# google-research/semivl

Hardware: AMD Instinct MI355X
Metric: train images/sec (512^2, ViT-B/16) (higher is better)
Workload: dtype f32 (fp32 in / out / accumulate everywhere; the MFMA products as split 16-bit terms with fp32 accumulation: the ViT's linears, in_proj weight gradients and fused attention and the decoder's 3x3 convolutions (tiled: forward, input and weight gradient; dilated: forward, input gradient) on fp16 x 2 ope; 1 GPU; SemiVL step, pascal N=21, vlm-vlg-aspp-s2p4-sk04-ftap-mcvitb, 512x512, bs=16/GPU labeled + 16/GPU unlabeled (BASELINE configs[1]); global_batch=32, parallelism=dp1

## Files before the change

### include/semivl_hip.h

```cpp
#ifndef SEMIVL_HIP_H_
#define SEMIVL_HIP_H_

#include <stddef.h>
#include <stdint.h>

#ifdef __cplusplus
extern "C" {
#endif

typedef void* svl_stream_t;

typedef enum svl_status {
  SVL_OK = 0,
  SVL_ERR_INVALID_ARG = -1,
  SVL_ERR_LAUNCH = -2,
  SVL_ERR_UNSUPPORTED = -3
} svl_status;

int svl_version(void);
int svl_stream_release(svl_stream_t stream);
int svl_stream_prepare(svl_stream_t stream);
int svl_stream_helper(svl_stream_t stream, void** helper);
int svl_shutdown(void);
int svl_num_stream_contexts(void);
// ... 128 lines not shown
                        svl_stream_t stream);

int svl_cutmix_f32(float* out, const float* a, const float* b, const float* box, int B, int C, int64_t HW,
                   svl_stream_t stream);
int svl_cutmix_i64(int64_t* out, const int64_t* a, const int64_t* b, const float* box, int B, int64_t HW,
                   svl_stream_t stream);

typedef struct svl_ce_desc {
  const float* logits;
  int B, N;
  int64_t HW;
  const int64_t* target;
  int use_ignore_t;
  const float* conf;
  const int64_t* ign;
  float conf_thresh;
  int all_pixels;
  const int64_t* mc_target;
  float* partials;
  float* dlogits;
  const float* gscale;
  const float* img_weight;
} svl_ce_desc;
int64_t svl_ce_num_blocks(int B, int N, int64_t HW);
int svl_ce_fused_f32(const svl_ce_desc* d, svl_stream_t stream);
int svl_ce_finalize(const float* partials, int64_t nblocks, double* sums , svl_stream_t stream);

typedef struct svl_ce_up_desc {
  const float* logits;
  int B, N;
  int h, w, H, W;
  int align_corners;
  const int64_t* target;
  int use_ignore_t;
  const float* conf;
  const int64_t* ign;
  float conf_thresh;
  int all_pixels;
  const int64_t* mc_target;
  float* partials;
  float* dlogits;
  const float* gscale;
  const float* img_weight;
} svl_ce_up_desc;
int64_t svl_ce_up_num_blocks(int B, int N, int h, int w, int H, int W, int align_corners);
int svl_ce_up_fused_f32(const svl_ce_up_desc* d, svl_stream_t stream);
int svl_softmax_max_up_f32(const float* logits, int B, int N, int h, int w, int H, int W, int align_corners, float* conf,
                           int64_t* label, svl_stream_t stream);

int svl_semivl_gscale(const int64_t* counts, double numel_u, float lam, const double* factors, const int64_t* mc_counts,
                      float* gscale, svl_stream_t stream);
int64_t svl_conf_avg_ws_doubles(int B);
int svl_conf_avg_factor(const float* conf, const int64_t* ign, int B, int64_t HW, double* factor, double* workspace,
                        svl_stream_t stream);
int svl_conf_ratio_f32(const float* conf, const int64_t* ign, int B, int64_t HW, float thresh, float* ratio,
                       double* workspace, svl_stream_t stream);
int svl_semivl_loss(const double* sums, double numel_u, float lam, const double* factors, const int64_t* mc_counts,
                    float* out, svl_stream_t stream);
int svl_softmax_planes_f32(const float* logits, int B, int N, int64_t HW, float* out, svl_stream_t stream);

int svl_target_prob_f32(const float* logits, int B, int N, int64_t HW, const int64_t* target, float* prob,
                        svl_stream_t stream);
int svl_target_prob_up_f32(const float* logits, int B, int N, int h, int w, int H, int W, int align_corners,
                           const int64_t* target, float* prob, svl_stream_t stream);
int64_t svl_ohem_ws_bytes(int64_t n);
int svl_ohem_threshold_f32(const float* prob, int64_t n, int64_t k, const int64_t* num_valid, int64_t min_kept,
                           float thresh, void* ws, float* threshold, svl_stream_t stream);
int svl_ohem_relabel_i64(const int64_t* target, const float* prob, int64_t n, const float* threshold, int64_t* out,
                         int64_t* count, svl_stream_t stream);

int svl_count_valid_i64(const int64_t* map, int64_t n, int64_t* count, svl_stream_t stream);

int svl_maskclip_labels(const float* dense, int B, int N, int h, int w, int H, int W, float scale,
                        float thresh, const int64_t* ign, int64_t* out, svl_stream_t stream);

int svl_concept_max_f32(const float* pred, int B, int NC, int64_t HW, const int* concept_offsets, int N,
                        float* out, svl_stream_t stream);

int svl_iou_hist_i64(const int64_t* pred, const int64_t* target, int64_t n, int K, int ignore_index, int64_t* hist,
                     svl_stream_t stream);


int svl_layernorm_fwd(const float* x, const float* gamma, const float* beta, float eps, int64_t rows, int C,
                      float* y, float* stats, svl_stream_t stream);
int svl_layernorm_fwd_planes(const float* x, const float* gamma, const float* beta, float eps, int64_t rows, int C,
                             float* y, float* stats, void* planes, int64_t planes_rows, svl_stream_t stream);
int svl_layernorm_fwd_planes_f16x2(const float* x, const float* gamma, const float* beta, float eps, int64_t rows, int C,
                                   float* y, float* stats, void* planes, int64_t planes_rows, int32_t* sexp, float* rnorm,
                                   svl_stream_t stream);
int svl_layernorm_fwd_pack_f16x2(const float* x, const float* gamma, const float* beta, float eps, int64_t rows, int C,
                                 float* y, float* stats, void* planes, int64_t planes_rows, int64_t row_off, int32_t* sexp,
                                 float* rnorm, int row_rnorm, unsigned* tensor_amax, svl_stream_t stream);
int svl_layernorm_bwd_pack_f16x2(const float* dy, const float* x, const float* stats, const float* gamma, int64_t rows, int C,
                                 const float* dx_add, float* dx, void* planes, int64_t planes_rows, int64_t row_off,
                                 int32_t* sexp, float* rnorm, unsigned* tensor_amax, svl_stream_t stream);
int svl_layernorm_bwd_parts(int64_t rows);
int svl_layernorm_bwd(const float* dy, const float* x, const float* stats, const float* gamma, int64_t rows,
                      int C, const float* dx_add, float* dx, float* dgamma_part, float* dbeta_part,
                      svl_stream_t stream);
int svl_softmax_rows_fwd(float* s, int64_t rows, int cols, int64_t ld, float scale, svl_stream_t stream);
int svl_softmax_rows_bwd(float* dp, const float* p, int64_t rows, int cols, int64_t ld, float scale,
                         svl_stream_t stream);

int svl_l2norm_fwd(const float* x, int64_t rows, int C, float eps, float* y, float* inv_norm, svl_stream_t stream);
int svl_l2norm_bwd(const float* dy, const float* y, const float* inv_norm, int64_t rows, int C, float* dx,
                   svl_stream_t stream);

int64_t svl_colsum_ws_floats(int64_t rows, int C);
int svl_colsum_f32(const float* x, int64_t rows, int C, int64_t ld, float* out, int accumulate, float* ws,
                   svl_stream_t stream);

int svl_eltwise_f32(int mode, const float* a, const float* b, float* out, int64_t n, svl_stream_t stream);
int svl_chanmask_f32(const float* x, const float* mask, float scale, int64_t rows, int rows_per_img, int C,
                     float* out, svl_stream_t stream);
int svl_fill_f32(float* p, float v, int64_t n, svl_stream_t stream);
int svl_bernoulli_f32(float* p, int64_t n, float keep_prob, uint64_t seed, uint64_t offset, svl_stream_t stream);
int svl_affine_planes_f32(const float* x, int64_t planes, int C, int64_t HW, const float* k4, float* y, svl_stream_t stream);
int svl_copy2d_f32(const float* src, int64_t sgrp, int64_t src_go, int64_t src_ld, float* dst, int64_t dgrp,
                   int64_t dst_go, int64_t dst_ld, int64_t rows, int C, int accumulate, svl_stream_t stream);
int svl_permute4_f32(const float* src, float* dst, int64_t n0, int64_t n1, int64_t n2, int64_t n3, int64_t s0, int64_t s1,
                     int64_t s2, int64_t s3, svl_stream_t stream);
int svl_bound2_f32(const float* rnorm, int64_t rows, const float* bias, int64_t nbias, float* out2, svl_stream_t stream);
int svl_permute_rows_f32(const float* src, int64_t outer, int A, int B, int C, float* dst, svl_stream_t stream);

int svl_groupnorm_fwd(const float* x, int64_t ldx, const float* gamma, const float* beta, float eps, int imgs,
                      int64_t HW, int C, int G, int relu, float* y, int64_t ldy, float* stats, svl_stream_t stream);
int64_t svl_conv3x3_gn_ws_doubles(int imgs, int H, int W, int N);
int svl_conv3x3_gn_f32(const float* src1, int64_t ld1, int C1, const float* src2, int64_t ld2, int C2, int rep,
                       const float* w, int imgs, int H, int W, int N, float* out, int64_t ldo, float eps, double* ws,
                       float* stats, const float* gn_in, const void* w_planes, svl_stream_t stream);
int64_t svl_conv3x3_weight_planes_bytes(int N, int Ct);
int svl_conv3x3_weight_planes(const float* w, int N, int Ct, void* planes, svl_stream_t stream);
int svl_groupnorm_scale_shift(const float* stats, const float* gamma, const float* beta, int imgs, int C, int G, float* scsh,
                              svl_stream_t stream);
int svl_groupnorm_apply(const float* x, int64_t ldx, const float* gamma, const float* beta, int imgs, int64_t HW, int C, int G,
                        int relu, const float* stats, float* y, int64_t ldy, svl_stream_t stream);
int svl_groupnorm_bwd(const float* dy, int64_t lddy, const float* x, int64_t ldx, const float* y, int64_t ldy,
                      const float* stats, const float* gamma, const float* beta, int imgs, int64_t HW, int C, int G,
                      int relu, float* dx, int64_t lddx, float* chan_sums, svl_stream_t stream);
int64_t svl_conv3x3_gnb_ws_doubles(int imgs, int H, int W, int N);
int svl_conv3x3_dgrad_gnb_f32(const float* dy, int64_t lddy, int C1, const float* w, int imgs, int H, int W, int N, float* out,
                              int64_t ldo, int accumulate, const float* gnb_x, const float* gnb_table, const float* gnb_stats,
                              double* ws, float* chan_sums, const void* w_planes, svl_stream_t stream);
int svl_groupnorm_bwd_apply(const float* dy, int64_t lddy, const float* x, int64_t ldx, const float* stats, const float* gamma,
                            const float* beta, int imgs, int64_t HW, int C, int G, int relu, const float* chan_sums, float* dx,
                            int64_t lddx, svl_stream_t stream);


int svl_attention_fwd(const float* qkv, int B, int T, int H, float* out, float* lse, void* out_planes,
                      int64_t planes_rows, svl_stream_t stream);
int svl_attention_bwd(const float* qkv, const float* out, const float* dout, const float* lse, int B, int T, int H,
                      float* dsum_ws, float* dqkv, void* dqkv_planes, int64_t planes_rows, svl_stream_t stream);
int64_t svl_attention_h2_ws_bytes(int B, int T, int H, int backward);
int svl_attention_fwd_h2(const float* qkv, int B, int T, int H, float* out, float* lse, void* out_planes,
                         int64_t planes_rows, void* ws, int64_t ws_bytes, svl_stream_t stream);
int svl_attention_bwd_h2(const float* qkv, const float* out, const float* dout, const float* lse, int B, int T, int H,
                         float* dsum_ws, float* dqkv, void* dqkv_planes, int64_t planes_rows, void* ws, int64_t ws_bytes,
                         svl_stream_t stream);

typedef struct svl_seqattn_desc {
  int groups, inner, seq, heads;
  int64_t outer_stride, inner_stride, seq_stride;
  const float* qkv;
  float* out;
  float* probs;
  const float* dout;
  float* dqkv;
  float* dscores;
} svl_seqattn_desc;
int svl_seqattn_fwd(const svl_seqattn_desc* d, svl_stream_t stream);
int svl_seqattn_bwd(const svl_seqattn_desc* d, svl_stream_t stream);

int svl_conv_cout1_fwd(const float* x, int64_t ldx, int imgs, int H, int W, int C, int KH, int KW, int dil, int pad,
                       const float* w, const float* bias, const float* gn_in, float* y, svl_stream_t stream);
int svl_conv_cout1_wgrad_blocks(int imgs, int H, int W);
int svl_conv_cout1_wgrad(const float* dy, const float* x, int64_t ldx, int imgs, int H, int W, int C, int dil, int pad,
                         const float* gn_in, float* slabs, svl_stream_t stream);
int svl_tap_gather(const float* T, int imgs, int H, int W, int KH, int KW, int dil, int pad, int sign, float* out,
                   svl_stream_t stream);

int svl_bilinear_nhwc_fwd(const float* x, int64_t ldx, int imgs, int h, int w, int C, int align_corners, int rep,
                          int H, int W, float* y, int64_t ldy, int accumulate, svl_stream_t stream);
int svl_sum_rep_f32(const float* src, int64_t ld, int64_t groups, int rep, int64_t rows, int C, float* out,
                    svl_stream_t stream);
int svl_bilinear_nhwc_bwd(const float* dy, int64_t lddy, int imgs, int h, int w, int C, int align_corners, int rep,
                          int H, int W, float* dx, int64_t lddx, int accumulate, svl_stream_t stream);
int svl_bilinear_planes_fwd(const float* x, int64_t planes, int h, int w, int align_corners, int H, int W, float* y,
                            svl_stream_t stream);
int svl_bilinear_planes_bwd(const float* dy, int64_t planes, int h, int w, int align_corners, int H, int W,
                            float* dx, svl_stream_t stream);
int svl_avgpool_cat_fwd(const float* x, int imgs, int H, int W, int C, int PH, int PW, const float* text, int Ct,
                        int nclass, float* y, svl_stream_t stream);
int svl_avgpool_cat_bwd(const float* dy, int imgs, int H, int W, int C, int PH, int PW, int Ct, float* dx,
                        int accumulate, svl_stream_t stream);
int svl_avgpool_cat_bwd_text(const float* dy, int imgs, int64_t HWp, int C, int Ct, int nclass, float* part, float* dtext,
                             svl_stream_t stream);

int svl_adamw_step(float* p, const float* g, float* m, float* v, const int64_t* seg_off, const float* seg_lr,
                   const float* seg_wd, int nseg, int64_t total, float beta1, float beta2, float eps, int step,
                   float gscale, float* ema, float ema_decay, svl_stream_t stream);
int svl_sgd_step(float* p, const float* g, float* m, const int64_t* seg_off, const float* seg_lr, const float* seg_wd,
                 int nseg, int64_t total, float momentum, float dampening, int nesterov, int step, float gscale,
                 float* ema, float ema_decay, svl_stream_t stream);

int64_t svl_bn_ws_doubles(int64_t rows, int C);
int svl_bn_stats(const float* x, int64_t ldx, int64_t rows, int C, double* sums, double* ws, svl_stream_t stream);
int svl_bn_finalize(const double* sums, double count, float eps, float momentum, float* running_mean, float* running_var,
                    int C, float* mean, float* invstd, svl_stream_t stream);
int svl_bn_eval_invstd(const float* running_var, float eps, int C, float* invstd, svl_stream_t stream);
int svl_bn_apply(const float* x, int64_t ldx, int64_t rows, int C, const float* mean, const float* invstd,
                 const float* gamma, const float* beta, const float* resid, int64_t ldr, int relu, float* y, int64_t ldy,
                 svl_stream_t stream);
int svl_bn_bwd_reduce(const float* dy, int64_t lddy, const float* x, int64_t ldx, const float* y, int64_t ldy,
                      const float* mean, const float* invstd, const float* remask_gamma, const float* remask_beta,
                      int64_t rows, int C, double* sums, double* ws, svl_stream_t stream);
int svl_bn_bwd_apply(const float* dy, int64_t lddy, const float* x, int64_t ldx, const float* y, int64_t ldy,
                     const float* mean, const float* invstd, const float* gamma, const float* remask_beta,
                     const double* sums, double count, int64_t rows, int C, float* dx, int64_t lddx, float* dres,
                     int64_t lddr, svl_stream_t stream);
int svl_maxpool3x3s2_fwd(const float* x, int imgs, int H, int W, int C, float* y, unsigned char* idx,
                         svl_stream_t stream);
int svl_maxpool3x3s2_bwd(const float* dy, const unsigned char* idx, int imgs, int H, int W, int C, float* dx,
                         svl_stream_t stream);

int svl_gap_tokens_fwd(const float* x, int64_t ldx, int imgs, int64_t HW, int C, float* pool, int64_t ldp,
                       svl_stream_t stream);
int svl_gap_tokens_bwd(const float* dpool, int64_t ldp, int imgs, int64_t HW, int C, float* dx, int64_t lddx,
                       int accumulate, svl_stream_t stream);
int svl_bcast_rows_fwd(const float* v, int64_t ldv, int imgs, int64_t HW, int C, float* dst, int64_t ldd, int c_off,
                       svl_stream_t stream);
int svl_bcast_rows_bwd(const float* dy, int64_t lddy, int c_off, int imgs, int64_t HW, int C, float* dv, int64_t ldv,
                       svl_stream_t stream);

int svl_aug_resample_u8(const unsigned char* src, int H, int W, int C, int rh, int rw, int x0, int y0, int OH, int OW,
                        int flip, int mode, int fill, unsigned char* dst, svl_stream_t stream);
int svl_aug_to_float(const unsigned char* src, int npix, const float* mean3, const float* std3, float* dst,
                     svl_stream_t stream);
int svl_aug_mask_i64(const unsigned char* src, int npix, int from, int to, int64_t* dst, svl_stream_t stream);
int svl_aug_photometric_u8(unsigned char* img, int npix, int op, float factor, unsigned long long* scratch,
                           svl_stream_t stream);
int svl_aug_gaussian_blur_u8(const unsigned char* src, int H, int W, float sigma, unsigned char* tmp, unsigned char* dst,
                             svl_stream_t stream);

#ifdef __cplusplus
}
#endif
#endif
```

### semivl_amd/csrc/attention.hip

```cpp
#include "attn_shared.h"
#include "attn_h2.h"

namespace {

__device__ __forceinline__ void tile_gload(float4 (&rg)[4], const float* base, long ld, int row0, int T, int tid) {
#pragma unroll
  for (int p = 0; p < 4; ++p) {
    const int f = tid + 256 * p;
    const int row = row0 + (f >> 4), c4 = (f & 15) << 2;
    rg[p] = (row < T) ? *reinterpret_cast<const float4*>(base + (long)row * ld + c4) : make_float4(0.f, 0.f, 0.f, 0.f);
  }
}
template <int LD>
__device__ __forceinline__ void tile_sstore(float* S, const float4 (&rg)[4], int tid, float mul) {
#pragma unroll
  for (int p = 0; p < 4; ++p) {
    const int f = tid + 256 * p;
    const int row = f >> 4, c = (f & 15) << 2;
    *reinterpret_cast<float4*>(S + row * LD + c) = make_float4(rg[p].x * mul, rg[p].y * mul, rg[p].z * mul, rg[p].w * mul);
  }
}

__device__ __forceinline__ float4 ld4(const float* p) { return *reinterpret_cast<const float4*>(p); }
__device__ __forceinline__ void row_gload32(float (&r)[32], const float* p, float mul) {
// ... 408 lines not shown
  sum = block_sum_256(sum, red);
  const float o = weighted_rowsum(w, head + 2 * p.E, p.ld, p.T, red, tid);
  if (tid < D) {
    if (p.out) p.out[((long)b * p.T + qi) * p.E + h * D + tid] = o / sum;
  }
  if (tid == 0 && p.lse) p.lse[(long)z * p.T + qi] = mx + logf(sum);
}

__global__ __launch_bounds__(256) void attn_bwd_dq_rows_kernel(const AttnP p, int row0) {
  __shared__ __attribute__((aligned(16))) float qv[D];
  __shared__ __attribute__((aligned(16))) float ov[D];
  __shared__ float w[ROWS_MAX_T];
  __shared__ float red[256];
  const int tid = threadIdx.x, sub = tid & 15, grp = tid >> 4;
  const int z = blockIdx.y, b = z / p.H, h = z - b * p.H, qi = row0 + blockIdx.x;
  const float* head = p.qkv + (long)b * p.T * p.ld + h * D;
  if (tid < D) {
    qv[tid] = head[(long)qi * p.ld + tid] * p.scale;
    ov[tid] = p.dout[((long)b * p.T + qi) * p.E + h * D + tid];
  }
  __syncthreads();
  const float lse_i = p.lse[(long)z * p.T + qi], d_i = p.dsum[(long)z * p.T + qi];
  for (int j0 = 0; j0 < p.T; j0 += 16) {
    const int j = j0 + grp;
    const float* kr = head + p.E + (long)min(j, p.T - 1) * p.ld;
    const float sc = dot16(qv, kr, sub), dp = dot16(ov, kr + p.E, sub);
    if (j < p.T && sub == 0) w[j] = expf(sc - lse_i) * (dp - d_i);
  }
  __syncthreads();
  const float dq = weighted_rowsum(w, head + p.E, p.ld, p.T, red, tid);
  if (tid < D) {
    p.dqkv[((long)b * p.T + qi) * p.ld + h * D + tid] = dq * p.scale;
  }
}

__global__ __launch_bounds__(256) void attn_bwd_dkv_rows_kernel(const AttnP p, int row0) {
  __shared__ __attribute__((aligned(16))) float kv[D];
  __shared__ __attribute__((aligned(16))) float vv[D];
  __shared__ float wp[ROWS_MAX_T];
  __shared__ float wd[ROWS_MAX_T];
  __shared__ float red[256];
  const int tid = threadIdx.x, sub = tid & 15, grp = tid >> 4;
  const int z = blockIdx.y, b = z / p.H, h = z - b * p.H, kj = row0 + blockIdx.x;
  const float* head = p.qkv + (long)b * p.T * p.ld + h * D;
  const float* dhead = p.dout + (long)b * p.T * p.E + h * D;
  if (tid < D) {
    kv[tid] = head[p.E + (long)kj * p.ld + tid] * p.scale;
    vv[tid] = head[2 * p.E + (long)kj * p.ld + tid];
  }
  __syncthreads();
  for (int i0 = 0; i0 < p.T; i0 += 16) {
    const int i = i0 + grp, ic = min(i, p.T - 1);
    const float sc = dot16(kv, head + (long)ic * p.ld, sub), dp = dot16(vv, dhead + (long)ic * p.E, sub);
    if (i < p.T && sub == 0) {
      const float pv = expf(sc - p.lse[(long)z * p.T + i]);
      wp[i] = pv;
      wd[i] = pv * (dp - p.dsum[(long)z * p.T + i]);
    }
  }
  __syncthreads();
  const float dv = weighted_rowsum(wp, dhead, p.E, p.T, red, tid);
  const float dk = weighted_rowsum(wd, head, p.ld, p.T, red, tid);
  if (tid < D) {
    float* row = p.dqkv + ((long)b * p.T + kj) * p.ld + h * D;
    row[p.E + tid] = dk * p.scale;
    row[2 * p.E + tid] = dv;
  }
}

__host__ inline int rows_split(int T, int* nb, int BQ = 128) {
  const int full = T / BQ, r = T - full * BQ;
  const bool use = r > 0 && r <= 4 && full > 0 && T <= ROWS_MAX_T;
  *nb = use ? full : (T + BQ - 1) / BQ;
  return use ? r : 0;
}

int check(const float* qkv, int B, int T, int H, const char* who) {
  SVL_CHECK_ARG(qkv && B > 0 && T > 0 && H > 0 && (long)B * H <= 65535, "%s: bad args", who);
  SVL_CHECK_ARG(((uintptr_t)qkv & 15) == 0, "%s: qkv must be 16-byte aligned", who);
  return SVL_OK;
}

int no_planes(const void* planes, const char* who) {
  if (!planes) return SVL_OK;
  svl_set_error("%s: planes outputs were retired with the bf16 x 6 attention kernels (pass null; pack the fp32 result)", who);
  return SVL_ERR_UNSUPPORTED;
}

}

extern "C" int svl_attention_fwd(const float* qkv, int B, int T, int H, float* out, float* lse, void* out_planes,
                                 int64_t planes_rows, svl_stream_t stream) {
  int rc = check(qkv, B, T, H, "svl_attention_fwd");
  if (rc) return rc;
  SVL_CHECK_ARG(out, "svl_attention_fwd: out missing");
  (void)planes_rows;
  rc = no_planes(out_planes, "svl_attention_fwd");
  if (rc) return rc;
  AttnP p;
  memset(&p, 0, sizeof(p));
  p.qkv = qkv; p.out = out; p.lse = lse; p.B = B; p.T = T; p.H = H; p.E = (long)H * D; p.ld = 3 * p.E; p.scale = 0.125f;
  hipStream_t st = (hipStream_t)stream;
  int nb = 0;
  const int r = rows_split(T, &nb, 128);
  if (r > 0) {
    hipStream_t aux = nullptr;
    rc = svl_fork(st, &aux);
    if (rc) return rc;
    hipLaunchKernelGGL(attn_fwd_rows_kernel, dim3(r, B * H), dim3(256), 0, aux, p, nb * 128);
    SVL_LAUNCH_CHECK("svl_attention_fwd/rows");
  }
  hipLaunchKernelGGL(attn_fwd_kernel, dim3(nb, B * H), dim3(256), 0, st, p);
  SVL_LAUNCH_CHECK("svl_attention_fwd");
  return r > 0 ? svl_join(st) : SVL_OK;
}

extern "C" int svl_attention_bwd(const float* qkv, const float* out, const float* dout, const float* lse, int B, int T,
                                 int H, float* dsum_ws, float* dqkv, void* dq_planes, int64_t planes_rows,
                                 svl_stream_t stream) {
  int rc = check(qkv, B, T, H, "svl_attention_bwd");
  if (rc) return rc;
  SVL_CHECK_ARG(out && dout && lse && dsum_ws && dqkv, "svl_attention_bwd: null args");
  (void)planes_rows;
  rc = no_planes(dq_planes, "svl_attention_bwd");
  if (rc) return rc;
  hipStream_t st = (hipStream_t)stream;
  AttnP p;
  memset(&p, 0, sizeof(p));
  p.qkv = qkv; p.dout = dout; p.lse = const_cast<float*>(lse); p.dsum = dsum_ws; p.dqkv = dqkv;
  p.B = B; p.T = T; p.H = H; p.E = (long)H * D; p.ld = 3 * p.E; p.scale = 0.125f;
  const long groups = (long)B * T * H;
  hipLaunchKernelGGL(attn_dsum_kernel, dim3((unsigned)((groups * 16 + 255) / 256)), dim3(256), 0, st, dout, out, dsum_ws,
                     B, T, H, p.E);
  SVL_LAUNCH_CHECK("svl_attention_bwd/dsum");
  int nb = 0;
  const int r = rows_split(T, &nb, 128);
  if (r > 0) {
    hipStream_t aux = nullptr;
    rc = svl_fork(st, &aux);
    if (rc) return rc;
    hipLaunchKernelGGL(attn_bwd_dkv_rows_kernel, dim3(r, B * H), dim3(256), 0, aux, p, nb * 128);
    SVL_LAUNCH_CHECK("svl_attention_bwd/dkv_rows");
    hipLaunchKernelGGL(attn_bwd_dq_rows_kernel, dim3(r, B * H), dim3(256), 0, aux, p, nb * 128);
    SVL_LAUNCH_CHECK("svl_attention_bwd/dq_rows");
  }
  hipLaunchKernelGGL(attn_bwd_dkv_kernel, dim3(nb, B * H), dim3(256), 0, st, p);
  SVL_LAUNCH_CHECK("svl_attention_bwd/dkv");
  hipLaunchKernelGGL(attn_bwd_dq_kernel, dim3(nb, B * H), dim3(256), 0, st, p);
  SVL_LAUNCH_CHECK("svl_attention_bwd/dq");
  return r > 0 ? svl_join(st) : SVL_OK;
}

extern "C" int64_t svl_attention_h2_ws_bytes(int B, int T, int H, int backward) {
  if (B <= 0 || T <= 0 || H <= 0) return 0;
  return svl_attn_h2::ws_bytes(B, T, H, backward);
}

extern "C" int svl_attention_fwd_h2(const float* qkv, int B, int T, int H, float* out, float* lse, void* out_planes,
                                    int64_t planes_rows, void* ws, int64_t ws_bytes, svl_stream_t stream) {
  int rc = check(qkv, B, T, H, "svl_attention_fwd_h2");
  if (rc) return rc;
  SVL_CHECK_ARG(out, "svl_attention_fwd_h2: out missing");
  (void)planes_rows;
  rc = no_planes(out_planes, "svl_attention_fwd_h2");
  if (rc) return rc;
  AttnP p;
  memset(&p, 0, sizeof(p));
  p.qkv = qkv; p.out = out; p.lse = lse; p.B = B; p.T = T; p.H = H; p.E = (long)H * D; p.ld = 3 * p.E; p.scale = 0.125f;
  hipStream_t st = (hipStream_t)stream;
  int nb = 0;
  const int r = rows_split(T, &nb, FQ);
  rc = svl_attn_h2::fwd_pack(p, ws, ws_bytes, st);
  if (rc) return rc;
  if (r > 0) {
    hipStream_t aux = nullptr;
    rc = svl_fork(st, &aux);
    if (rc) return rc;
    rc = svl_attn_h2::fwd_tail(p, nb * FQ, ws, aux);
    if (rc) return rc;
  }
  rc = svl_attn_h2::fwd(p, nb, ws, ws_bytes, st);
  if (rc) return rc;
  return r > 0 ? svl_join(st) : SVL_OK;
}

extern "C" int svl_attention_bwd_h2(const float* qkv, const float* out, const float* dout, const float* lse, int B, int T,
                                    int H, float* dsum_ws, float* dqkv, void* dq_planes, int64_t planes_rows, void* ws,
                                    int64_t ws_bytes, svl_stream_t stream) {
  int rc = check(qkv, B, T, H, "svl_attention_bwd_h2");
  if (rc) return rc;
  SVL_CHECK_ARG(out && dout && lse && dsum_ws && dqkv, "svl_attention_bwd_h2: null args");
  (void)planes_rows;
  rc = no_planes(dq_planes, "svl_attention_bwd_h2");
  if (rc) return rc;
  hipStream_t st = (hipStream_t)stream;
  AttnP p;
  memset(&p, 0, sizeof(p));
  p.qkv = qkv; p.dout = dout; p.lse = const_cast<float*>(lse); p.dsum = dsum_ws; p.dqkv = dqkv;
  p.B = B; p.T = T; p.H = H; p.E = (long)H * D; p.ld = 3 * p.E; p.scale = 0.125f;
  rc = svl_attn_h2::bwd_prepare(p, out, dsum_ws, ws, ws_bytes, st);
  if (rc) return rc;
  int nb = 0;
  const int r = rows_split(T, &nb, FQ);
  if (r > 0) {
    hipStream_t aux = nullptr;
    rc = svl_fork(st, &aux);
    if (rc) return rc;
    rc = svl_attn_h2::bwd_tail(p, nb * FQ, ws, aux);
    if (rc) return rc;
  }
  rc = svl_attn_h2::bwd_main(p, nb, ws, st);
  if (rc) return rc;
  return r > 0 ? svl_join(st) : SVL_OK;
}
```

### semivl_amd/csrc/attn_h2.h

```cpp
#pragma once
#include "attn_shared.h"

namespace svl_attn_h2 {

long ws_bytes(int B, int T, int H, int backward);
int fwd(const AttnP& p, int nb, void* ws, long wsb, hipStream_t st);
int bwd_prepare(const AttnP& p, const float* out, float* dsum_ws, void* ws, long wsb, hipStream_t st);
int bwd_main(const AttnP& p, int nb, void* ws, hipStream_t st);
int fwd_pack(const AttnP& p, void* ws, long wsb, hipStream_t st);
int fwd_tail(const AttnP& p, int row0, void* ws, hipStream_t aux);
int bwd_tail(const AttnP& p, int row0, void* ws, hipStream_t aux);

}
```

### semivl_amd/csrc/attn_h2.hip

```cpp
#include "attn_h2.h"
#include <atomic>

namespace {

typedef _Float16 f16x8 __attribute__((ext_vector_type(8)));
typedef _Float16 f16x2 __attribute__((ext_vector_type(2)));

struct H2W {
  const char *q_rm, *k_rm, *v_rm, *do_rm, *q_tr, *k_tr, *v_tr, *do_tr;
  const int* exps;
  const float* nrm;
  const float* ld;
  int Tp;
};

__device__ __forceinline__ void glds16(const char* base_, unsigned lane_off, unsigned lds_dst_) {
  const unsigned long long bv = (unsigned long long)base_;
  const unsigned b_hi = (unsigned)__builtin_amdgcn_readfirstlane((int)(bv >> 32));
  const unsigned b_lo = (unsigned)__builtin_amdgcn_readfirstlane((int)(unsigned)bv);
  const char* base = (const char*)(((unsigned long long)b_hi << 32) | (unsigned long long)b_lo);
  const unsigned lds_dst = __builtin_amdgcn_readfirstlane(lds_dst_);
  unsigned keep;
  asm volatile("s_mov_b32 %0, m0\n\ts_mov_b32 m0, %3\n\ts_nop 3\n\tglobal_load_lds_dwordx4 %2, %1\n\ts_mov_b32 m0, %0"
               : "=&s"(keep)
               : "s"(base), "v"(lane_off), "s"(lds_dst)
               : "memory");
}
template <int N_>
__device__ __forceinline__ void wait_vm() {
  asm volatile("s_waitcnt vmcnt(%0)" ::"n"(N_) : "memory");
}
__device__ __forceinline__ void interval_barrier() {
  asm volatile("s_waitcnt lgkmcnt(0)" ::: "memory");
  __builtin_amdgcn_sched_barrier(0);
  __builtin_amdgcn_s_barrier();
  __builtin_amdgcn_sched_barrier(0);
}

__device__ __forceinline__ f32x16 mfma_h(const f16x8& a, const f16x8& b, const f32x16& c) {
  return __builtin_amdgcn_mfma_f32_32x32x16_f16(a, b, c, 0, 0, 0);
}
#define H2_PAIR(c0, a0, c1, a1, b)    \
  c0 = mfma_h(a0[1], b[0], c0);       \
  c1 = mfma_h(a1[1], b[0], c1);       \
  c0 = mfma_h(a0[0], b[1], c0);       \
  c1 = mfma_h(a1[0], b[1], c1);       \
  c0 = mfma_h(a0[0], b[0], c0);       \
  c1 = mfma_h(a1[0], b[0], c1);
#define H2_2(c0, a0, b0, c1, a1, b1)  \
  c0 = mfma_h(a0[1], b0[0], c0);      \
  c1 = mfma_h(a1[1], b1[0], c1);      \
  c0 = mfma_h(a0[0], b0[1], c0);      \
  c1 = mfma_h(a1[0], b1[1], c1);      \
  c0 = mfma_h(a0[0], b0[0], c0);      \
  c1 = mfma_h(a1[0], b1[0], c1);
#define H2_2T(c0, a0, b0, c1, a1, b1) \
  c0 = mfma_h(a0[0], b0[1], c0);      \
  c1 = mfma_h(a1[0], b1[1], c1);      \
  c0 = mfma_h(a0[1], b0[0], c0);      \
  c1 = mfma_h(a1[1], b1[0], c1);      \
  c0 = mfma_h(a0[0], b0[0], c0);      \
  c1 = mfma_h(a1[0], b1[0], c1);

template <bool MIX>
__device__ __forceinline__ void split2x8(const float (&x)[8], f16x8 (&h)[2]) {
  u32x4 w0, w1;
#pragma unroll
  for (int jp = 0; jp < 4; ++jp) {
    const f32x2 pr = {x[2 * jp], x[2 * jp + 1]};
    const f16x2 ah = __builtin_convertvector(pr, f16x2);
    const unsigned a = __builtin_bit_cast(unsigned, ah);
    f32x2 r;
    if constexpr (MIX) {
      asm("v_fma_mix_f32 %0, %1, -1.0, %2 op_sel_hi:[1,0,0]" : "=v"(r[0]) : "v"(a), "v"(pr[0]));
      asm("v_fma_mix_f32 %0, %1, -1.0, %2 op_sel:[1,0,0] op_sel_hi:[1,0,0]" : "=v"(r[1]) : "v"(a), "v"(pr[1]));
    } else {
      r = pr - __builtin_convertvector(ah, f32x2);
    }
    w0[jp] = a;
    w1[jp] = __builtin_bit_cast(unsigned, __builtin_convertvector(r, f16x2));
  }
  h[0] = __builtin_bit_cast(f16x8, w0);
  h[1] = __builtin_bit_cast(f16x8, w1);
}
__device__ __forceinline__ void frag2(f16x8 (&a)[2], const char* chunk0) {
  a[0] = *reinterpret_cast<const f16x8*>(chunk0);
  a[1] = *reinterpret_cast<const f16x8*>(chunk0 + 1024);
}
__device__ __forceinline__ int ds_exp(float nrm_do, float nrm_v) {
  const float bt = 2.f * nrm_do * nrm_v;
  int g = bt > 0.f ? __builtin_amdgcn_frexp_expf(bt) : 0;
  return g < -100 ? -100 : (g > 100 ? 100 : g);
}

struct PackP {
  const float* src[4];
  long ld[4];
  char* rm[4];
  char* tr[4];
  int which[4];
  int* exps;
  float* nrm;
  int B, T, H, Tp;
};

__global__ __launch_bounds__(256) void attn_pack_kernel(const PackP p) {
  __shared__ __attribute__((aligned(16))) float tile[64 * LDP];
  __shared__ float red[4];
  const int tid = threadIdx.x, z = blockIdx.x, w = p.which[blockIdx.y];
  const int b = z / p.H, h = z - b * p.H;
  const long ld = p.ld[w];
  const float* src = p.src[w] + (long)b * p.T * ld + h * D;
  const int r16 = tid >> 4, c4 = (tid & 15) << 2;
  const int nrb = p.Tp >> 5;
  char* rm = p.rm[w] ? p.rm[w] + (long)z * nrb * 8192 : nullptr;
  char* tr = p.tr[w] ? p.tr[w] + (long)z * p.Tp * 256 : nullptr;
  const int lane = tid & 63, cq = tid >> 6, hh = lane >> 5, r = lane & 31;
  auto rows = [&](int r0, float4 (&v)[4]) __attribute__((always_inline)) {
#pragma unroll
    for (int i = 0; i < 4; ++i) {
      const int row = r0 + 16 * i + r16;
      v[i] = row < p.T ? *reinterpret_cast<const float4*>(src + (long)row * ld + c4) : make_float4(0.f, 0.f, 0.f, 0.f);
    }
  };
  auto amax4 = [](const float4& a) { return fmaxf(fmaxf(fabsf(a.x), fabsf(a.y)), fmaxf(fabsf(a.z), fabsf(a.w))); };
  auto exp_of = [](float mx) {
    const int e = mx > 0.f ? __builtin_amdgcn_frexp_expf(mx) - 15 : 0;
    return e < -100 ? -100 : (e > 100 ? 100 : e);
  };
  float4 v[4];
  rows(0, v);
  float m0 = fmaxf(fmaxf(amax4(v[0]), amax4(v[1])), fmaxf(amax4(v[2]), amax4(v[3])));
  m0 = block_max_256(m0, red);
  int e = exp_of(m0) + 3;
  float mx = 0.f, nr = 0.f;
  for (int attempt = 0; attempt < 2; ++attempt) {
    if (attempt) rows(0, v);
    mx = 0.f;
    nr = 0.f;
    for (int r0 = 0; r0 < p.Tp; r0 += 64) {
#pragma unroll
      for (int i = 0; i < 4; ++i) {
        mx = fmaxf(mx, amax4(v[i]));
        float ss = v[i].x * v[i].x + v[i].y * v[i].y + v[i].z * v[i].z + v[i].w * v[i].w;
#pragma unroll
        for (int o = 8; o > 0; o >>= 1) ss += __shfl_xor(ss, o, 64);
        nr = fmaxf(nr, ss);
        *reinterpret_cast<float4*>(&tile[(16 * i + r16) * LDP + c4]) =
            make_float4(__builtin_amdgcn_ldexpf(v[i].x, -e), __builtin_amdgcn_ldexpf(v[i].y, -e),
                        __builtin_amdgcn_ldexpf(v[i].z, -e), __builtin_amdgcn_ldexpf(v[i].w, -e));
      }
      if (r0 + 64 < p.Tp) rows(r0 + 64, v);
      __syncthreads();
#pragma unroll
      for (int half = 0; half < 2; ++half) {
        const int rb = (r0 >> 5) + half;
        const float* th = tile + half * 32 * LDP;
        if (rm) {
          const float* t = th + r * LDP + 16 * cq + 4 * hh;
          const float4 u = *reinterpret_cast<const float4*>(t), q = *reinterpret_cast<const float4*>(t + 8);
          const float x[8] = {u.x, u.y, u.z, u.w, q.x, q.y, q.z, q.w};
          f16x8 hp[2];
          split2x8<true>(x, hp);
          char* c = rm + (long)((rb * 4 + cq) * 2) * 1024 + lane * 16;
          *reinterpret_cast<f16x8*>(c) = hp[0];
          *reinterpret_cast<f16x8*>(c + 1024) = hp[1];
        }
        if (tr) {
          const int kgl = cq >> 1, rbd = cq & 1;
          const float* t = th + (16 * kgl + 4 * hh) * LDP + 32 * rbd + r;
          float x[8];
#pragma unroll
          for (int j = 0; j < 8; ++j) x[j] = t[((j & 3) + 8 * (j >> 2)) * LDP];
          f16x8 hp[2];
          split2x8<true>(x, hp);
          char* c = tr + (long)(((2 * rb + kgl) * 2 + rbd) * 2) * 1024 + lane * 16;
          *reinterpret_cast<f16x8*>(c) = hp[0];
          *reinterpret_cast<f16x8*>(c + 1024) = hp[1];
        }
      }
      __syncthreads();
    }
    mx = block_max_256(mx, red);
    const int ex = exp_of(mx);
    if (ex <= e && ex >= e - 3) break;
    e = ex;
  }
  nr = block_max_256(nr, red);
  if (tid == 0) {
    p.exps[z * 4 + w] = e;
    p.nrm[z * 4 + w] = sqrtf(nr);
  }
}

__global__ __launch_bounds__(256) void attn_ld_kernel(const float* __restrict__ dout, const float* __restrict__ out,
                                                      const float* __restrict__ lse, const float* __restrict__ nrm,
                                                      float* __restrict__ dsum, float* __restrict__ ld, int B, int T, int H,
                                                      int Tp, long E) {
  const long total = (long)B * H * Tp;
  const long g = ((long)blockIdx.x * 256 + threadIdx.x) >> 4;
  const int sub = threadIdx.x & 15;
  if (g >= total) return;
  const int z = (int)(g / Tp), t = (int)(g - (long)z * Tp);
  const int b = z / H, h = z - b * H;
  float s = 0.f;
  if (t < T) {
    const long off = ((long)b * T + t) * E + h * D + sub * 4;
    const float4 a = *reinterpret_cast<const float4*>(dout + off), c = *reinterpret_cast<const float4*>(out + off);
    s = a.x * c.x + a.y * c.y + a.z * c.z + a.w * c.w;
  }
#pragma unroll
  for (int o = 8; o > 0; o >>= 1) s += __shfl_xor(s, o, 64);
  if (sub == 0) {
    float2 v = make_float2(-INFINITY, 0.f);
    if (t < T) {
      dsum[(long)z * T + t] = s;
      v.x = -lse[(long)z * T + t] * LOG2E;
      v.y = __builtin_amdgcn_ldexpf(s, 14 - ds_exp(nrm[z * 4 + 3], nrm[z * 4 + 2]));
    }
    *reinterpret_cast<float2*>(ld + ((long)z * Tp + t) * 2) = v;
  }
}

constexpr int STG_F = 32 * 1024;

template <int V>
__global__ __launch_bounds__(512) void attn_fwd_h2_kernel(const AttnP p, const H2W w) {
  constexpr bool MIX = (V & 1) != 0;
  extern __shared__ __attribute__((aligned(1024))) char sm[];
  const int tid = threadIdx.x, lane = tid & 63, l31 = lane & 31, hi = lane >> 5;
  const int wave = __builtin_amdgcn_readfirstlane(tid >> 6);
  int rb_, z;
  attn_block(p, FQ, rb_, z);
  const int b = z / p.H, h = z - b * p.H;
  const int q0 = rb_ * FQ + wave * 32;
  const int qi = q0 + l31;
  const bool wave_active = q0 < p.T;
  const int off = wave >= 4 ? 1 : 0;
  const int nkt = w.Tp >> 6;
  const long rmz = (long)(w.Tp >> 5) * 8192, trz = (long)w.Tp * 256;
  const char* ksrc = w.k_rm + z * rmz;
  const char* vsrc = w.v_tr + z * trz;
  const unsigned lane16 = lane * 16;
  const unsigned sm_base = (unsigned)(uintptr_t)(__attribute__((address_space(3))) char*)sm;
  f16x8 qf[2][4];
  {
    const char* qs = w.q_rm + z * rmz + (long)(min(q0, w.Tp - 32) >> 5) * 8192 + lane16;
#pragma unroll
    for (int kg = 0; kg < 4; ++kg)
#pragma unroll
      for (int pl = 0; pl < 2; ++pl) qf[pl][kg] = *reinterpret_cast<const f16x8*>(qs + (kg * 2 + pl) * 1024);
  }
  const int eq = w.exps[z * 4], ek = w.exps[z * 4 + 1], ev = w.exps[z * 4 + 2];
  const float c = __builtin_amdgcn_ldexpf(LOG2E, eq + ek - 3);
  auto issue_part = [&](int tile, int part, int stage) __attribute__((always_inline)) {
    const int tc = min(tile, nkt - 1);
    const char* s = (part ? vsrc : ksrc) + (long)tc * 16384 + wave * 2048;
    const unsigned dst = sm_base + stage * STG_F + part * 16384 + wave * 2048;
    glds16(s, lane16, dst);
    glds16(s + 1024, lane16, dst + 1024);
  };
  f32x16 o0, o1, s0, s1;
#pragma unroll
  for (int r = 0; r < 16; ++r) { o0[r] = 0.f; o1[r] = 0.f; s0[r] = 0.f; s1[r] = 0.f; }
  float m2s = -INFINITY, l = 0.f;
  issue_part(0, 0, 0);
  issue_part(0, 1, 0);
  issue_part(1, 0, 1);
  issue_part(1, 1, 1);
  wait_vm<6>();
  interval_barrier();

  const bool short_last = p.T - (nkt - 1) * 64 <= 32;
  auto phase1 = [&](int kt, auto last_c) __attribute__((always_inline)) {
    constexpr bool LAST = decltype(last_c)::value;
    const char* Ks = sm + (kt % 3) * STG_F + lane16;
#pragma unroll
    for (int r = 0; r < 16; ++r) { s0[r] = 0.f; s1[r] = 0.f; }
    if (LAST && short_last) {
#pragma unroll
      for (int kg = 0; kg < 4; ++kg) {
        f16x8 a0[2], bq[2] = {qf[0][kg], qf[1][kg]};
        frag2(a0, Ks + (kg * 2) * 1024);
        s0 = mfma_h(a0[1], bq[0], s0);
        s0 = mfma_h(a0[0], bq[1], s0);
        s0 = mfma_h(a0[0], bq[0], s0);
      }
      return;
    }
#pragma unroll
    for (int kg = 0; kg < 4; ++kg) {
      f16x8 a0[2], a1[2], bq[2] = {qf[0][kg], qf[1][kg]};
      frag2(a0, Ks + (kg * 2) * 1024);
      frag2(a1, Ks + ((4 + kg) * 2) * 1024);
      H2_PAIR(s0, a0, s1, a1, bq)
    }
  };
  auto phase2 = [&](int kt, auto last_c) __attribute__((always_inline)) {
    constexpr bool LAST = decltype(last_c)::value;
    const char* Vt = sm + (kt % 3) * STG_F + 16384 + lane16;
    if (LAST) {
      const int j0 = kt * 64;
#pragma unroll
      for (int r = 0; r < 16; ++r) {
        const int key = j0 + crow(r, hi);
        if (key >= p.T) s0[r] = -INFINITY;
        if (key + 32 >= p.T) s1[r] = -INFINITY;
      }
    }
    auto max3c = [](float a, float b, float c) { return __builtin_fmaxf(__builtin_fmaxf(a, b), c); };
    float ma = max3c(s0[0], s0[1], s0[2]), mb = max3c(s1[0], s1[1], s1[2]);
#pragma unroll
    for (int r = 3; r < 15; r += 2) {
      ma = max3c(ma, s0[r], s0[r + 1]);
      mb = max3c(mb, s1[r], s1[r + 1]);
    }
    float mloc = max3c(ma, mb, fmaxf(s0[15], s1[15]));
    mloc = fmaxf(mloc, __shfl_xor(mloc, 32, 64));
    const float mloc2 = mloc * c;
    const bool raise = mloc2 > m2s + (7.f + RESCALE_LOG2);
    if (__any(raise)) {
      const float mnew = raise ? mloc2 - 7.f : m2s;
      const float alpha = __builtin_amdgcn_exp2f(m2s - mnew);
      l *= alpha;
#pragma unroll
      for (int r = 0; r < 16; ++r) { o0[r] *= alpha; o1[r] *= alpha; }
      m2s = mnew;
    }
    float sum0 = 0.f, sum1 = 0.f;
    const int ntp = (LAST && short_last) ? 2 : 4;
#pragma unroll
    for (int tp = 0; tp < 4; ++tp) {
      if (tp >= ntp) break;
      float x[8];
#pragma unroll
      for (int j = 0; j < 8; ++j) {
        x[j] = __builtin_amdgcn_exp2f(fmaf((tp < 2) ? s0[8 * (tp & 1) + j] : s1[8 * (tp & 1) + j], c, -m2s));
        if (j & 1) sum1 += x[j]; else sum0 += x[j];
      }
      f16x8 pb[2], a0[2], a1[2];
      split2x8<MIX>(x, pb);
      frag2(a0, Vt + ((tp * 2) * 2) * 1024);
      frag2(a1, Vt + ((tp * 2 + 1) * 2) * 1024);
      H2_PAIR(o0, a0, o1, a1, pb)
    }
    l += sum0 + sum1;
  };

  if constexpr ((V & 2) != 0) {
    wait_vm<4>();
    interval_barrier();
    for (int kt = 0; kt < nkt - 1; ++kt) {
      issue_part(kt + 2, 0, (kt + 2) % 3);
      issue_part(kt + 2, 1, (kt + 2) % 3);
      if (wave_active) {
        phase1(kt, std::false_type{});
        phase2(kt, std::false_type{});
      }
      wait_vm<4>();
      interval_barrier();
    }
    if (wave_active) {
      phase1(nkt - 1, std::true_type{});
      phase2(nkt - 1, std::true_type{});
    }
    interval_barrier();
  } else {
    const int nint = 2 * nkt + 1;
    for (int n = 0; n < nint; ++n) {
      issue_part((n >> 1) + 2, n & 1, ((n >> 1) + 2) % 3);
      const int k = n - off;
      if (wave_active && k >= 0 && k < 2 * nkt) {
        if ((k >> 1) == nkt - 1) {
          if (k & 1) phase2(k >> 1, std::true_type{});
          else phase1(k >> 1, std::true_type{});
        } else {
          if (k & 1) phase2(k >> 1, std::false_type{});
          else phase1(k >> 1, std::false_type{});
        }
      }
      wait_vm<6>();
      interval_barrier();
    }
  }
  wait_vm<0>();
  if (wave_active && qi < p.T) {
    const float lt = l + __shfl_xor(l, 32, 64);
    const float inv = __builtin_amdgcn_ldexpf(1.f / lt, ev);
    if (p.out) {
      float* orow = p.out + ((long)b * p.T + qi) * p.E + h * D;
#pragma unroll
      for (int g = 0; g < 4; ++g) {
        const int d0 = 8 * g + 4 * hi;
        *reinterpret_cast<float4*>(orow + d0) =
            make_float4(o0[4 * g] * inv, o0[4 * g + 1] * inv, o0[4 * g + 2] * inv, o0[4 * g + 3] * inv);
        *reinterpret_cast<float4*>(orow + 32 + d0) =
            make_float4(o1[4 * g] * inv, o1[4 * g + 1] * inv, o1[4 * g + 2] * inv, o1[4 * g + 3] * inv);
      }
    }
    if (p.lse && hi == 0) p.lse[(long)z * p.T + qi] = (m2s + __log2f(lt)) * LN2;
  } else if (wave_active) {
    (void)__shfl_xor(l, 32, 64);
  }
}

constexpr int STG_Q = 48 * 1024;

template <int V>
__global__ __launch_bounds__(512) void attn_dq_h2_kernel(const AttnP p, const H2W w) {
  constexpr bool MIX = (V & 1) != 0;
  extern __shared__ __attribute__((aligned(1024))) char sm[];
  const int tid = threadIdx.x, lane = tid & 63, l31 = lane & 31, hi = lane >> 5;
  const int wave = __builtin_amdgcn_readfirstlane(tid >> 6);
  int rb_, z;
  attn_block(p, FQ, rb_, z);
  const int b = z / p.H, h = z - b * p.H;
  const int q0 = rb_ * FQ + wave * 32;
  const int qi = q0 + l31;
  const bool wave_active = q0 < p.T;
  const int nkt = w.Tp >> 6;
  const long rmz = (long)(w.Tp >> 5) * 8192, trz = (long)w.Tp * 256;
  const char* src3[3] = {w.k_rm + z * rmz, w.v_rm + z * rmz, w.k_tr + z * trz};
  const unsigned lane16 = lane * 16;
  const unsigned sm_base = (unsigned)(uintptr_t)(__attribute__((address_space(3))) char*)sm;
  f16x8 qf[2][4], of[2][4];
  {
    const long ro = z * rmz + (long)(min(q0, w.Tp - 32) >> 5) * 8192 + lane16;
#pragma unroll
    for (int kg = 0; kg < 4; ++kg)
#pragma unroll
      for (int pl = 0; pl < 2; ++pl) {
        qf[pl][kg] = *reinterpret_cast<const f16x8*>(w.q_rm + ro + (kg * 2 + pl) * 1024);
        of[pl][kg] = *reinterpret_cast<const f16x8*>(w.do_rm + ro + (kg * 2 + pl) * 1024);
      }
  }
  const float2 ad = *reinterpret_cast<const float2*>(w.ld + ((long)z * w.Tp + min(qi, w.Tp - 1)) * 2);
  const float a_i = ad.x, d_i = ad.y;
  const int eq = w.exps[z * 4], ek = w.exps[z * 4 + 1], ev = w.exps[z * 4 + 2], edo = w.exps[z * 4 + 3];
  const int gs = ds_exp(w.nrm[z * 4 + 3], w.nrm[z * 4 + 2]);
  const float c = __builtin_amdgcn_ldexpf(LOG2E, eq + ek - 3);
  const float cdp = __builtin_amdgcn_ldexpf(1.f, edo + ev + 14 - gs);
  f32x16 dq0, dq1;
#pragma unroll
  for (int r = 0; r < 16; ++r) { dq0[r] = 0.f; dq1[r] = 0.f; }
  auto issue_tile = [&](int tile, int stage) __attribute__((always_inline)) {
    const int tc = min(tile, nkt - 1);
#pragma unroll
    for (int i = 0; i < 6; ++i) {
      const int cidx = wave * 6 + i, part = cidx >> 4, cc = cidx & 15;
      const char* s = (part == 0 ? src3[0] : part == 1 ? src3[1] : src3[2]) + (long)tc * 16384 + cc * 1024;
      glds16(s, lane16, sm_base + stage * STG_Q + cidx * 1024);
    }
  };
  issue_tile(0, 0);
  issue_tile(1, 1);
  wait_vm<6>();
  interval_barrier();
  auto tile = [&](int kt, auto last_c) __attribute__((always_inline)) {
    constexpr bool last = decltype(last_c)::value;
    {
      const char* Ks = sm + (kt % 3) * STG_Q + lane16;
      const char* Vs = Ks + 16384;
      const char* Kt = Ks + 32768;
#pragma unroll
      for (int jt = 0; jt < 2; ++jt) {
        if (!last || jt == 0 || p.T - kt * 64 > 32) {
          f32x16 sa, dp;
#pragma unroll
          for (int r = 0; r < 16; ++r) { sa[r] = 0.f; dp[r] = 0.f; }
#pragma unroll
          for (int kg = 0; kg < 4; ++kg) {
            f16x8 ka[2], va[2], bq[2] = {qf[0][kg], qf[1][kg]}, bo[2] = {of[0][kg], of[1][kg]};
            frag2(ka, Ks + ((jt * 4 + kg) * 2) * 1024);
            frag2(va, Vs + ((jt * 4 + kg) * 2) * 1024);
            H2_2(sa, ka, bq, dp, va, bo)
          }
          if (last) {
#pragma unroll
            for (int r = 0; r < 16; ++r)
              if (kt * 64 + jt * 32 + crow(r, hi) >= p.T) sa[r] = -INFINITY;
          }
#pragma unroll
          for (int t = 0; t < 2; ++t) {
            float x[8];
#pragma unroll
            for (int j = 0; j < 8; ++j)
              x[j] = __builtin_amdgcn_exp2f(fmaf(sa[8 * t + j], c, a_i)) * fmaf(dp[8 * t + j], cdp, -d_i);
            f16x8 pb[2], a0[2], a1[2];
            split2x8<MIX>(x, pb);
            frag2(a0, Kt + (((2 * jt + t) * 2) * 2) * 1024);
            frag2(a1, Kt + (((2 * jt + t) * 2 + 1) * 2) * 1024);
            H2_PAIR(dq0, a0, dq1, a1, pb)
          }
        }
      }
    }
  };
  for (int kt = 0; kt < nkt - 1; ++kt) {
    issue_tile(kt + 2, (kt + 2) % 3);
    if (wave_active) tile(kt, std::false_type{});
    wait_vm<6>();
    interval_barrier();
  }
  if (wave_active) tile(nkt - 1, std::true_type{});
  wait_vm<0>();
  if (wave_active && qi < p.T) {
    const float f = __builtin_amdgcn_ldexpf(1.f, gs - 14 + ek - 3);
    float* row = p.dqkv + ((long)b * p.T + qi) * p.ld + h * D;
#pragma unroll
    for (int g = 0; g < 4; ++g) {
      const int d0 = 8 * g + 4 * hi;
      *reinterpret_cast<float4*>(row + d0) = make_float4(dq0[4 * g] * f, dq0[4 * g + 1] * f, dq0[4 * g + 2] * f, dq0[4 * g + 3] * f);
      *reinterpret_cast<float4*>(row + 32 + d0) = make_float4(dq1[4 * g] * f, dq1[4 * g + 1] * f, dq1[4 * g + 2] * f, dq1[4 * g + 3] * f);
    }
  }
}

constexpr int STG_K = 33 * 1024;

template <int V>
__global__ __launch_bounds__(512) void attn_dkv_h2_kernel(const AttnP p, const H2W w) {
  constexpr bool MIX = (V & 1) != 0;
  extern __shared__ __attribute__((aligned(1024))) char sm[];
  const int tid = threadIdx.x, lane = tid & 63, l31 = lane & 31, hi = lane >> 5;
  const int wave = __builtin_amdgcn_readfirstlane(tid >> 6);
  int rb_, z;
  attn_block(p, FQ, rb_, z);
  const int b = z / p.H, h = z - b * p.H;
  const int k0 = rb_ * FQ + wave * 32;
  const bool wave_active = k0 < p.T;
  const int nqt = (p.T + 31) >> 5;
  const long rmz = (long)(w.Tp >> 5) * 8192, trz = (long)w.Tp * 256;
  const char* src4[4] = {w.q_rm + z * rmz, w.do_rm + z * rmz, w.q_tr + z * trz, w.do_tr + z * trz};
  const char* ldsrc = reinterpret_cast<const char*>(w.ld + (long)z * w.Tp * 2);
  const unsigned lane16 = lane * 16;
  const unsigned sm_base = (unsigned)(uintptr_t)(__attribute__((address_space(3))) char*)sm;
  f16x8 kf[2][4], vf[2][4];
  {
    const long ro = z * rmz + (long)(min(k0, w.Tp - 32) >> 5) * 8192 + lane16;
#pragma unroll
    for (int kg = 0; kg < 4; ++kg)
#pragma unroll
      for (int pl = 0; pl < 2; ++pl) {
        kf[pl][kg] = *reinterpret_cast<const f16x8*>(w.k_rm + ro + (kg * 2 + pl) * 1024);
        vf[pl][kg] = *reinterpret_cast<const f16x8*>(w.v_rm + ro + (kg * 2 + pl) * 1024);
      }
  }
  const int eq = w.exps[z * 4], ek = w.exps[z * 4 + 1], ev = w.exps[z * 4 + 2], edo = w.exps[z * 4 + 3];
  const int gs = ds_exp(w.nrm[z * 4 + 3], w.nrm[z * 4 + 2]);
  const float c = __builtin_amdgcn_ldexpf(LOG2E, eq + ek - 3);
  const float cdp = __builtin_amdgcn_ldexpf(1.f, edo + ev + 14 - gs);
  f32x16 dv0, dv1, dk0, dk1;
#pragma unroll
  for (int r = 0; r < 16; ++r) { dv0[r] = 0.f; dv1[r] = 0.f; dk0[r] = 0.f; dk1[r] = 0.f; }
  auto issue_tile = [&](int tile, int stage) __attribute__((always_inline)) {
    const int tc = min(tile, nqt - 1);
#pragma unroll
    for (int i = 0; i < 4; ++i) {
      const int cidx = wave * 4 + i, part = cidx >> 3, cc = cidx & 7;
      const char* s = (part == 0 ? src4[0] : part == 1 ? src4[1] : part == 2 ? src4[2] : src4[3]) + (long)tc * 8192 + cc * 1024;
      glds16(s, lane16, sm_base + stage * STG_K + cidx * 1024);
    }
    if (wave == 0) glds16(ldsrc + (long)tc * 256, lane16, sm_base + stage * STG_K + 32768);
  };
  auto wait_older = [&]() __attribute__((always_inline)) {
    if (wave == 0) wait_vm<5>();
    else wait_vm<4>();
  };
  issue_tile(0, 0);
  issue_tile(1, 1);
  wait_older();
  interval_barrier();
  for (int qt = 0; qt < nqt; ++qt) {
    issue_tile(qt + 2, (qt + 2) % 3);
    if (wave_active) {
      const char* Qs = sm + (qt % 3) * STG_K + lane16;
      const char* Os = Qs + 8192;
      const char* Qt = Qs + 16384;
      const char* Ot = Qs + 24576;
      const float* LD = reinterpret_cast<const float*>(sm + (qt % 3) * STG_K + 32768);
      f32x16 sa, dp;
#pragma unroll
      for (int r = 0; r < 16; ++r) { sa[r] = 0.f; dp[r] = 0.f; }
#pragma unroll
      for (int kg = 0; kg < 4; ++kg) {
        f16x8 qa[2], oa[2], bk[2] = {kf[0][kg], kf[1][kg]}, bv[2] = {vf[0][kg], vf[1][kg]};
        frag2(qa, Qs + (kg * 2) * 1024);
        frag2(oa, Os + (kg * 2) * 1024);
        H2_2T(sa, qa, bk, dp, oa, bv)
      }
#pragma unroll
      for (int t = 0; t < 2; ++t) {
        float xp[8], xs[8];
#pragma unroll
        for (int g = 0; g < 2; ++g) {
          const int r0 = 8 * t + 4 * g;
          const float4 u = *reinterpret_cast<const float4*>(LD + crow(r0, hi) * 2);
          const float4 v = *reinterpret_cast<const float4*>(LD + crow(r0, hi) * 2 + 4);
          const float aq[4] = {u.x, u.z, v.x, v.z}, dq[4] = {u.y, u.w, v.y, v.w};
#pragma unroll
          for (int i = 0; i < 4; ++i) {
            const float pv = __builtin_amdgcn_exp2f(fmaf(sa[r0 + i], c, aq[i]));
            xp[4 * g + i] = pv * 16384.f;
            xs[4 * g + i] = pv * fmaf(dp[r0 + i], cdp, -dq[i]);
          }
        }
        f16x8 pa[2], sa2[2], o0[2], o1[2], q0f[2], q1f[2];
        split2x8<MIX>(xp, pa);
        split2x8<MIX>(xs, sa2);
        frag2(o0, Ot + ((t * 2) * 2) * 1024);
        frag2(o1, Ot + ((t * 2 + 1) * 2) * 1024);
        H2_2(dv0, pa, o0, dv1, pa, o1)
        frag2(q0f, Qt + ((t * 2) * 2) * 1024);
        frag2(q1f, Qt + ((t * 2 + 1) * 2) * 1024);
        H2_2(dk0, sa2, q0f, dk1, sa2, q1f)
      }
    }
    wait_older();
    interval_barrier();
  }
  wait_vm<0>();
  interval_barrier();
  if (wave_active) {
    const float fk = __builtin_amdgcn_ldexpf(1.f, gs - 14 + eq - 3);
    const float fv = __builtin_amdgcn_ldexpf(1.f, edo - 14);
#pragma unroll
    for (int r = 0; r < 16; ++r) { dk0[r] *= fk; dk1[r] *= fk; dv0[r] *= fv; dv1[r] *= fv; }
#pragma unroll
    for (int r = 0; r < 16; ++r) {
      const int key = k0 + crow(r, hi);
      if (key < p.T) {
        float* row = p.dqkv + ((long)b * p.T + key) * p.ld + h * D;
        row[p.E + l31] = dk0[r];
        row[p.E + 32 + l31] = dk1[r];
        row[2 * p.E + l31] = dv0[r];
        row[2 * p.E + 32 + l31] = dv1[r];
      }
    }
  }
}

constexpr int TAILW = 4;
template <bool MIX>
__global__ __launch_bounds__(64 * TAILW) __attribute__((amdgpu_waves_per_eu(4, 4))) void attn_fwd_tail_h2_kernel(const AttnP p, const H2W w, int row0) {
  const int lane = threadIdx.x & 63, l31 = lane & 31, hi = lane >> 5;
  const int wave = __builtin_amdgcn_readfirstlane(threadIdx.x >> 6);
  const int z = blockIdx.x, b = z / p.H, h = z - b * p.H;
  const int q0 = row0 + 32 * (int)blockIdx.y, qi = q0 + l31;
  const int nkt = w.Tp >> 6;
  const long rmz = (long)(w.Tp >> 5) * 8192, trz = (long)w.Tp * 256;
  const unsigned lane16 = lane * 16;
  const char* ksrc = w.k_rm + z * rmz + lane16;
  const char* vsrc = w.v_tr + z * trz + lane16;
  const char* qs = w.q_rm + z * rmz + (long)(q0 >> 5) * 8192 + lane16;
  const int eq = w.exps[z * 4], ek = w.exps[z * 4 + 1], ev = w.exps[z * 4 + 2];
  const float c = __builtin_amdgcn_ldexpf(LOG2E, eq + ek - 3);
  f32x16 o0, o1;
#pragma unroll
  for (int r = 0; r < 16; ++r) { o0[r] = 0.f; o1[r] = 0.f; }
  float m2s = -INFINITY, l = 0.f;
  const bool short_last = p.T - (nkt - 1) * 64 <= 32;
  for (int kt = wave; kt < nkt; kt += TAILW) {
    const char* Ks = ksrc + (long)kt * 16384;
    const char* Vt = vsrc + (long)kt * 16384;
    const bool last = kt == nkt - 1, half = last && short_last;
    f32x16 s0, s1;
#pragma unroll
    for (int r = 0; r < 16; ++r) { s0[r] = 0.f; s1[r] = 0.f; }
#pragma unroll
    for (int kg = 0; kg < 4; ++kg) {
      f16x8 a0[2], bq[2];
      frag2(bq, qs + (kg * 2) * 1024);
      frag2(a0, Ks + (kg * 2) * 1024);
      s0 = mfma_h(a0[1], bq[0], s0);
      s0 = mfma_h(a0[0], bq[1], s0);
      s0 = mfma_h(a0[0], bq[0], s0);
      if (!half) {
        f16x8 a1[2];
        frag2(a1, Ks + ((4 + kg) * 2) * 1024);
        s1 = mfma_h(a1[1], bq[0], s1);
        s1 = mfma_h(a1[0], bq[1], s1);
        s1 = mfma_h(a1[0], bq[0], s1);
      }
    }
    if (last) {
#pragma unroll
      for (int r = 0; r < 16; ++r) {
        const int key = kt * 64 + crow(r, hi);
        if (key >= p.T) s0[r] = -INFINITY;
        if (key + 32 >= p.T) s1[r] = -INFINITY;
      }
    }
    float mloc = fmaxf(s0[0], s1[0]);
#pragma unroll
    for (int r = 1; r < 16; ++r) mloc = fmaxf(mloc, fmaxf(s0[r], s1[r]));
    mloc = fmaxf(mloc, __shfl_xor(mloc, 32, 64));
    const float mloc2 = mloc * c;
    const bool raise = mloc2 > m2s + (7.f + RESCALE_LOG2);
    if (__any(raise)) {
      const float mnew = raise ? mloc2 - 7.f : m2s;
      const float alpha = __builtin_amdgcn_exp2f(m2s - mnew);
      l *= alpha;
#pragma unroll
      for (int r = 0; r < 16; ++r) { o0[r] *= alpha; o1[r] *= alpha; }
      m2s = mnew;
    }
    float sum = 0.f;
#pragma unroll
    for (int tp = 0; tp < 4; ++tp) {
      if (half && tp >= 2) break;
      float x[8];
#pragma unroll
      for (int j = 0; j < 8; ++j) {
        x[j] = __builtin_amdgcn_exp2f(fmaf((tp < 2) ? s0[8 * (tp & 1) + j] : s1[8 * (tp & 1) + j], c, -m2s));
        sum += x[j];
      }
      f16x8 pb[2], a0[2], a1[2];
      split2x8<MIX>(x, pb);
      frag2(a0, Vt + ((tp * 2) * 2) * 1024);
      frag2(a1, Vt + ((tp * 2 + 1) * 2) * 1024);
      H2_PAIR(o0, a0, o1, a1, pb)
    }
    l += sum;
  }
  __shared__ float cmb[TAILW][8][34];
  if (l31 < 4) {
    float* c_ = cmb[wave][hi * 4 + l31];
    c_[0] = m2s;
    c_[1] = l;
#pragma unroll
    for (int r = 0; r < 16; ++r) { c_[2 + r] = o0[r]; c_[18 + r] = o1[r]; }
  }
  __syncthreads();
  if (wave != 0) return;
  if (l31 < 4) {
    float mm = m2s;
#pragma unroll
    for (int w_ = 1; w_ < TAILW; ++w_) mm = fmaxf(mm, cmb[w_][hi * 4 + l31][0]);
    const float a0_ = m2s == -INFINITY ? 0.f : __builtin_amdgcn_exp2f(m2s - mm);
    l *= a0_;
#pragma unroll
    for (int r = 0; r < 16; ++r) { o0[r] *= a0_; o1[r] *= a0_; }
#pragma unroll
    for (int w_ = 1; w_ < TAILW; ++w_) {
      const float* c_ = cmb[w_][hi * 4 + l31];
      const float aw = c_[0] == -INFINITY ? 0.f : __builtin_amdgcn_exp2f(c_[0] - mm);
      l += c_[1] * aw;
#pragma unroll
      for (int r = 0; r < 16; ++r) { o0[r] += c_[2 + r] * aw; o1[r] += c_[18 + r] * aw; }
    }
    m2s = mm;
  }
  const float lt = l + __shfl_xor(l, 32, 64);
  if (qi < p.T && l31 < 4) {
    const float inv = __builtin_amdgcn_ldexpf(1.f / lt, ev);
    if (p.out) {
      float* orow = p.out + ((long)b * p.T + qi) * p.E + h * D;
#pragma unroll
      for (int g = 0; g < 4; ++g) {
        const int d0 = 8 * g + 4 * hi;
        *reinterpret_cast<float4*>(orow + d0) =
            make_float4(o0[4 * g] * inv, o0[4 * g + 1] * inv, o0[4 * g + 2] * inv, o0[4 * g + 3] * inv);
        *reinterpret_cast<float4*>(orow + 32 + d0) =
            make_float4(o1[4 * g] * inv, o1[4 * g + 1] * inv, o1[4 * g + 2] * inv, o1[4 * g + 3] * inv);
      }
    }
    if (p.lse && hi == 0) p.lse[(long)z * p.T + qi] = (m2s + __log2f(lt)) * LN2;
  }
}

template <bool MIX>
__global__ __launch_bounds__(64 * TAILW) __attribute__((amdgpu_waves_per_eu(4, 4))) void attn_dq_tail_h2_kernel(const AttnP p, const H2W w, int row0) {
  const int lane = threadIdx.x & 63, l31 = lane & 31, hi = lane >> 5;
  const int wave = __builtin_amdgcn_readfirstlane(threadIdx.x >> 6);
  const int z = blockIdx.x, b = z / p.H, h = z - b * p.H;
  const int q0 = row0 + 32 * (int)blockIdx.y, qi = q0 + l31;
  const int nkt = w.Tp >> 6;
  const long rmz = (long)(w.Tp >> 5) * 8192, trz = (long)w.Tp * 256;
  const unsigned lane16 = lane * 16;
  const char* k_rm = w.k_rm + z * rmz + lane16;
  const char* v_rm = w.v_rm + z * rmz + lane16;
  const char* k_tr = w.k_tr + z * trz + lane16;
  const char* qs = w.q_rm + z * rmz + (long)(q0 >> 5) * 8192 + lane16;
  const char* os = w.do_rm + z * rmz + (long)(q0 >> 5) * 8192 + lane16;
  const float2 ad = *reinterpret_cast<const float2*>(w.ld + ((long)z * w.Tp + min(qi, w.Tp - 1)) * 2);
  const float a_i = ad.x, d_i = ad.y;
  const int eq = w.exps[z * 4], ek = w.exps[z * 4 + 1], ev = w.exps[z * 4 + 2], edo = w.exps[z * 4 + 3];
  const int gs = ds_exp(w.nrm[z * 4 + 3], w.nrm[z * 4 + 2]);
  const float c = __builtin_amdgcn_ldexpf(LOG2E, eq + ek - 3);
  const float cdp = __builtin_amdgcn_ldexpf(1.f, edo + ev + 14 - gs);
  f32x16 dq0, dq1;
#pragma unroll
  for (int r = 0; r < 16; ++r) { dq0[r] = 0.f; dq1[r] = 0.f; }
  for (int kt = wave; kt < nkt; kt += TAILW) {
    const char* Ks = k_rm + (long)kt * 16384;
    const char* Vs = v_rm + (long)kt * 16384;
    const char* Kt = k_tr + (long)kt * 16384;
    const bool last = kt == nkt - 1;
#pragma unroll
    for (int jt = 0; jt < 2; ++jt) {
      if (!last || jt == 0 || p.T - kt * 64 > 32) {
        f32x16 sa, dp;
#pragma unroll
        for (int r = 0; r < 16; ++r) { sa[r] = 0.f; dp[r] = 0.f; }
#pragma unroll
        for (int kg = 0; kg < 4; ++kg) {
          f16x8 ka[2], bq[2];
          frag2(bq, qs + (kg * 2) * 1024);
          frag2(ka, Ks + ((jt * 4 + kg) * 2) * 1024);
          sa = mfma_h(ka[1], bq[0], sa);
          sa = mfma_h(ka[0], bq[1], sa);
          sa = mfma_h(ka[0], bq[0], sa);
          __builtin_amdgcn_sched_barrier(0);
        }
#pragma unroll
        for (int kg = 0; kg < 4; ++kg) {
          f16x8 va[2], bo[2];
          frag2(bo, os + (kg * 2) * 1024);
          frag2(va, Vs + ((jt * 4 + kg) * 2) * 1024);
          dp = mfma_h(va[1], bo[0], dp);
          dp = mfma_h(va[0], bo[1], dp);
          dp = mfma_h(va[0], bo[0], dp);
          __builtin_amdgcn_sched_barrier(0);
        }
        if (last) {
#pragma unroll
          for (int r = 0; r < 16; ++r)
            if (kt * 64 + jt * 32 + crow(r, hi) >= p.T) sa[r] = -INFINITY;
        }
#pragma unroll
        for (int t = 0; t < 2; ++t) {
          float x[8];
#pragma unroll
          for (int j = 0; j < 8; ++j)
            x[j] = __builtin_amdgcn_exp2f(fmaf(sa[8 * t + j], c, a_i)) * fmaf(dp[8 * t + j], cdp, -d_i);
          f16x8 pb[2], a0[2], a1[2];
          split2x8<MIX>(x, pb);
          frag2(a0, Kt + (((2 * jt + t) * 2) * 2) * 1024);
          frag2(a1, Kt + (((2 * jt + t) * 2 + 1) * 2) * 1024);
          H2_PAIR(dq0, a0, dq1, a1, pb)
          __builtin_amdgcn_sched_barrier(0);
        }
      }
    }
  }
  __shared__ float cmb[TAILW][8][32];
  if (l31 < 4 && wave != 0) {
    float* c_ = cmb[wave][hi * 4 + l31];
#pragma unroll
    for (int r = 0; r < 16; ++r) { c_[r] = dq0[r]; c_[16 + r] = dq1[r]; }
  }
  __syncthreads();
  if (wave != 0) return;
  if (l31 < 4) {
#pragma unroll
    for (int w_ = 1; w_ < TAILW; ++w_) {
      const float* c_ = cmb[w_][hi * 4 + l31];
#pragma unroll
      for (int r = 0; r < 16; ++r) { dq0[r] += c_[r]; dq1[r] += c_[16 + r]; }
    }
  }
  if (qi < p.T && l31 < 4) {
    const float f = __builtin_amdgcn_ldexpf(1.f, gs - 14 + ek - 3);
    float* row = p.dqkv + ((long)b * p.T + qi) * p.ld + h * D;
#pragma unroll
    for (int g = 0; g < 4; ++g) {
      const int d0 = 8 * g + 4 * hi;
      *reinterpret_cast<float4*>(row + d0) = make_float4(dq0[4 * g] * f, dq0[4 * g + 1] * f, dq0[4 * g + 2] * f, dq0[4 * g + 3] * f);
      *reinterpret_cast<float4*>(row + 32 + d0) = make_float4(dq1[4 * g] * f, dq1[4 * g + 1] * f, dq1[4 * g + 2] * f, dq1[4 * g + 3] * f);
    }
  }
}

template <bool MIX>
__global__ __launch_bounds__(64 * TAILW) __attribute__((amdgpu_waves_per_eu(4, 4))) void attn_dkv_tail_h2_kernel(const AttnP p, const H2W w, int row0) {
  const int lane = threadIdx.x & 63, l31 = lane & 31, hi = lane >> 5;
  const int wave = __builtin_amdgcn_readfirstlane(threadIdx.x >> 6);
  const int z = blockIdx.x, b = z / p.H, h = z - b * p.H;
  const int k0 = row0 + 32 * (int)blockIdx.y;
  const int nqt = (p.T + 31) >> 5;
  const long rmz = (long)(w.Tp >> 5) * 8192, trz = (long)w.Tp * 256;
  const unsigned lane16 = lane * 16;
  const char* q_rm = w.q_rm + z * rmz;
  const char* o_rm = w.do_rm + z * rmz;
  const char* q_tr = w.q_tr + z * trz;
  const char* o_tr = w.do_tr + z * trz;
  const float* ldz = w.ld + (long)z * w.Tp * 2;
  const char* ks = w.k_rm + z * rmz + (long)(k0 >> 5) * 8192;
  const char* vs = w.v_rm + z * rmz + (long)(k0 >> 5) * 8192;
  const int eq = w.exps[z * 4], ek = w.exps[z * 4 + 1], ev = w.exps[z * 4 + 2], edo = w.exps[z * 4 + 3];
  const int gs = ds_exp(w.nrm[z * 4 + 3], w.nrm[z * 4 + 2]);
  const float c = __builtin_amdgcn_ldexpf(LOG2E, eq + ek - 3);
  const float cdp = __builtin_amdgcn_ldexpf(1.f, edo + ev + 14 - gs);
  f32x16 dv0, dv1, dk0, dk1;
#pragma unroll
  for (int r = 0; r < 16; ++r) { dv0[r] = 0.f; dv1[r] = 0.f; dk0[r] = 0.f; dk1[r] = 0.f; }
  for (int qt = wave; qt < nqt; qt += TAILW) {
    const char* Qs = q_rm + (long)qt * 8192;
    const char* Os = o_rm + (long)qt * 8192;
    const char* Qt = q_tr + (long)qt * 8192;
    const char* Ot = o_tr + (long)qt * 8192;
    const float* LD = ldz + qt * 64;
    f32x16 sa, dp;
#pragma unroll
    for (int r = 0; r < 16; ++r) { sa[r] = 0.f; dp[r] = 0.f; }
#pragma unroll
    for (int kg = 0; kg < 4; ++kg) {
      f16x8 qa[2], bk[2];
      frag2(bk, ks + lane16 + (kg * 2) * 1024);
      frag2(qa, Qs + lane16 + (kg * 2) * 1024);
      sa = mfma_h(qa[0], bk[1], sa);
      sa = mfma_h(qa[1], bk[0], sa);
      sa = mfma_h(qa[0], bk[0], sa);
      __builtin_amdgcn_sched_barrier(0);
    }
#pragma unroll
    for (int kg = 0; kg < 4; ++kg) {
      f16x8 oa[2], bv[2];
      frag2(bv, vs + lane16 + (kg * 2) * 1024);
      frag2(oa, Os + lane16 + (kg * 2) * 1024);
      dp = mfma_h(oa[0], bv[1], dp);
      dp = mfma_h(oa[1], bv[0], dp);
      dp = mfma_h(oa[0], bv[0], dp);
      __builtin_amdgcn_sched_barrier(0);
    }
    f16x8 pa[2][2], sa2[2][2];
#pragma unroll
    for (int t = 0; t < 2; ++t) {
      float xp[8], xs[8];
#pragma unroll
      for (int g = 0; g < 2; ++g) {
        const int r0 = 8 * t + 4 * g;
        const float4 u = *reinterpret_cast<const float4*>(LD + crow(r0, hi) * 2);
        const float4 v = *reinterpret_cast<const float4*>(LD + crow(r0, hi) * 2 + 4);
        const float aq[4] = {u.x, u.z, v.x, v.z}, dq[4] = {u.y, u.w, v.y, v.w};
#pragma unroll
        for (int i = 0; i < 4; ++i) {
          const float pv = __builtin_amdgcn_exp2f(fmaf(sa[r0 + i], c, aq[i]));
          xp[4 * g + i] = pv * 16384.f;
          xs[4 * g + i] = pv * fmaf(dp[r0 + i], cdp, -dq[i]);
        }
      }
      split2x8<MIX>(xp, pa[t]);
      split2x8<MIX>(xs, sa2[t]);
    }
    __builtin_amdgcn_sched_barrier(0);
#pragma unroll
    for (int t = 0; t < 2; ++t) {
      f16x8 o0[2], o1[2], q0f[2], q1f[2];
      frag2(o0, Ot + lane16 + ((t * 2) * 2) * 1024);
      frag2(o1, Ot + lane16 + ((t * 2 + 1) * 2) * 1024);
      H2_2(dv0, pa[t], o0, dv1, pa[t], o1)
      __builtin_amdgcn_sched_barrier(0);
      frag2(q0f, Qt + lane16 + ((t * 2) * 2) * 1024);
      frag2(q1f, Qt + lane16 + ((t * 2 + 1) * 2) * 1024);
      H2_2(dk0, sa2[t], q0f, dk1, sa2[t], q1f)
      __builtin_amdgcn_sched_barrier(0);
    }
  }
  __shared__ float cmb[TAILW][32][16];
  if (hi == 0 && wave != 0) {
    float* c_ = cmb[wave][l31];
#pragma unroll
    for (int r = 0; r < 4; ++r) { c_[r] = dk0[r]; c_[4 + r] = dk1[r]; c_[8 + r] = dv0[r]; c_[12 + r] = dv1[r]; }
  }
  __syncthreads();
  if (wave != 0) return;
  if (hi == 0) {
#pragma unroll
    for (int w_ = 1; w_ < TAILW; ++w_) {
      const float* c_ = cmb[w_][l31];
#pragma unroll
      for (int r = 0; r < 4; ++r) { dk0[r] += c_[r]; dk1[r] += c_[4 + r]; dv0[r] += c_[8 + r]; dv1[r] += c_[12 + r]; }
    }
  }
  const float fk = __builtin_amdgcn_ldexpf(1.f, gs - 14 + eq - 3);
  const float fv = __builtin_amdgcn_ldexpf(1.f, edo - 14);
#pragma unroll
  for (int r = 0; r < 16; ++r) { dk0[r] *= fk; dk1[r] *= fk; dv0[r] *= fv; dv1[r] *= fv; }
#pragma unroll
  for (int r = 0; r < 16; ++r) {
    const int key = k0 + crow(r, hi);
    if (key < p.T) {
      float* row = p.dqkv + ((long)b * p.T + key) * p.ld + h * D;
      row[p.E + l31] = dk0[r];
      row[p.E + 32 + l31] = dk1[r];
      row[2 * p.E + l31] = dv0[r];
      row[2 * p.E + 32 + l31] = dv1[r];
    }
  }
}

struct Layout {
  long set;
  long exps, nrm, ld, total;
  int Tp;
};
Layout layout(int B, int T, int H, int backward) {
  Layout l;
  l.Tp = (T + 63) / 64 * 64;
  l.set = (long)B * H * l.Tp * 256;
  const long nset = backward ? 7 : 3;
  l.exps = nset * l.set;
  l.nrm = l.exps + (((long)B * H * 16 + 1023) & ~1023L);
  l.ld = l.nrm + (((long)B * H * 16 + 1023) & ~1023L);
  l.total = l.ld + (backward ? (((long)B * H * l.Tp * 8 + 1023) & ~1023L) + 1024 : 0);
  return l;
}

template <typename K>
int set_lds(K kernel, std::atomic<uint64_t>& mask, int bytes) {
  int dev = 0;
  (void)hipGetDevice(&dev);
  const uint64_t bit = 1ull << (dev & 63);
  if (mask.load(std::memory_order_acquire) & bit) return SVL_OK;
  SVL_HIP_CHECK(hipFuncSetAttribute(reinterpret_cast<const void*>(kernel), hipFuncAttributeMaxDynamicSharedMemorySize, bytes));
  mask.fetch_or(bit, std::memory_order_acq_rel);
  return SVL_OK;
}

H2W views(const Layout& l, char* ws, int backward) {
  H2W w;
  memset(&w, 0, sizeof(w));
  w.Tp = l.Tp;
  w.q_rm = ws;
  w.k_rm = ws + l.set;
  if (backward) {
    w.v_rm = ws + 2 * l.set;
    w.do_rm = ws + 3 * l.set;
    w.q_tr = ws + 4 * l.set;
    w.k_tr = ws + 5 * l.set;
    w.do_tr = ws + 6 * l.set;
  } else {
    w.v_tr = ws + 2 * l.set;
  }
  w.exps = reinterpret_cast<const int*>(ws + l.exps);
  w.nrm = reinterpret_cast<const float*>(ws + l.nrm);
  w.ld = reinterpret_cast<const float*>(ws + l.ld);
  return w;
}

int check_ws(const AttnP& p, const void* ws, long wsb, int backward, const char* who) {
  const Layout l = layout(p.B, p.T, p.H, backward);
  SVL_CHECK_ARG(ws && ((uintptr_t)ws & 1023) == 0 && wsb >= l.total, "%s: workspace of %ld bytes (1 KiB aligned) needed, got %ld",
                who, l.total, wsb);
  return SVL_OK;
}

}

namespace svl_attn_h2 {

long ws_bytes(int B, int T, int H, int backward) { return layout(B, T, H, backward).total; }

int fwd_pack(const AttnP& p, void* ws_, long wsb, hipStream_t st) {
  int rc = check_ws(p, ws_, wsb, 0, "svl_attention_fwd_h2");
  if (rc) return rc;
  const Layout l = layout(p.B, p.T, p.H, 0);
  char* ws = static_cast<char*>(ws_);
  const H2W w = views(l, ws, 0);
  PackP q;
  memset(&q, 0, sizeof(q));
  for (int i = 0; i < 3; ++i) {
    q.src[i] = p.qkv + i * p.E;
    q.ld[i] = p.ld;
    q.which[i] = i;
  }
  q.rm[0] = const_cast<char*>(w.q_rm);
  q.rm[1] = const_cast<char*>(w.k_rm);
  q.tr[2] = const_cast<char*>(w.v_tr);
  q.exps = const_cast<int*>(w.exps);
  q.nrm = const_cast<float*>(w.nrm);
  q.B = p.B; q.T = p.T; q.H = p.H; q.Tp = l.Tp;
  hipLaunchKernelGGL(attn_pack_kernel, dim3(p.B * p.H, 3), dim3(256), 0, st, q);
  SVL_LAUNCH_CHECK("svl_attention_fwd_h2/pack");
  return SVL_OK;
}

#define SVL_LAUNCH_V(KERN, LDS)                                       \
    rc = set_lds(KERN<3>, mask, LDS);                                   \
    if (rc) return rc;                                                  \
    hipLaunchKernelGGL(KERN<3>, grid, dim3(512), LDS, st, p, w);

int fwd(const AttnP& p, int nb, void* ws_, long wsb, hipStream_t st) {
  (void)wsb;
  if (nb <= 0) return SVL_OK;
  const Layout l = layout(p.B, p.T, p.H, 0);
  const H2W w = views(l, static_cast<char*>(ws_), 0);
  int rc = SVL_OK;
  static std::atomic<uint64_t> mask;
  const dim3 grid(nb * p.B * p.H);
  SVL_LAUNCH_V(attn_fwd_h2_kernel, 3 * STG_F)
  SVL_LAUNCH_CHECK("svl_attention_fwd_h2");
  return SVL_OK;
}

int bwd_prepare(const AttnP& p, const float* out, float* dsum_ws, void* ws_, long wsb, hipStream_t st) {
  int rc = check_ws(p, ws_, wsb, 1, "svl_attention_bwd_h2");
  if (rc) return rc;
  const Layout l = layout(p.B, p.T, p.H, 1);
  char* ws = static_cast<char*>(ws_);
  const H2W w = views(l, ws, 1);
  PackP q;
  memset(&q, 0, sizeof(q));
  for (int i = 0; i < 3; ++i) {
    q.src[i] = p.qkv + i * p.E;
    q.ld[i] = p.ld;
  }
  q.src[3] = p.dout;
  q.ld[3] = p.E;
  for (int i = 0; i < 4; ++i) q.which[i] = i;
  q.rm[0] = const_cast<char*>(w.q_rm);
  q.rm[1] = const_cast<char*>(w.k_rm);
  q.rm[2] = const_cast<char*>(w.v_rm);
  q.rm[3] = const_cast<char*>(w.do_rm);
  q.tr[0] = const_cast<char*>(w.q_tr);
  q.tr[1] = const_cast<char*>(w.k_tr);
  q.tr[3] = const_cast<char*>(w.do_tr);
  q.exps = const_cast<int*>(w.exps);
  q.nrm = const_cast<float*>(w.nrm);
  q.B = p.B; q.T = p.T; q.H = p.H; q.Tp = l.Tp;
  hipLaunchKernelGGL(attn_pack_kernel, dim3(p.B * p.H, 4), dim3(256), 0, st, q);
  SVL_LAUNCH_CHECK("svl_attention_bwd_h2/pack");
  const long groups = (long)p.B * p.H * l.Tp;
  hipLaunchKernelGGL(attn_ld_kernel, dim3((unsigned)((groups * 16 + 255) / 256)), dim3(256), 0, st, p.dout, out, p.lse, w.nrm,
                     dsum_ws, const_cast<float*>(w.ld), p.B, p.T, p.H, l.Tp, p.E);
  SVL_LAUNCH_CHECK("svl_attention_bwd_h2/dsum");
  return SVL_OK;
}

int fwd_tail(const AttnP& p, int row0, void* ws_, hipStream_t aux) {
  const Layout l = layout(p.B, p.T, p.H, 0);
  const H2W w = views(l, static_cast<char*>(ws_), 0);
  const dim3 grid(p.B * p.H, (p.T - row0 + 31) / 32);
  hipLaunchKernelGGL(attn_fwd_tail_h2_kernel<true>, grid, dim3(64 * TAILW), 0, aux, p, w, row0);
  SVL_LAUNCH_CHECK("svl_attention_fwd_h2/tail");
  return SVL_OK;
}

int bwd_tail(const AttnP& p, int row0, void* ws_, hipStream_t aux) {
  const Layout l = layout(p.B, p.T, p.H, 1);
  const H2W w = views(l, static_cast<char*>(ws_), 1);
  const dim3 grid(p.B * p.H, (p.T - row0 + 31) / 32);
  hipLaunchKernelGGL(attn_dkv_tail_h2_kernel<true>, grid, dim3(64 * TAILW), 0, aux, p, w, row0);
  hipLaunchKernelGGL(attn_dq_tail_h2_kernel<true>, grid, dim3(64 * TAILW), 0, aux, p, w, row0);
  SVL_LAUNCH_CHECK("svl_attention_bwd_h2/tail");
  return SVL_OK;
}

int bwd_main(const AttnP& p, int nb, void* ws_, hipStream_t st) {
  if (nb <= 0) return SVL_OK;
  const Layout l = layout(p.B, p.T, p.H, 1);
  const H2W w = views(l, static_cast<char*>(ws_), 1);
  int rc = SVL_OK;
  const dim3 grid(nb * p.B * p.H);
  {
    static std::atomic<uint64_t> mask;
    SVL_LAUNCH_V(attn_dkv_h2_kernel, 3 * STG_K)
    SVL_LAUNCH_CHECK("svl_attention_bwd_h2/dkv");
  }
  {
    static std::atomic<uint64_t> mask;
    SVL_LAUNCH_V(attn_dq_h2_kernel, 3 * STG_Q)
    SVL_LAUNCH_CHECK("svl_attention_bwd_h2/dq");
  }
  return SVL_OK;
}

}
```

### semivl_amd/lib.py

```python
import ctypes as C
import os
import subprocess

import torch

_HERE = os.path.dirname(os.path.abspath(__file__))
LIB_PATH = os.path.join(_HERE, "libsemivl_hip.so")
CSRC = os.path.join(_HERE, "csrc")

c_f32p = C.c_void_p
c_i64p = C.c_void_p


class Operand(C.Structure):
    _fields_ = [("ptr", C.c_void_p), ("ld", C.c_int64), ("bs_outer", C.c_int64), ("bs_inner", C.c_int64)]


class ConvGeom(C.Structure):
    _fields_ = [("H", C.c_int), ("W", C.c_int), ("Ho", C.c_int), ("Wo", C.c_int), ("stride", C.c_int),
                ("C1", C.c_int), ("C2", C.c_int), ("rep", C.c_int),
                ("KH", C.c_int), ("KW", C.c_int), ("dil", C.c_int), ("pad", C.c_int), ("sign", C.c_int),
                ("src2", C.c_void_p), ("ld2", C.c_int64), ("patch", C.c_int)]


class GemmDesc(C.Structure):
    _fields_ = [("a_mode", C.c_int), ("b_mode", C.c_int), ("M", C.c_int), ("N", C.c_int), ("K", C.c_int),
                ("batch", C.c_int), ("batch_inner", C.c_int), ("ksplit", C.c_int),
                ("A", Operand), ("B", Operand), ("conv", ConvGeom),
                ("C", C.c_void_p), ("out_mode", C.c_int),
                ("ldc_m", C.c_int64), ("ldc_n", C.c_int64), ("c_bs_outer", C.c_int64), ("c_bs_inner", C.c_int64),
                ("ct_H", C.c_int), ("ct_W", C.c_int), ("ct_Cout", C.c_int),
                ("alpha", C.c_float), ("bias", C.c_void_p), ("bias_mod", C.c_int), ("act", C.c_int),
                ("preact", C.c_void_p), ("resid", C.c_void_p),
                ("ldr_m", C.c_int64), ("ldr_n", C.c_int64), ("r_bs_outer", C.c_int64), ("r_bs_inner", C.c_int64),
                ("accumulate", C.c_int), ("conv_w_planes", C.c_void_p), ("emu_ws", C.c_void_p),
                ("b_stats", C.c_void_p), ("b_gamma", C.c_void_p), ("b_beta", C.c_void_p),
                ("a_amax", C.c_void_p), ("b_amax", C.c_void_p)]


class PGemmDesc(C.Structure):
    _fields_ = [("A", C.c_void_p), ("B", C.c_void_p), ("a_rows", C.c_int64), ("b_rows", C.c_int64),
                ("m_off", C.c_int), ("M", C.c_int), ("N", C.c_int), ("K", C.c_int),
                ("C", C.c_void_p), ("ldc", C.c_int64), ("planes_out", C.c_void_p), ("p_rows", C.c_int64),
                ("bias", C.c_void_p), ("act", C.c_int), ("preact", C.c_void_p), ("resid", C.c_void_p),
                ("ldr", C.c_int64), ("accumulate", C.c_int),
                ("fmt", C.c_int), ("p_fmt", C.c_int), ("a_sexp", C.c_void_p), ("b_sexp", C.c_void_p),
                ("a_rnorm", C.c_void_p), ("b_bound", C.c_void_p), ("p_sexp", C.c_void_p)]


class CeDesc(C.Structure):
    _fields_ = [("logits", C.c_void_p), ("B", C.c_int), ("N", C.c_int), ("HW", C.c_int64),
                ("target", C.c_void_p), ("use_ignore_t", C.c_int), ("conf", C.c_void_p), ("ign", C.c_void_p),
                ("conf_thresh", C.c_float), ("all_pixels", C.c_int), ("mc_target", C.c_void_p), ("partials", C.c_void_p),
                ("dlogits", C.c_void_p), ("gscale", C.c_void_p), ("img_weight", C.c_void_p)]


class CeUpDesc(C.Structure):
    _fields_ = [("logits", C.c_void_p), ("B", C.c_int), ("N", C.c_int), ("h", C.c_int), ("w", C.c_int), ("H", C.c_int),
                ("W", C.c_int), ("align_corners", C.c_int), ("target", C.c_void_p), ("use_ignore_t", C.c_int),
                ("conf", C.c_void_p), ("ign", C.c_void_p), ("conf_thresh", C.c_float), ("all_pixels", C.c_int),
                ("mc_target", C.c_void_p), ("partials", C.c_void_p), ("dlogits", C.c_void_p), ("gscale", C.c_void_p),
                ("img_weight", C.c_void_p)]


class SeqAttnDesc(C.Structure):
    _fields_ = [("groups", C.c_int), ("inner", C.c_int), ("seq", C.c_int), ("heads", C.c_int),
                ("outer_stride", C.c_int64), ("inner_stride", C.c_int64), ("seq_stride", C.c_int64),
                ("qkv", C.c_void_p), ("out", C.c_void_p), ("probs", C.c_void_p),
                ("dout", C.c_void_p), ("dqkv", C.c_void_p), ("dscores", C.c_void_p)]


_I, _L, _F, _D, _P = C.c_int, C.c_int64, C.c_float, C.c_double, C.c_void_p
SIGNATURES = {
    "svl_version": (_I, []),
    "svl_last_error": (_I, [C.c_char_p, C.c_size_t]),
    "svl_gemm_f32": (_I, [C.POINTER(GemmDesc), _P]),
    "svl_set_gemm_emulation": (_I, [_I]),
    "svl_get_gemm_emulation": (_I, []),
    "svl_set_conv_tiled": (_I, [_I]),
    "svl_planes_rows": (_L, [_L]),
    "svl_planes_bytes": (_L, [_L, _I]),
    "svl_split_planes_bf16x3": (_I, [_P, _L, _L, _L, _I, _P, _L, _L, _P]),
    "svl_planes_bytes_fmt": (_L, [_L, _I, _I]),
    "svl_split_planes_f16x2": (_I, [_P, _L, _L, _L, _I, _P, _L, _L, _P, _P, _P, _P]),
    "svl_gemm_planes_f32": (_I, [C.POINTER(PGemmDesc), _P]),
    "svl_conv3x3_wgrad_tiled_groups": (_I, [_I, _I, _I, _I, _I]),
    "svl_conv3x3_wgrad_tiled": (_I, [_P, _L, _I, _P, _L, _I, _P, _L, _I, _I, _I, _I, _I, _P, _I, _P, _P]),
    "svl_reduce_slabs_f32": (_I, [_P, _P, _I, _L, _I, _P]),
    "svl_softmax_max_f32": (_I, [_P, _I, _I, _L, _P, _P, _P]),
    "svl_cutmix_f32": (_I, [_P, _P, _P, _P, _I, _I, _L, _P]),
    "svl_cutmix_i64": (_I, [_P, _P, _P, _P, _I, _L, _P]),
    "svl_ce_num_blocks": (_L, [_I, _I, _L]),
    "svl_ce_fused_f32": (_I, [C.POINTER(CeDesc), _P]),
    "svl_ce_finalize": (_I, [_P, _L, _P, _P]),
    "svl_ce_up_num_blocks": (_L, [_I, _I, _I, _I, _I, _I, _I]),
    "svl_ce_up_fused_f32": (_I, [C.POINTER(CeUpDesc), _P]),
    "svl_softmax_max_up_f32": (_I, [_P, _I, _I, _I, _I, _I, _I, _I, _P, _P, _P]),
    "svl_semivl_gscale": (_I, [_P, _D, _F, _P, _P, _P, _P]),
    "svl_semivl_loss": (_I, [_P, _D, _F, _P, _P, _P, _P]),
    "svl_conf_ratio_f32": (_I, [_P, _P, _I, _L, _F, _P, _P, _P]),
    "svl_conf_avg_ws_doubles": (_L, [_I]),
    "svl_conf_avg_factor": (_I, [_P, _P, _I, _L, _P, _P, _P]),
    "svl_stream_release": (_I, [_P]),
    "svl_stream_prepare": (_I, [_P]),
    "svl_stream_helper": (_I, [_P, C.POINTER(C.c_void_p)]),
    "svl_last_gemm_path": (_I, []),
    "svl_absmax_launches": (_L, []),
    "svl_shutdown": (_I, []),
    "svl_num_stream_contexts": (_I, []),
    "svl_clock_probe": (_I, [_P, _I, C.c_uint64, _P]),
    "svl_bernoulli_f32": (_I, [_P, _L, _F, C.c_uint64, C.c_uint64, _P]),
    "svl_softmax_planes_f32": (_I, [_P, _I, _I, _L, _P, _P]),
    "svl_count_valid_i64": (_I, [_P, _L, _P, _P]),
    "svl_target_prob_f32": (_I, [_P, _I, _I, _L, _P, _P, _P]),
    "svl_target_prob_up_f32": (_I, [_P, _I, _I, _I, _I, _I, _I, _I, _P, _P, _P]),
    "svl_ohem_ws_bytes": (_L, [_L]),
    "svl_ohem_threshold_f32": (_I, [_P, _L, _L, _P, _L, _F, _P, _P, _P]),
    "svl_ohem_relabel_i64": (_I, [_P, _P, _L, _P, _P, _P, _P]),
    "svl_maskclip_labels": (_I, [_P, _I, _I, _I, _I, _I, _I, _F, _F, _P, _P, _P]),
    "svl_concept_max_f32": (_I, [_P, _I, _I, _L, _P, _I, _P, _P]),
    "svl_iou_hist_i64": (_I, [_P, _P, _L, _I, _I, _P, _P]),
    "svl_layernorm_fwd": (_I, [_P, _P, _P, _F, _L, _I, _P, _P, _P]),
    "svl_layernorm_fwd_planes": (_I, [_P, _P, _P, _F, _L, _I, _P, _P, _P, _L, _P]),
    "svl_layernorm_fwd_planes_f16x2": (_I, [_P, _P, _P, _F, _L, _I, _P, _P, _P, _L, _P, _P, _P]),
    "svl_layernorm_fwd_pack_f16x2": (_I, [_P, _P, _P, _F, _L, _I, _P, _P, _P, _L, _L, _P, _P, _I, _P, _P]),
    "svl_layernorm_bwd_pack_f16x2": (_I, [_P, _P, _P, _P, _L, _I, _P, _P, _P, _L, _L, _P, _P, _P, _P]),
    "svl_layernorm_bwd_parts": (_I, [_L]),
    "svl_layernorm_bwd": (_I, [_P, _P, _P, _P, _L, _I, _P, _P, _P, _P, _P]),
    "svl_softmax_rows_fwd": (_I, [_P, _L, _I, _L, _F, _P]),
    "svl_softmax_rows_bwd": (_I, [_P, _P, _L, _I, _L, _F, _P]),
    "svl_l2norm_fwd": (_I, [_P, _L, _I, _F, _P, _P, _P]),
    "svl_l2norm_bwd": (_I, [_P, _P, _P, _L, _I, _P, _P]),
    "svl_colsum_ws_floats": (_L, [_L, _I]),
    "svl_colsum_f32": (_I, [_P, _L, _I, _L, _P, _I, _P, _P]),
    "svl_eltwise_f32": (_I, [_I, _P, _P, _P, _L, _P]),
    "svl_chanmask_f32": (_I, [_P, _P, _F, _L, _I, _I, _P, _P]),
    "svl_fill_f32": (_I, [_P, _F, _L, _P]),
    "svl_affine_planes_f32": (_I, [_P, _L, _I, _L, _P, _P, _P]),
    "svl_permute_rows_f32": (_I, [_P, _L, _I, _I, _I, _P, _P]),
    "svl_permute4_f32": (_I, [_P, _P, _L, _L, _L, _L, _L, _L, _L, _L, _P]),
    "svl_bound2_f32": (_I, [_P, _L, _P, _L, _P, _P]),
    "svl_copy2d_f32": (_I, [_P, _L, _L, _L, _P, _L, _L, _L, _L, _I, _I, _P]),
    "svl_groupnorm_fwd": (_I, [_P, _L, _P, _P, _F, _I, _L, _I, _I, _I, _P, _L, _P, _P]),
    "svl_conv3x3_gn_ws_doubles": (_L, [_I, _I, _I, _I]),
    "svl_conv3x3_gn_f32": (_I, [_P, _L, _I, _P, _L, _I, _I, _P, _I, _I, _I, _I, _P, _L, _F, _P, _P, _P, _P, _P]),
    "svl_conv3x3_weight_planes_bytes": (_L, [_I, _I]),
    "svl_conv3x3_weight_planes": (_I, [_P, _I, _I, _P, _P]),
    "svl_groupnorm_scale_shift": (_I, [_P, _P, _P, _I, _I, _I, _P, _P]),
    "svl_groupnorm_apply": (_I, [_P, _L, _P, _P, _I, _L, _I, _I, _I, _P, _P, _L, _P]),
    "svl_groupnorm_bwd": (_I, [_P, _L, _P, _L, _P, _L, _P, _P, _P, _I, _L, _I, _I, _I, _P, _L, _P, _P]),
    "svl_conv3x3_gnb_ws_doubles": (_L, [_I, _I, _I, _I]),
    "svl_conv3x3_dgrad_gnb_f32": (_I, [_P, _L, _I, _P, _I, _I, _I, _I, _P, _L, _I, _P, _P, _P, _P, _P, _P, _P]),
    "svl_groupnorm_bwd_apply": (_I, [_P, _L, _P, _L, _P, _P, _P, _I, _L, _I, _I, _I, _P, _P, _L, _P]),
    "svl_bn_ws_doubles": (_L, [_L, _I]),
    "svl_bn_stats": (_I, [_P, _L, _L, _I, _P, _P, _P]),
    "svl_bn_finalize": (_I, [_P, _D, _F, _F, _P, _P, _I, _P, _P, _P]),
    "svl_bn_eval_invstd": (_I, [_P, _F, _I, _P, _P]),
    "svl_bn_apply": (_I, [_P, _L, _L, _I, _P, _P, _P, _P, _P, _L, _I, _P, _L, _P]),
    "svl_bn_bwd_reduce": (_I, [_P, _L, _P, _L, _P, _L, _P, _P, _P, _P, _L, _I, _P, _P, _P]),
    "svl_bn_bwd_apply": (_I, [_P, _L, _P, _L, _P, _L, _P, _P, _P, _P, _P, _D, _L, _I, _P, _L, _P, _L, _P]),
    "svl_maxpool3x3s2_fwd": (_I, [_P, _I, _I, _I, _I, _P, _P, _P]),
    "svl_maxpool3x3s2_bwd": (_I, [_P, _P, _I, _I, _I, _I, _P, _P]),
    "svl_aug_resample_u8": (_I, [_P, _I, _I, _I, _I, _I, _I, _I, _I, _I, _I, _I, _I, _P, _P]),
    "svl_aug_to_float": (_I, [_P, _I, C.POINTER(C.c_float), C.POINTER(C.c_float), _P, _P]),
    "svl_aug_mask_i64": (_I, [_P, _I, _I, _I, _P, _P]),
    "svl_aug_photometric_u8": (_I, [_P, _I, _I, _F, _P, _P]),
    "svl_aug_gaussian_blur_u8": (_I, [_P, _I, _I, _F, _P, _P, _P]),
    "svl_attention_fwd": (_I, [_P, _I, _I, _I, _P, _P, _P, _L, _P]),
    "svl_attention_bwd": (_I, [_P, _P, _P, _P, _I, _I, _I, _P, _P, _P, _L, _P]),
    "svl_attention_h2_ws_bytes": (_L, [_I, _I, _I, _I]),
    "svl_attention_fwd_h2": (_I, [_P, _I, _I, _I, _P, _P, _P, _L, _P, _L, _P]),
    "svl_attention_bwd_h2": (_I, [_P, _P, _P, _P, _I, _I, _I, _P, _P, _P, _L, _P, _L, _P]),
    "svl_conv_cout1_fwd": (_I, [_P, _L, _I, _I, _I, _I, _I, _I, _I, _I, _P, _P, _P, _P, _P]),
    "svl_conv_cout1_wgrad_blocks": (_I, [_I, _I, _I]),
    "svl_conv_cout1_wgrad": (_I, [_P, _P, _L, _I, _I, _I, _I, _I, _I, _P, _P, _P]),
    "svl_tap_gather": (_I, [_P, _I, _I, _I, _I, _I, _I, _I, _I, _P, _P]),
    "svl_seqattn_fwd": (_I, [C.POINTER(SeqAttnDesc), _P]),
    "svl_seqattn_bwd": (_I, [C.POINTER(SeqAttnDesc), _P]),
    "svl_bilinear_nhwc_fwd": (_I, [_P, _L, _I, _I, _I, _I, _I, _I, _I, _I, _P, _L, _I, _P]),
    "svl_sum_rep_f32": (_I, [_P, _L, _L, _I, _L, _I, _P, _P]),
    "svl_bilinear_nhwc_bwd": (_I, [_P, _L, _I, _I, _I, _I, _I, _I, _I, _I, _P, _L, _I, _P]),
    "svl_bilinear_planes_fwd": (_I, [_P, _L, _I, _I, _I, _I, _I, _P, _P]),
    "svl_bilinear_planes_bwd": (_I, [_P, _L, _I, _I, _I, _I, _I, _P, _P]),
    "svl_avgpool_cat_fwd": (_I, [_P, _I, _I, _I, _I, _I, _I, _P, _I, _I, _P, _P]),
    "svl_avgpool_cat_bwd": (_I, [_P, _I, _I, _I, _I, _I, _I, _I, _P, _I, _P]),
    "svl_avgpool_cat_bwd_text": (_I, [_P, _I, _L, _I, _I, _I, _P, _P, _P]),
    "svl_gap_tokens_fwd": (_I, [_P, _L, _I, _L, _I, _P, _L, _P]),
    "svl_gap_tokens_bwd": (_I, [_P, _L, _I, _L, _I, _P, _L, _I, _P]),
    "svl_bcast_rows_fwd": (_I, [_P, _L, _I, _L, _I, _P, _L, _I, _P]),
    "svl_bcast_rows_bwd": (_I, [_P, _L, _I, _I, _L, _I, _P, _L, _P]),
    "svl_adamw_step": (_I, [_P, _P, _P, _P, _P, _P, _P, _I, _L, _F, _F, _F, _I, _F, _P, _F, _P]),
    "svl_sgd_step": (_I, [_P, _P, _P, _P, _P, _P, _I, _L, _F, _F, _I, _I, _F, _P, _F, _P]),
}

_lib = None


def build_library(force=False):
    if os.path.exists(LIB_PATH) and not force:
        srcs = [os.path.join(CSRC, f) for f in os.listdir(CSRC) if f.endswith((".hip", ".h"))]
        srcs.append(os.path.join(_HERE, "..", "include", "semivl_hip.h"))
        if all(os.path.getmtime(s) <= os.path.getmtime(LIB_PATH) for s in srcs):
            return LIB_PATH
    subprocess.run(["make", "-C", CSRC, "-j8"], check=True, stdout=subprocess.DEVNULL)
    return LIB_PATH


def load():
    global _lib
    if _lib is not None:
        return _lib
    if not os.path.exists(LIB_PATH):
        raise RuntimeError(
            f"semivl_amd: {LIB_PATH} is missing. Build it with `python -c 'import __graft_entry__ as g; g.build()'` "
            "or `make -C semivl_amd/csrc`. There is no fallback path.")
    lib = C.CDLL(LIB_PATH)
    for name, (res, args) in SIGNATURES.items():
        fn = getattr(lib, name)
        fn.restype = res
        fn.argtypes = args
    _lib = lib
    return lib


def last_error():
    buf = C.create_string_buffer(512)
    load().svl_last_error(buf, 512)
    return buf.value.decode()


def check(rc, what=""):
    if rc != 0:
        raise RuntimeError(f"semivl_hip {what} failed (status {rc}): {last_error()}")
```

### semivl_amd/model/vit.py

```python
import math

import torch
import torch.nn as nn
import torch.nn.functional as F

from .. import gradsync, ops


class _MHAParams(nn.Module):
    def __init__(self, dims):
        super().__init__()
        self.in_proj_weight = nn.Parameter(torch.empty(3 * dims, dims))
        self.in_proj_bias = nn.Parameter(torch.zeros(3 * dims))
        self.out_proj = nn.Linear(dims, dims)
        nn.init.xavier_uniform_(self.in_proj_weight)
        nn.init.constant_(self.out_proj.bias, 0.)


class _AttnParams(nn.Module):
    def __init__(self, dims):
        super().__init__()
        self.attn = _MHAParams(dims)


class _FFNParams(nn.Module):
    def __init__(self, dims, hidden):
        super().__init__()
        self.layers = nn.Sequential(nn.Sequential(nn.Linear(dims, hidden), nn.Identity(), nn.Identity()),
                                    nn.Linear(hidden, dims), nn.Identity())


class TransformerEncoderLayer(nn.Module):

    def __init__(self, embed_dims, num_heads, feedforward_channels, eps=1e-5):
        super().__init__()
        self.embed_dims, self.num_heads, self.eps = embed_dims, num_heads, eps
        self.ln1 = nn.LayerNorm(embed_dims, eps=eps)
        self.attn = _AttnParams(embed_dims)
        self.ln2 = nn.LayerNorm(embed_dims, eps=eps)
        self.ffn = _FFNParams(embed_dims, feedforward_channels)

    def plist(self):
        a, f = self.attn.attn, self.ffn.layers
        return dict(ln1w=self.ln1.weight, ln1b=self.ln1.bias, win=a.in_proj_weight, bin=a.in_proj_bias,
                    wout=a.out_proj.weight, bout=a.out_proj.bias, ln2w=self.ln2.weight, ln2b=self.ln2.bias,
                    w1=f[0][0].weight, b1=f[0][0].bias, w2=f[1].weight, b2=f[1].bias)


class _PatchEmbedParams(nn.Module):
    def __init__(self, cin, dims, patch, bias):
        super().__init__()
        self.projection = nn.Conv2d(cin, dims, patch, stride=patch, bias=bias)


def sink_grad(param, grad_fn, shape=None):
    mg = getattr(param, "main_grad", None)
    if mg is not None:
        grad_fn(mg, True)
        return None
    out = ops.empty(*param.shape, device=param.device)
    grad_fn(out, False)
    return out


def block_forward(x, p, heads, eps, Bn, T, want_v, skip_x, save):
    E = x.shape[1]
    D = E // heads
    pp = ops.planes_eligible(x.shape[0], E, E)
    if pp:
        y1, st1, y1a = ops.layernorm_fwd(x, p["ln1w"], p["ln1b"], eps, planes=True, want_y=save is not None)
    else:
        y1, st1 = ops.layernorm_fwd(x, p["ln1w"], p["ln1b"], eps)
        y1a = y1
    if skip_x:
        vproj = ops.linear(y1a, p["win"][2 * E:], p["bin"][2 * E:])
        qkv = None
    else:
        qkv = ops.linear(y1a, p["win"], p["bin"])
        vproj = qkv[:, 2 * E:]
    v = None
    if save is not None:
        save.update(x=x, y1=y1, st1=st1, qkv=qkv, vproj=vproj, want_v=want_v, skip_x=skip_x, eps=eps,
                    y1_amax=y1a.amax if pp else None)

    def ffn(pre, want_pre):
        if pp:
            _, st2_, y2a = ops.layernorm_fwd(pre, p["ln2w"], p["ln2b"], eps, planes=True, want_y=False)
        else:
            y2a, st2_ = ops.layernorm_fwd(pre, p["ln2w"], p["ln2b"], eps)
        h_pre_ = ops.empty(pre.shape[0], p["w1"].shape[0], device=x.device) if want_pre else None
        h_ = ops.linear(y2a, p["w1"], p["b1"], act=ops.ACT_GELU, preact=h_pre_, planes_only=True)
        return ops.linear(h_, p["w2"], p["b2"], resid=pre), st2_, h_pre_

    if want_v:
        vo = ops.linear(ops.split_planes(vproj) if pp else vproj, p["wout"], p["bout"], resid=x)
        v, st2v, hv_pre = ffn(vo, save is not None)
        if save is not None:
            save.update(vo=vo, st2v=st2v, hv_pre=hv_pre)
    xo = None
    if not skip_x:
        o_p = None
        if D == 64 and pp and ops.attention_planes_ok():
            o, P, o_p = ops.attention_fwd(qkv, Bn, T, heads, want_lse=save is not None, planes=True, want_out=save is not None)
        elif D == 64:
            o, P = ops.attention_fwd(qkv, Bn, T, heads, want_lse=save is not None)
        else:
            o, P = ops.vit_attention_fwd(qkv, Bn, T, heads, D)
        x2 = ops.linear(o_p if o_p is not None else (ops.split_planes(o) if pp else o), p["wout"], p["bout"], resid=x)
        xo, st2, h_pre = ffn(x2, save is not None)
        if save is not None:
            save.update(o=o, P=P, x2=x2, st2=st2, h_pre=h_pre)
    return xo, v


FFN_LN_KEYS = ("ln1w", "ln1b", "ln2w", "ln2b", "w1", "b1", "w2", "b2")


def block_backward(dxo, dv, p, s, heads, Bn, T, want=frozenset(), dxo_p=None):
    x, y1 = s["x"], s["y1"]
    E = x.shape[1]
    D = E // heads
    pp = ops.planes_eligible(x.shape[0], E, E)
    g = {}
    dx_res = None
    dqkv = dqkv_p = dqkv_amax = None
    wout_parts = []
    need_h = "w1" in want or "b1" in want

    def ffn_ln_bwd(dout, dout_p, pre_ln_in, st2, h_pre):
        a_ = dout_p if dout_p is not None else dout
        dhp = ops.matmul_nn(a_, p["w2"], dact=ops.ACT_MUL_DGELU, z=h_pre, planes_only=not need_h)
        dy2 = ops.matmul_nn(dhp, p["w1"])
        if "w2" in want:
            g.setdefault("w2", []).append(("gelu", dout, h_pre))
        if "b2" in want:
            g.setdefault("b2", []).append(("sum", dout))
        if "w1" in want:
            g.setdefault("w1", []).append(("ln", dhp, pre_ln_in, st2))
        if "b1" in want:
            g.setdefault("b1", []).append(("sum", dhp))
        if "ln2w" in want or "ln2b" in want:
            r_ = ops.layernorm_bwd(dy2, pre_ln_in, st2, p["ln2w"], dx_add=dout, want_wgrad=True, planes=pp)
            g.setdefault("ln2w", []).append(("add", r_[1]))
            g.setdefault("ln2b", []).append(("add", r_[2]))
            return r_[0], (r_[3] if pp else None)
        if pp:
            return ops.layernorm_bwd(dy2, pre_ln_in, st2, p["ln2w"], dx_add=dout, planes=True)
        return ops.layernorm_bwd(dy2, pre_ln_in, st2, p["ln2w"], dx_add=dout), None

    if not s["skip_x"] and dxo is not None:
        dx2, dx2p = ffn_ln_bwd(dxo, dxo_p, s["x2"], s["st2"], s["h_pre"])
        do = ops.matmul_nn(dx2p if dx2p is not None else dx2, p["wout"])
        wout_parts.append((dx2, s["o"]))
        if D == 64 and pp and ops.attention_planes_ok() and not (s["want_v"] and dv is not None):
            dqkv, dqkv_p = ops.attention_bwd(do, s["qkv"], s["o"], s["P"], Bn, T, heads, planes=True)
            dqkv_amax = dqkv_p.amax
        elif D == 64:
            dqkv = ops.attention_bwd(do, s["qkv"], s["o"], s["P"], Bn, T, heads)
        else:
            dqkv = ops.vit_attention_bwd(do, s["qkv"], s["P"], Bn, T, heads, D)
        dx_res = dx2
    dvproj = None
    if s["want_v"] and dv is not None:
        dvo, dvop = ffn_ln_bwd(dv, None, s["vo"], s["st2v"], s["hv_pre"])
        dvproj = ops.matmul_nn(dvop if dvop is not None else dvo, p["wout"])
        wout_parts.append((dvo, s["vproj"]))
        dx_res = dvo if dx_res is None else ops.add(dx_res, dvo)
    if dqkv is not None and dvproj is not None:
        rows = dqkv.shape[0]
        ops.copy2d(dvproj, 0, rows, 0, E, dqkv, 2 * E, rows, 0, 3 * E, rows, E, accumulate=True)
        dvproj = dqkv_amax = None
    g["wout_parts"] = wout_parts
    if dqkv is not None:
        g["in_full"] = (dqkv, y1, dqkv_amax, s.get("y1_amax"))
        dy1 = ops.matmul_nn(dqkv_p if dqkv_p is not None else dqkv, p["win"])
    elif dvproj is not None:
        g["in_v"] = (dvproj, y1)
        dy1 = ops.matmul_nn(dvproj, p["win"][2 * E:])
    else:
        return dx_res, None, g
    if "ln1w" in want or "ln1b" in want:
        r_ = ops.layernorm_bwd(dy1, x, s["st1"], p["ln1w"], dx_add=dx_res, want_wgrad=True, planes=pp)
        g["ln1w"], g["ln1b"] = [("add", r_[1])], [("add", r_[2])]
        return r_[0], (r_[3] if pp else None), g
    if pp:
        dx_in, dx_in_p = ops.layernorm_bwd(dy1, x, s["st1"], p["ln1w"], dx_add=dx_res, planes=True)
        return dx_in, dx_in_p, g
    return ops.layernorm_bwd(dy1, x, s["st1"], p["ln1w"], dx_add=dx_res), None, g


def ffn_ln_wgrads(p, g):
    out = {}
    for key, parts in g.items():
        if key not in FFN_LN_KEYS:
            continue

        def fn(dst, acc, parts=parts):
            for j, part in enumerate(parts):
                a_ = acc or j > 0
                if part[0] == "gelu":
                    ops.matmul_tn_gelu(part[1], part[2], out=dst, accumulate=a_)
                elif part[0] == "ln":
                    ops.matmul_tn_ln(part[1], part[2], part[3], p["ln2w"], p["ln2b"], out=dst, accumulate=a_)
                elif part[0] == "sum":
                    ops.colsum(part[1], out=dst, accumulate=a_)
                elif a_:
                    ops.add(dst, part[1], out=dst)
                else:
                    ops.eltwise(4, part[1], None, out=dst)
        out[key] = sink_grad(p[key], fn)
    return out


def attn_wgrads(p_mod, g, E):
    a = p_mod.attn.attn
    out = {}

    def wout_fn(dst, acc):
        first = not acc
        for dy, xin in g["wout_parts"]:
            ops.matmul_tn(dy, xin, out=dst, accumulate=not first)
            first = False

    def bout_fn(dst, acc):
        first = not acc
        for dy, _ in g["wout_parts"]:
            ops.colsum(dy, out=dst, accumulate=not first)
            first = False

    if g["wout_parts"]:
        out["wout"] = sink_grad(a.out_proj.weight, wout_fn)
        out["bout"] = sink_grad(a.out_proj.bias, bout_fn)
    else:
        out["wout"] = out["bout"] = None
    if "in_full" in g:
        dqkv, y1, dq_amax, y1_amax = g["in_full"]
        out["win"] = sink_grad(a.in_proj_weight, lambda dst, acc: ops.matmul_tn(dqkv, y1, out=dst, accumulate=acc,
                                                                                a_amax=dq_amax, b_amax=y1_amax))
        out["bin"] = sink_grad(a.in_proj_bias, lambda dst, acc: ops.colsum(dqkv, out=dst, accumulate=acc))
    elif "in_v" in g:
        dvp, y1 = g["in_v"]

        def win_fn(dst, acc):
            if not acc:
                ops.fill(dst, 0.0)
            ops.matmul_tn(dvp, y1, out=dst[2 * E:], accumulate=acc)

        def bin_fn(dst, acc):
            if not acc:
                ops.fill(dst, 0.0)
            ops.colsum(dvp, out=dst[2 * E:], accumulate=acc)

        out["win"] = sink_grad(a.in_proj_weight, win_fn)
        out["bin"] = sink_grad(a.in_proj_bias, bin_fn)
    else:
        out["win"] = out["bin"] = None
    return out


class MaskClipVisionTransformer(nn.Module):
    def __init__(self, img_size=224, patch_size=16, patch_bias=True, in_channels=3, embed_dims=768, num_layers=12,
                 num_heads=12, mlp_ratio=4, out_indices=-1, qkv_bias=True, drop_rate=0., attn_drop_rate=0.,
                 drop_path_rate=0., with_cls_token=True, output_cls_token=False, norm_cfg=dict(type='LN'),
                 act_cfg=dict(type='GELU'), patch_norm=False, pre_norm=False, final_norm=False, return_qkv=False,
                 return_clip_embed=False, skip_last_attn=False, interpolate_mode='bicubic', num_fcs=2,
                 norm_eval=False, with_cp=False, pretrained=None, num_prompt_tokens=None, lora_layers=[], lora_r=4,
                 lora_scaling=1, lora_dropout=0, lora_targets='qkvo', init_cfg=None, type=None,
                 allow_random_init=False):
        super().__init__()
        if isinstance(img_size, int):
            img_size = (img_size, img_size)
        unsupported = dict(patch_bias=patch_bias, drop_rate=drop_rate, attn_drop_rate=attn_drop_rate,
                           drop_path_rate=drop_path_rate, patch_norm=patch_norm, skip_last_attn=skip_last_attn,
                           output_cls_token=output_cls_token, num_prompt_tokens=num_prompt_tokens,
                           lora_layers=list(lora_layers))
        bad = {k: v for k, v in unsupported.items() if v not in (False, 0, 0.0, None, [])}
        if bad or not (pre_norm and final_norm and return_clip_embed and with_cls_token and qkv_bias):
            raise NotImplementedError(f"MaskClipVisionTransformer (HIP): only the SemiVL hot-path configuration is "
                                      f"implemented (off-path options: {bad})")
        assert act_cfg.get("type") == "GELU" and norm_cfg.get("type") == "LN" and interpolate_mode == "bicubic"
        self.img_size, self.patch_size = tuple(img_size), patch_size
        self.embed_dims, self.num_layers, self.num_heads = embed_dims, num_layers, num_heads
        self.eps = norm_cfg.get("eps", 1e-5)
        self.pretrained = pretrained
        self.allow_random_init = allow_random_init
        self.patch_embed = _PatchEmbedParams(in_channels, embed_dims, patch_size, False)
        npatch = (img_size[0] // patch_size) * (img_size[1] // patch_size)
        self.cls_token = nn.Parameter(torch.zeros(1, 1, embed_dims))
        self.pos_embed = nn.Parameter(torch.zeros(1, npatch + 1, embed_dims))
        if out_indices is None:
            self.out_indices = [num_layers]
        elif isinstance(out_indices, int):
            self.out_indices = [num_layers - 1 if out_indices == -1 else out_indices]
        else:
            self.out_indices = list(out_indices)
        self.layers = nn.ModuleList([TransformerEncoderLayer(embed_dims, num_heads, mlp_ratio * embed_dims, self.eps)
                                     for _ in range(num_layers)])
        self.ln0 = nn.LayerNorm(embed_dims, eps=self.eps)
        self.ln1 = nn.LayerNorm(embed_dims, eps=self.eps)
        self.proj = nn.Conv2d(embed_dims, 512, 1, bias=False)
        self.return_qkv = [False] * num_layers
        rq = return_qkv if isinstance(return_qkv, (list, tuple)) else [return_qkv] * len(self.out_indices)
        for j, o in enumerate(self.out_indices):
            if o < num_layers:
                self.return_qkv[o] = bool(rq[j])
        self.return_qkv[num_layers - 1] = True
        for o in self.out_indices:
            if o < num_layers and not self.return_qkv[o]:
                raise NotImplementedError("out_indices without return_qkv is off the SemiVL path")
        self.init_weights()

# ... 314 lines not shown
```

### semivl_amd/ops.py

```python
import collections
import ctypes as C
import os
import math
import weakref

import torch

from . import lib as L

A_KC, A_MC, A_CONV, A_PATCH = 0, 1, 2, 3
B_KC, B_NC, B_CONVW = 0, 1, 2
B_NC_GELU, B_NC_LN, B_PATCHT = 3, 4, 5
ACT_NONE, ACT_GELU, ACT_RELU, ACT_MUL_DGELU, ACT_MUL_DRELU = 0, 1, 2, 3, 4
OUT_STRIDED, OUT_CONVT2X, OUT_PATCH = 0, 1, 2


def _st():
    return C.c_void_p(torch.cuda.current_stream().cuda_stream)


PROFILE = None
PROFILE_SCOPE = None


# ... 661 lines not shown
                "svl_layernorm_fwd")
        return (y if want_y else None), stats, split_planes(y, want_amax=True)
    pl = Planes(rows, Cc, device=x.device, fmt="b3")
    L.check(L.load().svl_layernorm_fwd_planes(_p(x), _p(gamma), _p(beta), float(eps), rows, Cc, None, _p(stats),
                                              _p(pl.buf), pl.prow, _st()), "svl_layernorm_fwd_planes")
    return None, stats, pl


def layernorm_bwd(dy, x, stats, gamma, dx_add=None, want_wgrad=False, planes=False):
    rows, Cc = x.shape
    dx = torch.empty_like(x)
    lib = L.load()
    if planes and not want_wgrad and PLANES_FMT == "h2" and ONEPASS and Cc == 768:
        pl = Planes(rows, Cc, device=x.device, fmt="h2")
        pl.rnorm = torch.empty(pl.prow, dtype=torch.float32, device=x.device)
        L.check(lib.svl_layernorm_bwd_pack_f16x2(_p(dy), _p(x), _p(stats), _p(gamma), rows, Cc, _p(dx_add), _p(dx), _p(pl.buf),
                                                 pl.prow, 0, _p(pl.sexp), _p(pl.rnorm), None, _st()),
                "svl_layernorm_bwd_pack_f16x2")
        return dx, pl
    dgp = dbp = None
    if want_wgrad:
        nparts = lib.svl_layernorm_bwd_parts(rows)
        dgp = empty(nparts, Cc, device=x.device)
        dbp = empty(nparts, Cc, device=x.device)
    L.check(lib.svl_layernorm_bwd(_p(dy), _p(x), _p(stats), _p(gamma), rows, Cc, _p(dx_add), _p(dx), _p(dgp), _p(dbp),
                                  _st()), "svl_layernorm_bwd")
    res = (dx, colsum(dgp), colsum(dbp)) if want_wgrad else (dx,)
    if planes:
        res = res + (split_planes(dx),)
    return res if len(res) > 1 else res[0]


def softmax_rows_fwd(s, rows, cols, ld, scale):
    L.check(L.load().svl_softmax_rows_fwd(_p(s), rows, cols, ld, float(scale), _st()), "svl_softmax_rows_fwd")


def softmax_rows_bwd(dp, p, rows, cols, ld, scale):
    L.check(L.load().svl_softmax_rows_bwd(_p(dp), _p(p), rows, cols, ld, float(scale), _st()), "svl_softmax_rows_bwd")


def l2norm_fwd(x, eps=0.0):
    rows, Cc = x.shape
    y = torch.empty_like(x)
    inv = empty(rows, device=x.device)
    L.check(L.load().svl_l2norm_fwd(_p(x), rows, Cc, float(eps), _p(y), _p(inv), _st()), "svl_l2norm_fwd")
    return y, inv


def l2norm_bwd(dy, y, inv):
    rows, Cc = y.shape
    dx = torch.empty_like(y)
    L.check(L.load().svl_l2norm_bwd(_p(dy), _p(y), _p(inv), rows, Cc, _p(dx), _st()), "svl_l2norm_bwd")
    return dx


def groupnorm_fwd(x, ldx, gamma, beta, eps, imgs, HW, Cc, G, relu, y, ldy):
    stats = empty(imgs, G, 2, device=x.device)
    L.check(L.load().svl_groupnorm_fwd(_p(x), ldx, _p(gamma), _p(beta), float(eps), imgs, HW, Cc, G, 1 if relu else 0,
                                       _p(y), ldy, _p(stats), _st()), "svl_groupnorm_fwd")
    return stats


UP_LOSS = not os.environ.get("SVL_NO_UP_LOSS")
GN_DEFER = True


def groupnorm_scale_shift(stats, gamma, beta, imgs, Cc, G):
    t = empty(imgs, 2, Cc, device=stats.device)
    L.check(L.load().svl_groupnorm_scale_shift(_p(stats), _p(gamma), _p(beta), imgs, Cc, G, _p(t), _st()),
            "svl_groupnorm_scale_shift")
    return t


def conv3x3_gn(x, ldx, imgs, H, W, C1, wf, Co, eps, src2=None, ld2=0, C2=0, rep=1, gn_in=None):
    if not (CONV_TILED and Co % 16 == 0):
        return None
    lib = L.load()
    ws = torch.empty(max(1, lib.svl_conv3x3_gn_ws_doubles(imgs, H, W, Co)), dtype=torch.float64, device=x.device)
    pre = empty(imgs * H * W, Co, device=x.device)
    stats = empty(imgs, Co // 16, 2, device=x.device)
    e0 = _prof_begin()
    rc = lib.svl_conv3x3_gn_f32(_p(x), ldx, C1, _p(src2), ld2, C2, rep, _p(wf), imgs, H, W, Co, _p(pre), Co, float(eps),
                                _p(ws), _p(stats), _p(gn_in), _p(w_planes_of(wf)), _st())
    if rc == -3:
        return None
    L.check(rc, "svl_conv3x3_gn_f32")
    if e0 is not None:
        x6 = get_gemm_emulation() == 6 and not os.environ.get("SVL_CONV_TILED_NO_EMU")
        K = 9 * (C1 + C2)
        _prof_end("gemm_bf16x" if x6 else "gemm", e0, 2.0 * imgs * H * W * Co * K, (A_CONV, B_KC, imgs * H * W, Co, K, 1))
    return pre, stats


def groupnorm_apply(x, ldx, gamma, beta, imgs, HW, Cc, G, relu, stats, y, ldy):
    L.check(L.load().svl_groupnorm_apply(_p(x), ldx, _p(gamma), _p(beta), imgs, HW, Cc, G, 1 if relu else 0, _p(stats),
                                         _p(y), ldy, _st()), "svl_groupnorm_apply")
    return y


def groupnorm_bwd(dy, lddy, x, ldx, y, ldy, stats, gamma, imgs, HW, Cc, G, relu, dx, lddx, beta=None):
    cs = empty(imgs, 2, Cc, device=x.device)
    L.check(L.load().svl_groupnorm_bwd(_p(dy), lddy, _p(x), ldx, _p(None if beta is not None else y), ldy, _p(stats),
                                       _p(gamma), _p(beta), imgs, HW, Cc, G, 1 if relu else 0, _p(dx), lddx, _p(cs),
                                       _st()), "svl_groupnorm_bwd")
    flat = cs.view(imgs, 2 * Cc)
    dbeta = colsum(flat, C_=Cc, ld=2 * Cc)
    dgamma = colsum(flat[:, Cc:], C_=Cc, ld=2 * Cc)
    return dgamma, dbeta


GN_BWD_FUSED = True


def conv3x3_dgrad_gnb(dy, lddy, imgs, H, W, Co, wd, Ci, gn_x, gn_stats, gn_gamma, gn_beta, G):
    if not (GN_BWD_FUSED and CONV_TILED and Ci % 16 == 0 and G * 16 == Ci and dy.is_cuda and get_gemm_emulation() == 6):
        return None
    lib = L.load()
    table = groupnorm_scale_shift(gn_stats, gn_gamma, gn_beta, imgs, Ci, G)
    ws = torch.empty(max(1, lib.svl_conv3x3_gnb_ws_doubles(imgs, H, W, Ci)), dtype=torch.float64, device=dy.device)
    dx = empty(imgs * H * W, Ci, device=dy.device)
    cs = empty(imgs, 2, Ci, device=dy.device)
    e0 = _prof_begin()
    rc = lib.svl_conv3x3_dgrad_gnb_f32(_p(dy), lddy, Co, _p(wd), imgs, H, W, Ci, _p(dx), Ci, 0, _p(gn_x), _p(table), _p(gn_stats),
                                       _p(ws), _p(cs), _p(w_planes_of(wd)), _st())
    if rc == -3:
        return None
    L.check(rc, "svl_conv3x3_dgrad_gnb_f32")
    _prof_end("gemm_bf16x", e0, 2.0 * imgs * H * W * Ci * 9 * Co, (A_CONV, B_KC, imgs * H * W, Ci, 9 * Co, 1))
    return dx, cs


def groupnorm_bwd_from_sums(dy, lddy, x, ldx, stats, gamma, beta, imgs, HW, Cc, G, relu, cs, dx, lddx):
    L.check(L.load().svl_groupnorm_bwd_apply(_p(dy), lddy, _p(x), ldx, _p(stats), _p(gamma), _p(beta), imgs, HW, Cc, G,
                                             1 if relu else 0, _p(cs), _p(dx), lddx, _st()), "svl_groupnorm_bwd_apply")
    flat = cs.view(imgs, 2 * Cc)
    dbeta = colsum(flat, C_=Cc, ld=2 * Cc)
    dgamma = colsum(flat[:, Cc:], C_=Cc, ld=2 * Cc)
    return dgamma, dbeta


def attention_h2():
    return get_gemm_emulation() == 6 and not os.environ.get("SVL_ATTN_NO_EMU")


def _attn_family():
    return "attention_bf16x" if (PROFILE is not None and attention_h2()) else "attention"


def attention_planes_ok():
    return attention_h2() and PLANES_PATH


def _attn_ws(Bn, T, H, backward, dev):
    n = L.load().svl_attention_h2_ws_bytes(Bn, T, H, 1 if backward else 0)
    return torch.empty(n + 1024, dtype=torch.uint8, device=dev), n


def _ws_ptr(ws):
    return (ws.data_ptr() + 1023) // 1024 * 1024


def attention_fwd(qkv, Bn, T, H, want_lse=True, planes=False, want_out=True):
    E = H * 64
    if planes and not attention_planes_ok():
        raise RuntimeError("attention_fwd: planes outputs need emulation mode 6 (attention_planes_ok())")
    out = empty(Bn * T, E, device=qkv.device)
    lse = empty(Bn * H * T, device=qkv.device) if want_lse else None
    e0 = _prof_begin()
    if attention_h2():
        ws, n = _attn_ws(Bn, T, H, False, qkv.device)
        L.check(L.load().svl_attention_fwd_h2(_p(qkv), Bn, T, H, _p(out), _p(lse), None, 0, _ws_ptr(ws), n, _st()),
                "svl_attention_fwd_h2")
    else:
        L.check(L.load().svl_attention_fwd(_p(qkv), Bn, T, H, _p(out), _p(lse), None, 0, _st()), "svl_attention_fwd")
    _prof_end(_attn_family(), e0, 4.0 * Bn * H * T * T * 64, ("fwd_h2" if attention_h2() else "fwd", Bn, T, H))
    if not planes:
        return out, lse
    op = split_planes(out)
    return (out if want_out else None), lse, op


def attention_bwd(dout, qkv, out, lse, Bn, T, H, planes=False):
    if planes and not attention_planes_ok():
        raise RuntimeError("attention_bwd: planes outputs need emulation mode 6 (attention_planes_ok())")
    dqkv = torch.empty_like(qkv)
    ws = empty(Bn * H * T, device=qkv.device)
    e0 = _prof_begin()
    if attention_h2():
        wsb, n = _attn_ws(Bn, T, H, True, qkv.device)
        L.check(L.load().svl_attention_bwd_h2(_p(qkv), _p(out), _p(dout), _p(lse), Bn, T, H, _p(ws), _p(dqkv), None, 0,
                                              _ws_ptr(wsb), n, _st()), "svl_attention_bwd_h2")
    else:
        L.check(L.load().svl_attention_bwd(_p(qkv), _p(out), _p(dout), _p(lse), Bn, T, H, _p(ws), _p(dqkv), None, 0, _st()),
                "svl_attention_bwd")
    _prof_end(_attn_family(), e0, 14.0 * Bn * H * T * T * 64, ("bwd_h2" if attention_h2() else "bwd", Bn, T, H))
    return (dqkv, split_planes(dqkv, want_amax=True)) if planes else dqkv


def vit_attention_fwd(qkv, Bn, T, H, D):
    E = H * D
    Tp = (T + 3) // 4 * 4
    dev = qkv.device
    P = empty(Bn * H, T, Tp, device=dev)
    gemm(A_KC, B_KC, T, T, D, Op(qkv, 3 * E, 0, T * 3 * E, D), Op(qkv, 3 * E, E, T * 3 * E, D), P, ldc_m=Tp,
         batch=Bn * H, batch_inner=H, c_bso=H * T * Tp, c_bsi=T * Tp)
    softmax_rows_fwd(P, Bn * H * T, T, Tp, 1.0 / math.sqrt(D))
    out = empty(Bn * T, E, device=dev)
    gemm(A_KC, B_NC, T, D, T, Op(P, Tp, 0, H * T * Tp, T * Tp), Op(qkv, 3 * E, 2 * E, T * 3 * E, D), out, ldc_m=E,
         batch=Bn * H, batch_inner=H, c_bso=T * E, c_bsi=D)
    return out, P


def vit_attention_bwd(dout, qkv, P, Bn, T, H, D):
    E = H * D
    Tp = P.shape[2]
    dev = qkv.device
    dqkv = empty(Bn * T, 3 * E, device=dev)
    bh = dict(batch=Bn * H, batch_inner=H)
    p_op = Op(P, Tp, 0, H * T * Tp, T * Tp)
    do_op = Op(dout, E, 0, T * E, D)
    gemm(A_MC, B_NC, T, D, T, p_op, do_op, dqkv, c_off=2 * E, ldc_m=3 * E, c_bso=T * 3 * E, c_bsi=D, **bh)
    dP = empty(Bn * H, T, Tp, device=dev)
    gemm(A_KC, B_KC, T, T, D, do_op, Op(qkv, 3 * E, 2 * E, T * 3 * E, D), dP, ldc_m=Tp, c_bso=H * T * Tp,
         c_bsi=T * Tp, **bh)
    softmax_rows_bwd(dP, P, Bn * H * T, T, Tp, 1.0 / math.sqrt(D))
    ds_op = Op(dP, Tp, 0, H * T * Tp, T * Tp)
    gemm(A_KC, B_NC, T, D, T, ds_op, Op(qkv, 3 * E, E, T * 3 * E, D), dqkv, c_off=0, ldc_m=3 * E, c_bso=T * 3 * E,
         c_bsi=D, **bh)
    gemm(A_MC, B_NC, T, D, T, ds_op, Op(qkv, 3 * E, 0, T * 3 * E, D), dqkv, c_off=E, ldc_m=3 * E, c_bso=T * 3 * E,
         c_bsi=D, **bh)
    return dqkv


def permute_rows(x, outer, A, Bd, Cc):
    out = empty(outer * A * Bd, Cc, device=x.device)
    L.check(L.load().svl_permute_rows_f32(_p(x), outer, A, Bd, Cc, _p(out), _st()), "svl_permute_rows_f32")
    return out


SEQATTN_MFMA_MIN = int(os.environ.get("SVL_SEQATTN_MFMA_MIN", "64"))


def seqattn_fwd(qkv, groups, inner, seq, heads, outer_stride, inner_stride, seq_stride):
    rows, E3 = qkv.shape
    E = E3 // 3
    out = empty(rows, E, device=qkv.device)
    probs = empty(groups, heads, seq, seq, device=qkv.device)
    d = L.SeqAttnDesc(groups, inner, seq, heads, outer_stride, inner_stride, seq_stride, _p(qkv), _p(out), _p(probs),
                      None, None, None)
    L.check(L.load().svl_seqattn_fwd(C.byref(d), _st()), "svl_seqattn_fwd")
    return out, probs


def seqattn_bwd(dout, qkv, probs, groups, inner, seq, heads, outer_stride, inner_stride, seq_stride):
    dqkv = torch.empty_like(qkv)
    ds = torch.empty_like(probs)
    d = L.SeqAttnDesc(groups, inner, seq, heads, outer_stride, inner_stride, seq_stride, _p(qkv), None, _p(probs),
                      _p(dout), _p(dqkv), _p(ds))
    L.check(L.load().svl_seqattn_bwd(C.byref(d), _st()), "svl_seqattn_bwd")
    return dqkv


_PACKS = {}


def cached_pack(W, tag, fn):
    base = W._base if W._base is not None else W
    if not isinstance(base, torch.nn.Parameter):
        return fn(W.detach())
    key = (W.data_ptr(), tuple(W.shape), tag)
    ver = (base._version, WEIGHT_EPOCH if base.requires_grad else 0)
    hit = _PACKS.get(key)
    if hit is not None and hit[0] == ver and hit[2]() is base:
        return hit[1].get()
    out = fn(W.detach())
    if len(_PACKS) > 4096:
        _PACKS.clear()
    _PACKS[key] = (ver, StreamCached(out), weakref.ref(base))
    return out


def conv3x3_weight_planes(pack, N, Ct):
    if not (pack.is_cuda and N in (32, 64, 128) and Ct % 16 == 0):
        return None
    lib = L.load()
    pl = torch.empty(lib.svl_conv3x3_weight_planes_bytes(N, Ct), dtype=torch.uint8, device=pack.device)
    L.check(lib.svl_conv3x3_weight_planes(_p(pack), N, Ct, _p(pl), _st()), "svl_conv3x3_weight_planes")
    return pl


def w_planes_of(pack):
    return getattr(pack, "_svl_planes", None)


def pack_conv_w(W):
    def build(w):
        Co, Ci, kh, kw = w.shape
        w = w.contiguous()
        cs = (Ci * kh * kw, kh * kw, kw, 1)
        wf = permute4(w, (Co, kh, kw, Ci), (cs[0], cs[2], cs[3], cs[1])).view(Co, kh * kw * Ci)
        wd = permute4(w, (Ci, kh, kw, Co), (cs[1], cs[2], cs[3], cs[0])).view(Ci, kh * kw * Co)
        out = [wf, wd]
        if kh == 3 and kw == 3:
            for pk, n, ct in ((wf, Co, Ci), (wd, Ci, Co)):
                pl = conv3x3_weight_planes(pk, n, ct)
                if pl is not None:
                    pk._svl_planes = pl
                    out.append(pl)
        return tuple(out)
    r = cached_pack(W, "conv", build)
    return r[0], r[1]


def unpack_conv_wgrad(dwf, Co, Ci, kh, kw):
    return permute4(dwf, (Co, Ci, kh, kw), (kh * kw * Ci, 1, kw * Ci, Ci))


CONV_TILED = not os.environ.get("SVL_CONV_NO_TILED")


def conv_out_size(H, W, KH, KW, dil, pad, stride):
    return (H + 2 * pad - dil * (KH - 1) - 1) // stride + 1, (W + 2 * pad - dil * (KW - 1) - 1) // stride + 1


def conv_fwd(x, ldx, imgs, H, W, C1, wf, Co, KH, KW, dil, pad, bias=None, act=ACT_NONE, out=None, ldo=None, src2=None,
             ld2=0, C2=0, rep=1, resid=None, ldr=None, stride=1):
    Ho, Wo = conv_out_size(H, W, KH, KW, dil, pad, stride) if stride != 1 else (H, W)
    M = imgs * Ho * Wo
    K = KH * KW * (C1 + C2)
    if out is None:
        out = empty(M, Co, device=x.device)
        ldo = Co
    g = conv_geom(H, W, C1, KH, KW, dil, pad, 1, C2, rep, src2, ld2, stride=stride, Ho=Ho, Wo=Wo)
    gemm(A_CONV, B_KC, M, Co, K, Op(x, ldx), Op(wf, K), out, ldc_m=ldo, bias=bias, act=act, conv=g, resid=resid,
         ldr_m=ldr, w_planes=w_planes_of(wf) if (KH, KW, pad, stride) == (3, 3, dil, 1) else None, emu_h2=EMU_H2_CONVFWD)
    return out


def conv_dgrad(dy, lddy, imgs, H, W, Co, wd, Ci, KH, KW, dil, pad, out=None, ldo=None, accumulate=False):
    M = imgs * H * W
    K = KH * KW * Co
    if out is None:
# ... 537 lines not shown
```

Before: 104.9 images/s.

## Use ds_read_tr16 transposed LDS reads and reuse forward K/V packs in attention backward

Adds a row-major-only mode for the fp16x2 fused attention. The transposed copies of V, K, Q and dO are no longer packed; the B operands are instead produced with ds_read_tr16_b64 transposing LDS reads, which shrinks the staged LDS per pipeline stage and the global-to-LDS traffic. The forward workspace (packed K/V plus exponent and norm sets) is kept alive and passed to a new backward entry point, so backward skips repacking. The cost is keeping the forward workspace in memory until backward, plus a swizzle scheme that adds complexity and bank-conflict risk.

```diff
diff --git a/include/semivl_hip.h b/include/semivl_hip.h
--- a/include/semivl_hip.h
+++ b/include/semivl_hip.h
@@ -304,6 +304,10 @@
 int svl_attention_bwd(const float* qkv, const float* out, const float* dout, const float* lse, int B, int T, int H,
                       float* dsum_ws, float* dqkv, void* dqkv_planes, int64_t planes_rows, svl_stream_t stream);
 int64_t svl_attention_h2_ws_bytes(int B, int T, int H, int backward);
+int svl_attention_h2_tr_sets(int on);
+int svl_attention_bwd_h2_sets(const float* qkv, const float* out, const float* dout, const float* lse, int B, int T, int H,
+                              float* dsum_ws, float* dqkv, const void* sets, int64_t sets_bytes, void* ws, int64_t ws_bytes,
+                              svl_stream_t stream);
 int svl_attention_fwd_h2(const float* qkv, int B, int T, int H, float* out, float* lse, void* out_planes,
                          int64_t planes_rows, void* ws, int64_t ws_bytes, svl_stream_t stream);
 int svl_attention_bwd_h2(const float* qkv, const float* out, const float* dout, const float* lse, int B, int T, int H,
diff --git a/semivl_amd/csrc/attention.hip b/semivl_amd/csrc/attention.hip
--- a/semivl_amd/csrc/attention.hip
+++ b/semivl_amd/csrc/attention.hip
@@ -584,9 +584,11 @@
 }
 
 extern "C" int64_t svl_attention_h2_ws_bytes(int B, int T, int H, int backward) {
-  if (B <= 0 || T <= 0 || H <= 0) return 0;
-  return svl_attn_h2::ws_bytes(B, T, H, backward);
-}
+  if (B <= 0 || T <= 0 || H <= 0 || backward < 0 || backward > 2) return 0;
+  return svl_attn_h2::ws_bytes(B, T, H, backward, svl_attn_h2::tr_sets(-1));
+}
+
+extern "C" int svl_attention_h2_tr_sets(int on) { return svl_attn_h2::tr_sets(on); }
 
 extern "C" int svl_attention_fwd_h2(const float* qkv, int B, int T, int H, float* out, float* lse, void* out_planes,
                                     int64_t planes_rows, void* ws, int64_t ws_bytes, svl_stream_t stream) {
@@ -602,35 +604,37 @@
   hipStream_t st = (hipStream_t)stream;
   int nb = 0;
   const int r = rows_split(T, &nb, FQ);
-  rc = svl_attn_h2::fwd_pack(p, ws, ws_bytes, st);
+  const int tr = svl_attn_h2::tr_sets(-1);
+  rc = svl_attn_h2::fwd_pack(p, ws, ws_bytes, tr, st);
   if (rc) return rc;
   if (r > 0) {
     hipStream_t aux = nullptr;
     rc = svl_fork(st, &aux);
     if (rc) return rc;
-    rc = svl_attn_h2::fwd_tail(p, nb * FQ, ws, aux);
+    rc = svl_attn_h2::fwd_tail(p, nb * FQ, ws, tr, aux);
     if (rc) return rc;
   }
-  rc = svl_attn_h2::fwd(p, nb, ws, ws_bytes, st);
+  rc = svl_attn_h2::fwd(p, nb, ws, ws_bytes, tr, st);
   if (rc) return rc;
   return r > 0 ? svl_join(st) : SVL_OK;
 }
 
-extern "C" int svl_attention_bwd_h2(const float* qkv, const float* out, const float* dout, const float* lse, int B, int T,
-                                    int H, float* dsum_ws, float* dqkv, void* dq_planes, int64_t planes_rows, void* ws,
-                                    int64_t ws_bytes, svl_stream_t stream) {
-  int rc = check(qkv, B, T, H, "svl_attention_bwd_h2");
-  if (rc) return rc;
-  SVL_CHECK_ARG(out && dout && lse && dsum_ws && dqkv, "svl_attention_bwd_h2: null args");
-  (void)planes_rows;
-  rc = no_planes(dq_planes, "svl_attention_bwd_h2");
+namespace {
+int bwd_h2(const char* who, const float* qkv, const float* out, const float* dout, const float* lse, int B, int T, int H,
+           float* dsum_ws, float* dqkv, void* dq_planes, const void* sets, int64_t sets_bytes, void* ws, int64_t ws_bytes,
+           svl_stream_t stream) {
+  int rc = check(qkv, B, T, H, who);
+  if (rc) return rc;
+  SVL_CHECK_ARG(out && dout && lse && dsum_ws && dqkv, "%s: null args", who);
+  rc = no_planes(dq_planes, who);
   if (rc) return rc;
   hipStream_t st = (hipStream_t)stream;
   AttnP p;
   memset(&p, 0, sizeof(p));
   p.qkv = qkv; p.dout = dout; p.lse = const_cast<float*>(lse); p.dsum = dsum_ws; p.dqkv = dqkv;
   p.B = B; p.T = T; p.H = H; p.E = (long)H * D; p.ld = 3 * p.E; p.scale = 0.125f;
-  rc = svl_attn_h2::bwd_prepare(p, out, dsum_ws, ws, ws_bytes, st);
+  const int tr = svl_attn_h2::tr_sets(-1);
+  rc = svl_attn_h2::bwd_prepare(p, out, dsum_ws, ws, ws_bytes, sets, sets_bytes, tr, st);
   if (rc) return rc;
   int nb = 0;
   const int r = rows_split(T, &nb, FQ);
@@ -638,10 +642,26 @@
     hipStream_t aux = nullptr;
     rc = svl_fork(st, &aux);
     if (rc) return rc;
-    rc = svl_attn_h2::bwd_tail(p, nb * FQ, ws, aux);
+    rc = svl_attn_h2::bwd_tail(p, nb * FQ, ws, sets, tr, aux);
     if (rc) return rc;
   }
-  rc = svl_attn_h2::bwd_main(p, nb, ws, st);
+  rc = svl_attn_h2::bwd_main(p, nb, ws, sets, tr, st);
   if (rc) return rc;
   return r > 0 ? svl_join(st) : SVL_OK;
 }
+}
+
+extern "C" int svl_attention_bwd_h2(const float* qkv, const float* out, const float* dout, const float* lse, int B, int T,
+                                    int H, float* dsum_ws, float* dqkv, void* dq_planes, int64_t planes_rows, void* ws,
+                                    int64_t ws_bytes, svl_stream_t stream) {
+  (void)planes_rows;
+  return bwd_h2("svl_attention_bwd_h2", qkv, out, dout, lse, B, T, H, dsum_ws, dqkv, dq_planes, nullptr, 0, ws, ws_bytes, stream);
+}
+
+extern "C" int svl_attention_bwd_h2_sets(const float* qkv, const float* out, const float* dout, const float* lse, int B, int T,
+                                         int H, float* dsum_ws, float* dqkv, const void* sets, int64_t sets_bytes, void* ws,
+                                         int64_t ws_bytes, svl_stream_t stream) {
+  SVL_CHECK_ARG(sets, "svl_attention_bwd_h2_sets: sets missing");
+  return bwd_h2("svl_attention_bwd_h2_sets", qkv, out, dout, lse, B, T, H, dsum_ws, dqkv, nullptr, sets, sets_bytes, ws, ws_bytes,
+                stream);
+}
diff --git a/semivl_amd/csrc/attn_h2.h b/semivl_amd/csrc/attn_h2.h
--- a/semivl_amd/csrc/attn_h2.h
+++ b/semivl_amd/csrc/attn_h2.h
@@ -3,12 +3,14 @@
 
 namespace svl_attn_h2 {
 
-long ws_bytes(int B, int T, int H, int backward);
-int fwd(const AttnP& p, int nb, void* ws, long wsb, hipStream_t st);
-int bwd_prepare(const AttnP& p, const float* out, float* dsum_ws, void* ws, long wsb, hipStream_t st);
-int bwd_main(const AttnP& p, int nb, void* ws, hipStream_t st);
-int fwd_pack(const AttnP& p, void* ws, long wsb, hipStream_t st);
-int fwd_tail(const AttnP& p, int row0, void* ws, hipStream_t aux);
-int bwd_tail(const AttnP& p, int row0, void* ws, hipStream_t aux);
+int tr_sets(int on);
+long ws_bytes(int B, int T, int H, int mode, int tr);
+int fwd(const AttnP& p, int nb, void* ws, long wsb, int tr, hipStream_t st);
+int bwd_prepare(const AttnP& p, const float* out, float* dsum_ws, void* ws, long wsb, const void* sets, long setsb, int tr,
+                hipStream_t st);
+int bwd_main(const AttnP& p, int nb, void* ws, const void* sets, int tr, hipStream_t st);
+int fwd_pack(const AttnP& p, void* ws, long wsb, int tr, hipStream_t st);
+int fwd_tail(const AttnP& p, int row0, void* ws, int tr, hipStream_t aux);
+int bwd_tail(const AttnP& p, int row0, void* ws, const void* sets, int tr, hipStream_t aux);
 
 }
diff --git a/semivl_amd/csrc/attn_h2.hip b/semivl_amd/csrc/attn_h2.hip
--- a/semivl_amd/csrc/attn_h2.hip
+++ b/semivl_amd/csrc/attn_h2.hip
@@ -87,6 +87,43 @@
   a[0] = *reinterpret_cast<const f16x8*>(chunk0);
   a[1] = *reinterpret_cast<const f16x8*>(chunk0 + 1024);
 }
+typedef short s16x4 __attribute__((__vector_size__(4 * sizeof(short))));
+typedef short s16x8 __attribute__((__vector_size__(8 * sizeof(short))));
+struct TrLane {
+  unsigned rm[2];
+  unsigned tr[2];
+};
+__device__ __forceinline__ TrLane tr_lane(int lane) {
+  const int hh = lane >> 5, r = lane & 31, g = (lane >> 4) & 1, q = (lane >> 2) & 3, p = lane & 3;
+  TrLane t;
+  t.rm[0] = (unsigned)(hh * 32 + (r ^ (4 * hh))) * 16u;
+  t.rm[1] = (unsigned)(hh * 32 + (r ^ (4 * hh + 8))) * 16u;
+  t.tr[0] = (unsigned)(g * 2048 + ((p & 1) * 32 + ((4 * hh + q) ^ (4 * (p & 1) + 8 * g))) * 16 + (p >> 1) * 8);
+  t.tr[1] = t.tr[0] ^ 128u;
+  return t;
+}
+typedef __attribute__((address_space(3))) char lchar;
+__device__ __forceinline__ const lchar* tr_base(const char* img, unsigned off) {
+  const lchar* b = (const lchar*)(img + off);
+  asm("" : "+v"(b));
+  return b;
+}
+__device__ __forceinline__ f16x8 tr_read8(const lchar* a0, const lchar* a1) {
+  typedef __attribute__((address_space(3))) s16x4 lds4;
+  const s16x4 lo = __builtin_amdgcn_ds_read_tr16_b64_v4i16((lds4*)a0);
+  const s16x4 hi = __builtin_amdgcn_ds_read_tr16_b64_v4i16((lds4*)a1);
+  return __builtin_bit_cast(f16x8, (s16x8)__builtin_shufflevector(lo, hi, 0, 1, 2, 3, 4, 5, 6, 7));
+}
+__device__ __forceinline__ void frag2(f16x8 (&a)[2], const lchar* chunk0) {
+  typedef __attribute__((address_space(3))) f16x8 lds8;
+  a[0] = *reinterpret_cast<const lds8*>(chunk0);
+  a[1] = *reinterpret_cast<const lds8*>(chunk0 + 1024);
+}
+__device__ __forceinline__ void frag2_tr(f16x8 (&a)[2], const lchar* t0, const lchar* t1, int kgl, int rbd) {
+  const int o = kgl * 256 + rbd * 4096;
+  a[0] = tr_read8(t0 + o, t1 + o);
+  a[1] = tr_read8(t0 + o + 1024, t1 + o + 1024);
+}
 __device__ __forceinline__ int ds_exp(float nrm_do, float nrm_v) {
   const float bt = 2.f * nrm_do * nrm_v;
   int g = bt > 0.f ? __builtin_amdgcn_frexp_expf(bt) : 0;
@@ -101,6 +138,8 @@
   int which[4];
   int* exps;
   float* nrm;
+  const int* exps_in;
+  const float* nrm_in;
   int B, T, H, Tp;
 };
 
@@ -191,6 +230,10 @@
     p.exps[z * 4 + w] = e;
     p.nrm[z * 4 + w] = sqrtf(nr);
   }
+  if (p.exps_in && tid < 3) {
+    p.exps[z * 4 + tid] = p.exps_in[z * 4 + tid];
+    p.nrm[z * 4 + tid] = p.nrm_in[z * 4 + tid];
+  }
 }
 
 __global__ __launch_bounds__(256) void attn_ld_kernel(const float* __restrict__ dout, const float* __restrict__ out,
@@ -227,6 +270,7 @@
 template <int V>
 __global__ __launch_bounds__(512) void attn_fwd_h2_kernel(const AttnP p, const H2W w) {
   constexpr bool MIX = (V & 1) != 0;
+  constexpr bool RM = (V & 4) != 0;
   extern __shared__ __attribute__((aligned(1024))) char sm[];
   const int tid = threadIdx.x, lane = tid & 63, l31 = lane & 31, hi = lane >> 5;
   const int wave = __builtin_amdgcn_readfirstlane(tid >> 6);
@@ -240,8 +284,10 @@
   const int nkt = w.Tp >> 6;
   const long rmz = (long)(w.Tp >> 5) * 8192, trz = (long)w.Tp * 256;
   const char* ksrc = w.k_rm + z * rmz;
-  const char* vsrc = w.v_tr + z * trz;
+  const char* vsrc = RM ? w.v_rm + z * rmz : w.v_tr + z * trz;
   const unsigned lane16 = lane * 16;
+  const TrLane tl = tr_lane(lane);
+  const unsigned lane_v = RM ? (wave & 1 ? tl.rm[1] : tl.rm[0]) : lane16;
   const unsigned sm_base = (unsigned)(uintptr_t)(__attribute__((address_space(3))) char*)sm;
   f16x8 qf[2][4];
   {
@@ -257,8 +303,9 @@
     const int tc = min(tile, nkt - 1);
     const char* s = (part ? vsrc : ksrc) + (long)tc * 16384 + wave * 2048;
     const unsigned dst = sm_base + stage * STG_F + part * 16384 + wave * 2048;
-    glds16(s, lane16, dst);
-    glds16(s + 1024, lane16, dst + 1024);
+    const unsigned lo = part ? lane_v : lane16;
+    glds16(s, lo, dst);
+    glds16(s + 1024, lo, dst + 1024);
   };
   f32x16 o0, o1, s0, s1;
 #pragma unroll
@@ -299,6 +346,8 @@
   auto phase2 = [&](int kt, auto last_c) __attribute__((always_inline)) {
     constexpr bool LAST = decltype(last_c)::value;
     const char* Vt = sm + (kt % 3) * STG_F + 16384 + lane16;
+    const lchar* Vt0 = RM ? tr_base(sm + (kt % 3) * STG_F + 16384, tl.tr[0]) : nullptr;
+    const lchar* Vt1 = RM ? tr_base(sm + (kt % 3) * STG_F + 16384, tl.tr[1]) : nullptr;
     if (LAST) {
       const int j0 = kt * 64;
 #pragma unroll
@@ -340,8 +389,13 @@
       }
       f16x8 pb[2], a0[2], a1[2];
       split2x8<MIX>(x, pb);
-      frag2(a0, Vt + ((tp * 2) * 2) * 1024);
-      frag2(a1, Vt + ((tp * 2 + 1) * 2) * 1024);
+      if constexpr (RM) {
+        frag2_tr(a0, Vt0 + (tp >> 1) * 8192, Vt1 + (tp >> 1) * 8192, tp & 1, 0);
+        frag2_tr(a1, Vt0 + (tp >> 1) * 8192, Vt1 + (tp >> 1) * 8192, tp & 1, 1);
+      } else {
+        frag2(a0, Vt + ((tp * 2) * 2) * 1024);
+        frag2(a1, Vt + ((tp * 2 + 1) * 2) * 1024);
+      }
       H2_PAIR(o0, a0, o1, a1, pb)
     }
     l += sum0 + sum1;
@@ -405,10 +459,13 @@
 }
 
 constexpr int STG_Q = 48 * 1024;
+constexpr int STG_Q_RM = 32 * 1024;
 
 template <int V>
 __global__ __launch_bounds__(512) void attn_dq_h2_kernel(const AttnP p, const H2W w) {
   constexpr bool MIX = (V & 1) != 0;
+  constexpr bool RM = (V & 4) != 0;
+  constexpr int STG = RM ? STG_Q_RM : STG_Q, NCH = RM ? 4 : 6;
   extern __shared__ __attribute__((aligned(1024))) char sm[];
   const int tid = threadIdx.x, lane = tid & 63, l31 = lane & 31, hi = lane >> 5;
   const int wave = __builtin_amdgcn_readfirstlane(tid >> 6);
@@ -420,8 +477,9 @@
   const bool wave_active = q0 < p.T;
   const int nkt = w.Tp >> 6;
   const long rmz = (long)(w.Tp >> 5) * 8192, trz = (long)w.Tp * 256;
-  const char* src3[3] = {w.k_rm + z * rmz, w.v_rm + z * rmz, w.k_tr + z * trz};
+  const char* src3[3] = {w.k_rm + z * rmz, w.v_rm + z * rmz, RM ? nullptr : w.k_tr + z * trz};
   const unsigned lane16 = lane * 16;
+  const TrLane tl = tr_lane(lane);
   const unsigned sm_base = (unsigned)(uintptr_t)(__attribute__((address_space(3))) char*)sm;
   f16x8 qf[2][4], of[2][4];
   {
@@ -446,20 +504,25 @@
   auto issue_tile = [&](int tile, int stage) __attribute__((always_inline)) {
     const int tc = min(tile, nkt - 1);
 #pragma unroll
-    for (int i = 0; i < 6; ++i) {
-      const int cidx = wave * 6 + i, part = cidx >> 4, cc = cidx & 15;
+    for (int i = 0; i < NCH; ++i) {
+      const int cidx = wave * NCH + i, part = cidx >> 4, cc = cidx & 15;
       const char* s = (part == 0 ? src3[0] : part == 1 ? src3[1] : src3[2]) + (long)tc * 16384 + cc * 1024;
-      glds16(s, lane16, sm_base + stage * STG_Q + cidx * 1024);
+      const unsigned lo = RM && part == 0 ? tl.rm[(i >> 1) & 1] : lane16;
+      glds16(s, lo, sm_base + stage * STG + cidx * 1024);
     }
   };
   issue_tile(0, 0);
   issue_tile(1, 1);
-  wait_vm<6>();
+  wait_vm<NCH>();
   interval_barrier();
   auto tile = [&](int kt, auto last_c) __attribute__((always_inline)) {
     constexpr bool last = decltype(last_c)::value;
     {
-      const char* Ks = sm + (kt % 3) * STG_Q + lane16;
+      const char* Ki = sm + (kt % 3) * STG;
+      const lchar* Kr[2] = {RM ? tr_base(Ki, tl.rm[0]) : nullptr, RM ? tr_base(Ki, tl.rm[1]) : nullptr};
+      const lchar* Kt0 = RM ? tr_base(Ki, tl.tr[0]) : nullptr;
+      const lchar* Kt1 = RM ? tr_base(Ki, tl.tr[1]) : nullptr;
+      const char* Ks = Ki + lane16;
       const char* Vs = Ks + 16384;
       const char* Kt = Ks + 32768;
 #pragma unroll
@@ -471,7 +534,8 @@
 #pragma unroll
           for (int kg = 0; kg < 4; ++kg) {
             f16x8 ka[2], va[2], bq[2] = {qf[0][kg], qf[1][kg]}, bo[2] = {of[0][kg], of[1][kg]};
-            frag2(ka, Ks + ((jt * 4 + kg) * 2) * 1024);
+            if constexpr (RM) frag2(ka, Kr[kg & 1] + ((jt * 4 + kg) * 2) * 1024);
+            else frag2(ka, Ks + ((jt * 4 + kg) * 2) * 1024);
             frag2(va, Vs + ((jt * 4 + kg) * 2) * 1024);
             H2_2(sa, ka, bq, dp, va, bo)
           }
@@ -488,8 +552,14 @@
               x[j] = __builtin_amdgcn_exp2f(fmaf(sa[8 * t + j], c, a_i)) * fmaf(dp[8 * t + j], cdp, -d_i);
             f16x8 pb[2], a0[2], a1[2];
             split2x8<MIX>(x, pb);
-            frag2(a0, Kt + (((2 * jt + t) * 2) * 2) * 1024);
-            frag2(a1, Kt + (((2 * jt + t) * 2 + 1) * 2) * 1024);
+            if constexpr (RM) {
+              __builtin_amdgcn_sched_barrier(0);
+              frag2_tr(a0, Kt0 + jt * 8192, Kt1 + jt * 8192, t, 0);
+              frag2_tr(a1, Kt0 + jt * 8192, Kt1 + jt * 8192, t, 1);
+            } else {
+              frag2(a0, Kt + (((2 * jt + t) * 2) * 2) * 1024);
+              frag2(a1, Kt + (((2 * jt + t) * 2 + 1) * 2) * 1024);
+            }
             H2_PAIR(dq0, a0, dq1, a1, pb)
           }
         }
@@ -499,7 +569,7 @@
   for (int kt = 0; kt < nkt - 1; ++kt) {
     issue_tile(kt + 2, (kt + 2) % 3);
     if (wave_active) tile(kt, std::false_type{});
-    wait_vm<6>();
+    wait_vm<NCH>();
     interval_barrier();
   }
   if (wave_active) tile(nkt - 1, std::true_type{});
@@ -517,10 +587,13 @@
 }
 
 constexpr int STG_K = 33 * 1024;
+constexpr int STG_K_RM = 17 * 1024;
 
 template <int V>
 __global__ __launch_bounds__(512) void attn_dkv_h2_kernel(const AttnP p, const H2W w) {
   constexpr bool MIX = (V & 1) != 0;
+  constexpr bool RM = (V & 4) != 0;
+  constexpr int STG = RM ? STG_K_RM : STG_K, NCH = RM ? 2 : 4, LDO = RM ? 16384 : 32768;
   extern __shared__ __attribute__((aligned(1024))) char sm[];
   const int tid = threadIdx.x, lane = tid & 63, l31 = lane & 31, hi = lane >> 5;
   const int wave = __builtin_amdgcn_readfirstlane(tid >> 6);
@@ -531,7 +604,8 @@
   const bool wave_active = k0 < p.T;
   const int nqt = (p.T + 31) >> 5;
   const long rmz = (long)(w.Tp >> 5) * 8192, trz = (long)w.Tp * 256;
-  const char* src4[4] = {w.q_rm + z * rmz, w.do_rm + z * rmz, w.q_tr + z * trz, w.do_tr + z * trz};
+  const char* src4[4] = {w.q_rm + z * rmz, w.do_rm + z * rmz, RM ? nullptr : w.q_tr + z * trz, RM ? nullptr : w.do_tr + z * trz};
+  const TrLane tl = tr_lane(lane);
   const char* ldsrc = reinterpret_cast<const char*>(w.ld + (long)z * w.Tp * 2);
   const unsigned lane16 = lane * 16;
   const unsigned sm_base = (unsigned)(uintptr_t)(__attribute__((address_space(3))) char*)sm;
@@ -553,19 +627,20 @@
   f32x16 dv0, dv1, dk0, dk1;
 #pragma unroll
   for (int r = 0; r < 16; ++r) { dv0[r] = 0.f; dv1[r] = 0.f; dk0[r] = 0.f; dk1[r] = 0.f; }
+  const unsigned lane_s = RM ? (wave & 1 ? tl.rm[1] : tl.rm[0]) : lane16;
   auto issue_tile = [&](int tile, int stage) __attribute__((always_inline)) {
     const int tc = min(tile, nqt - 1);
 #pragma unroll
-    for (int i = 0; i < 4; ++i) {
-      const int cidx = wave * 4 + i, part = cidx >> 3, cc = cidx & 7;
+    for (int i = 0; i < NCH; ++i) {
+      const int cidx = wave * NCH + i, part = cidx >> 3, cc = cidx & 7;
       const char* s = (part == 0 ? src4[0] : part == 1 ? src4[1] : part == 2 ? src4[2] : src4[3]) + (long)tc * 8192 + cc * 1024;
-      glds16(s, lane16, sm_base + stage * STG_K + cidx * 1024);
-    }
-    if (wave == 0) glds16(ldsrc + (long)tc * 256, lane16, sm_base + stage * STG_K + 32768);
+      glds16(s, lane_s, sm_base + stage * STG + cidx * 1024);
+    }
+    if (wave == 0) glds16(ldsrc + (long)tc * 256, lane16, sm_base + stage * STG + LDO);
   };
   auto wait_older = [&]() __attribute__((always_inline)) {
-    if (wave == 0) wait_vm<5>();
-    else wait_vm<4>();
+    if (wave == 0) wait_vm<NCH + 1>();
+    else wait_vm<NCH>();
   };
   issue_tile(0, 0);
   issue_tile(1, 1);
@@ -574,19 +649,28 @@
   for (int qt = 0; qt < nqt; ++qt) {
     issue_tile(qt + 2, (qt + 2) % 3);
     if (wave_active) {
-      const char* Qs = sm + (qt % 3) * STG_K + lane16;
+      const char* Qi = sm + (qt % 3) * STG;
+      const lchar* Qr[2] = {RM ? tr_base(Qi, tl.rm[0]) : nullptr, RM ? tr_base(Qi, tl.rm[1]) : nullptr};
+      const lchar* Qt0 = RM ? tr_base(Qi, tl.tr[0]) : nullptr;
+      const lchar* Qt1 = RM ? tr_base(Qi, tl.tr[1]) : nullptr;
+      const char* Qs = Qi + lane16;
       const char* Os = Qs + 8192;
       const char* Qt = Qs + 16384;
       const char* Ot = Qs + 24576;
-      const float* LD = reinterpret_cast<const float*>(sm + (qt % 3) * STG_K + 32768);
+      const float* LD = reinterpret_cast<const float*>(sm + (qt % 3) * STG + LDO);
       f32x16 sa, dp;
 #pragma unroll
       for (int r = 0; r < 16; ++r) { sa[r] = 0.f; dp[r] = 0.f; }
 #pragma unroll
       for (int kg = 0; kg < 4; ++kg) {
         f16x8 qa[2], oa[2], bk[2] = {kf[0][kg], kf[1][kg]}, bv[2] = {vf[0][kg], vf[1][kg]};
-        frag2(qa, Qs + (kg * 2) * 1024);
-        frag2(oa, Os + (kg * 2) * 1024);
+        if constexpr (RM) {
+          frag2(qa, Qr[kg & 1] + (kg * 2) * 1024);
+          frag2(oa, Qr[kg & 1] + 8192 + (kg * 2) * 1024);
+        } else {
+          frag2(qa, Qs + (kg * 2) * 1024);
+          frag2(oa, Os + (kg * 2) * 1024);
+        }
         H2_2T(sa, qa, bk, dp, oa, bv)
       }
 #pragma unroll
@@ -608,11 +692,23 @@
         f16x8 pa[2], sa2[2], o0[2], o1[2], q0f[2], q1f[2];
         split2x8<MIX>(xp, pa);
         split2x8<MIX>(xs, sa2);
-        frag2(o0, Ot + ((t * 2) * 2) * 1024);
-        frag2(o1, Ot + ((t * 2 + 1) * 2) * 1024);
+        if constexpr (RM) __builtin_amdgcn_sched_barrier(0);
+        if constexpr (RM) {
+          frag2_tr(o0, Qt0 + 8192, Qt1 + 8192, t, 0);
+          frag2_tr(o1, Qt0 + 8192, Qt1 + 8192, t, 1);
+        } else {
+          frag2(o0, Ot + ((t * 2) * 2) * 1024);
+          frag2(o1, Ot + ((t * 2 + 1) * 2) * 1024);
+        }
         H2_2(dv0, pa, o0, dv1, pa, o1)
-        frag2(q0f, Qt + ((t * 2) * 2) * 1024);
-        frag2(q1f, Qt + ((t * 2 + 1) * 2) * 1024);
+        if constexpr (RM) __builtin_amdgcn_sched_barrier(0);
+        if constexpr (RM) {
+          frag2_tr(q0f, Qt0, Qt1, t, 0);
+          frag2_tr(q1f, Qt0, Qt1, t, 1);
+        } else {
+          frag2(q0f, Qt + ((t * 2) * 2) * 1024);
+          frag2(q1f, Qt + ((t * 2 + 1) * 2) * 1024);
+        }
         H2_2(dk0, sa2, q0f, dk1, sa2, q1f)
       }
     }
@@ -641,17 +737,28 @@
 }
 
 constexpr int TAILW = 4;
-template <bool MIX>
+__device__ __forceinline__ void tail_stage(const char* blk, const TrLane& tl, unsigned dst) {
+  asm volatile("s_waitcnt lgkmcnt(0)" ::: "memory");
+#pragma unroll
+  for (int c = 0; c < 8; ++c) glds16(blk + c * 1024, tl.rm[(c >> 1) & 1], dst + c * 1024);
+}
+template <bool MIX, bool RM>
 __global__ __launch_bounds__(64 * TAILW) __attribute__((amdgpu_waves_per_eu(4, 4))) void attn_fwd_tail_h2_kernel(const AttnP p, const H2W w, int row0) {
+  __shared__ __attribute__((aligned(1024))) char stg[RM ? TAILW * 8192 : 16];
   const int lane = threadIdx.x & 63, l31 = lane & 31, hi = lane >> 5;
   const int wave = __builtin_amdgcn_readfirstlane(threadIdx.x >> 6);
+  const TrLane tl = tr_lane(lane);
+  const char* stw = stg + (RM ? wave * 8192 : 0);
+  const lchar* st0 = RM ? tr_base(stw, tl.tr[0]) : nullptr;
+  const lchar* st1 = RM ? tr_base(stw, tl.tr[1]) : nullptr;
+  const unsigned stw_a = (unsigned)(uintptr_t)(__attribute__((address_space(3))) char*)stg + (RM ? wave * 8192 : 0);
   const int z = blockIdx.x, b = z / p.H, h = z - b * p.H;
   const int q0 = row0 + 32 * (int)blockIdx.y, qi = q0 + l31;
   const int nkt = w.Tp >> 6;
   const long rmz = (long)(w.Tp >> 5) * 8192, trz = (long)w.Tp * 256;
   const unsigned lane16 = lane * 16;
   const char* ksrc = w.k_rm + z * rmz + lane16;
-  const char* vsrc = w.v_tr + z * trz + lane16;
+  const char* vsrc = RM ? w.v_rm + z * rmz : w.v_tr + z * trz + lane16;
   const char* qs = w.q_rm + z * rmz + (long)(q0 >> 5) * 8192 + lane16;
   const int eq = w.exps[z * 4], ek = w.exps[z * 4 + 1], ev = w.exps[z * 4 + 2];
   const float c = __builtin_amdgcn_ldexpf(LOG2E, eq + ek - 3);
@@ -664,6 +771,7 @@
     const char* Ks = ksrc + (long)kt * 16384;
     const char* Vt = vsrc + (long)kt * 16384;
     const bool last = kt == nkt - 1, half = last && short_last;
+    if constexpr (RM) tail_stage(Vt, tl, stw_a);
     f32x16 s0, s1;
 #pragma unroll
     for (int r = 0; r < 16; ++r) { s0[r] = 0.f; s1[r] = 0.f; }
@@ -717,8 +825,15 @@
       }
       f16x8 pb[2], a0[2], a1[2];
       split2x8<MIX>(x, pb);
-      frag2(a0, Vt + ((tp * 2) * 2) * 1024);
-      frag2(a1, Vt + ((tp * 2 + 1) * 2) * 1024);
+      if constexpr (RM) {
+        if (tp == 2) tail_stage(Vt + 8192, tl, stw_a);
+        if (tp == 0 || tp == 2) wait_vm<0>();
+        frag2_tr(a0, st0, st1, tp & 1, 0);
+        frag2_tr(a1, st0, st1, tp & 1, 1);
+      } else {
+        frag2(a0, Vt + ((tp * 2) * 2) * 1024);
+        frag2(a1, Vt + ((tp * 2 + 1) * 2) * 1024);
+      }
       H2_PAIR(o0, a0, o1, a1, pb)
     }
     l += sum;
@@ -769,10 +884,16 @@
   }
 }
 
-template <bool MIX>
+template <bool MIX, bool RM>
 __global__ __launch_bounds__(64 * TAILW) __attribute__((amdgpu_waves_per_eu(4, 4))) void attn_dq_tail_h2_kernel(const AttnP p, const H2W w, int row0) {
+  __shared__ __attribute__((aligned(1024))) char stg[RM ? TAILW * 8192 : 16];
   const int lane = threadIdx.x & 63, l31 = lane & 31, hi = lane >> 5;
   const int wave = __builtin_amdgcn_readfirstlane(threadIdx.x >> 6);
+  const TrLane tl = tr_lane(lane);
+  const char* stw = stg + (RM ? wave * 8192 : 0);
+  const lchar* st0 = RM ? tr_base(stw, tl.tr[0]) : nullptr;
+  const lchar* st1 = RM ? tr_base(stw, tl.tr[1]) : nullptr;
+  const unsigned stw_a = (unsigned)(uintptr_t)(__attribute__((address_space(3))) char*)stg + (RM ? wave * 8192 : 0);
   const int z = blockIdx.x, b = z / p.H, h = z - b * p.H;
   const int q0 = row0 + 32 * (int)blockIdx.y, qi = q0 + l31;
   const int nkt = w.Tp >> 6;
@@ -780,7 +901,7 @@
   const unsigned lane16 = lane * 16;
   const char* k_rm = w.k_rm + z * rmz + lane16;
   const char* v_rm = w.v_rm + z * rmz + lane16;
-  const char* k_tr = w.k_tr + z * trz + lane16;
+  const char* k_tr = RM ? w.k_rm + z * rmz : w.k_tr + z * trz + lane16;
   const char* qs = w.q_rm + z * rmz + (long)(q0 >> 5) * 8192 + lane16;
   const char* os = w.do_rm + z * rmz + (long)(q0 >> 5) * 8192 + lane16;
   const float2 ad = *reinterpret_cast<const float2*>(w.ld + ((long)z * w.Tp + min(qi, w.Tp - 1)) * 2);
@@ -800,6 +921,7 @@
 #pragma unroll
     for (int jt = 0; jt < 2; ++jt) {
       if (!last || jt == 0 || p.T - kt * 64 > 32) {
+        if constexpr (RM) tail_stage(Kt + jt * 8192, tl, stw_a);
         f32x16 sa, dp;
 #pragma unroll
         for (int r = 0; r < 16; ++r) { sa[r] = 0.f; dp[r] = 0.f; }
@@ -836,8 +958,14 @@
             x[j] = __builtin_amdgcn_exp2f(fmaf(sa[8 * t + j], c, a_i)) * fmaf(dp[8 * t + j], cdp, -d_i);
           f16x8 pb[2], a0[2], a1[2];
           split2x8<MIX>(x, pb);
-          frag2(a0, Kt + (((2 * jt + t) * 2) * 2) * 1024);
-          frag2(a1, Kt + (((2 * jt + t) * 2 + 1) * 2) * 1024);
+          if constexpr (RM) {
+            if (t == 0) wait_vm<0>();
+            frag2_tr(a0, st0, st1, t, 0);
+            frag2_tr(a1, st0, st1, t, 1);
+          } else {
+            frag2(a0, Kt + (((2 * jt + t) * 2) * 2) * 1024);
+            frag2(a1, Kt + (((2 * jt + t) * 2 + 1) * 2) * 1024);
+          }
           H2_PAIR(dq0, a0, dq1, a1, pb)
           __builtin_amdgcn_sched_barrier(0);
         }
@@ -872,10 +1000,16 @@
   }
 }
 
-template <bool MIX>
+template <bool MIX, bool RM>
 __global__ __launch_bounds__(64 * TAILW) __attribute__((amdgpu_waves_per_eu(4, 4))) void attn_dkv_tail_h2_kernel(const AttnP p, const H2W w, int row0) {
+  __shared__ __attribute__((aligned(1024))) char stg[RM ? TAILW * 8192 : 16];
   const int lane = threadIdx.x & 63, l31 = lane & 31, hi = lane >> 5;
   const int wave = __builtin_amdgcn_readfirstlane(threadIdx.x >> 6);
+  const TrLane tl = tr_lane(lane);
+  const char* stw = stg + (RM ? wave * 8192 : 0);
+  const lchar* st0 = RM ? tr_base(stw, tl.tr[0]) : nullptr;
+  const lchar* st1 = RM ? tr_base(stw, tl.tr[1]) : nullptr;
+  const unsigned stw_a = (unsigned)(uintptr_t)(__attribute__((address_space(3))) char*)stg + (RM ? wave * 8192 : 0);
   const int z = blockIdx.x, b = z / p.H, h = z - b * p.H;
   const int k0 = row0 + 32 * (int)blockIdx.y;
   const int nqt = (p.T + 31) >> 5;
@@ -883,8 +1017,8 @@
   const unsigned lane16 = lane * 16;
   const char* q_rm = w.q_rm + z * rmz;
   const char* o_rm = w.do_rm + z * rmz;
-  const char* q_tr = w.q_tr + z * trz;
-  const char* o_tr = w.do_tr + z * trz;
+  const char* q_tr = RM ? nullptr : w.q_tr + z * trz;
+  const char* o_tr = RM ? nullptr : w.do_tr + z * trz;
   const float* ldz = w.ld + (long)z * w.Tp * 2;
   const char* ks = w.k_rm + z * rmz + (long)(k0 >> 5) * 8192;
   const char* vs = w.v_rm + z * rmz + (long)(k0 >> 5) * 8192;
@@ -901,6 +1035,7 @@
     const char* Qt = q_tr + (long)qt * 8192;
     const char* Ot = o_tr + (long)qt * 8192;
     const float* LD = ldz + qt * 64;
+    if constexpr (RM) tail_stage(Os, tl, stw_a);
     f32x16 sa, dp;
 #pragma unroll
     for (int r = 0; r < 16; ++r) { sa[r] = 0.f; dp[r] = 0.f; }
@@ -945,6 +1080,28 @@
       split2x8<MIX>(xs, sa2[t]);
     }
     __builtin_amdgcn_sched_barrier(0);
+    if constexpr (RM) {
+      wait_vm<0>();
+#pragma unroll
+      for (int t = 0; t < 2; ++t) {
+        f16x8 o0[2], o1[2];
+        frag2_tr(o0, st0, st1, t, 0);
+        frag2_tr(o1, st0, st1, t, 1);
+        H2_2(dv0, pa[t], o0, dv1, pa[t], o1)
+        __builtin_amdgcn_sched_barrier(0);
+      }
+      tail_stage(Qs, tl, stw_a);
+      wait_vm<0>();
+#pragma unroll
+      for (int t = 0; t < 2; ++t) {
+        f16x8 q0f[2], q1f[2];
+        frag2_tr(q0f, st0, st1, t, 0);
+        frag2_tr(q1f, st0, st1, t, 1);
+        H2_2(dk0, sa2[t], q0f, dk1, sa2[t], q1f)
+        __builtin_amdgcn_sched_barrier(0);
+      }
+      continue;
+    }
 #pragma unroll
     for (int t = 0; t < 2; ++t) {
       f16x8 o0[2], o1[2], q0f[2], q1f[2];
@@ -996,17 +1153,19 @@
   long exps, nrm, ld, total;
   int Tp;
 };
-Layout layout(int B, int T, int H, int backward) {
+Layout layout(int B, int T, int H, int mode, int tr) {
   Layout l;
   l.Tp = (T + 63) / 64 * 64;
   l.set = (long)B * H * l.Tp * 256;
-  const long nset = backward ? 7 : 3;
+  const long nset = mode == 0 ? 3 : mode == 2 ? 1 : tr ? 7 : 4;
   l.exps = nset * l.set;
   l.nrm = l.exps + (((long)B * H * 16 + 1023) & ~1023L);
   l.ld = l.nrm + (((long)B * H * 16 + 1023) & ~1023L);
-  l.total = l.ld + (backward ? (((long)B * H * l.Tp * 8 + 1023) & ~1023L) + 1024 : 0);
+  l.total = l.ld + (mode ? (((long)B * H * l.Tp * 8 + 1023) & ~1023L) + 1024 : 0);
   return l;
 }
+
+std::atomic<int> g_tr{-1};
 
 template <typename K>
 int set_lds(K kernel, std::atomic<uint64_t>& mask, int bytes) {
@@ -1019,20 +1178,31 @@
   return SVL_OK;
 }
 
-H2W views(const Layout& l, char* ws, int backward) {
+H2W views(const Layout& l, char* ws, int mode, int tr, const char* sets = nullptr) {
   H2W w;
   memset(&w, 0, sizeof(w));
   w.Tp = l.Tp;
-  w.q_rm = ws;
-  w.k_rm = ws + l.set;
-  if (backward) {
-    w.v_rm = ws + 2 * l.set;
-    w.do_rm = ws + 3 * l.set;
-    w.q_tr = ws + 4 * l.set;
-    w.k_tr = ws + 5 * l.set;
-    w.do_tr = ws + 6 * l.set;
+  if (mode == 2) {
+    w.q_rm = sets;
+    w.k_rm = sets + l.set;
+    w.v_rm = sets + 2 * l.set;
+    w.do_rm = ws;
   } else {
-    w.v_tr = ws + 2 * l.set;
+    w.q_rm = ws;
+    w.k_rm = ws + l.set;
+    if (mode == 1) {
+      w.v_rm = ws + 2 * l.set;
+      w.do_rm = ws + 3 * l.set;
+      if (tr) {
+        w.q_tr = ws + 4 * l.set;
+        w.k_tr = ws + 5 * l.set;
+        w.do_tr = ws + 6 * l.set;
+      }
+    } else if (tr) {
+      w.v_tr = ws + 2 * l.set;
+    } else {
+      w.v_rm = ws + 2 * l.set;
+    }
   }
   w.exps = reinterpret_cast<const int*>(ws + l.exps);
   w.nrm = reinterpret_cast<const float*>(ws + l.nrm);
@@ -1040,8 +1210,8 @@
   return w;
 }
 
-int check_ws(const AttnP& p, const void* ws, long wsb, int backward, const char* who) {
-  const Layout l = layout(p.B, p.T, p.H, backward);
+int check_ws(const AttnP& p, const void* ws, long wsb, int mode, int tr, const char* who) {
+  const Layout l = layout(p.B, p.T, p.H, mode, tr);
   SVL_CHECK_ARG(ws && ((uintptr_t)ws & 1023) == 0 && wsb >= l.total, "%s: workspace of %ld bytes (1 KiB aligned) needed, got %ld",
                 who, l.total, wsb);
   return SVL_OK;
@@ -1051,14 +1221,26 @@
 
 namespace svl_attn_h2 {
 
-long ws_bytes(int B, int T, int H, int backward) { return layout(B, T, H, backward).total; }
-
-int fwd_pack(const AttnP& p, void* ws_, long wsb, hipStream_t st) {
-  int rc = check_ws(p, ws_, wsb, 0, "svl_attention_fwd_h2");
+int tr_sets(int on) {
+  int cur = g_tr.load(std::memory_order_acquire);
+  if (cur < 0) {
+    const char* e = getenv("SVL_ATTN_TR_SETS");
+    int expect = -1;
+    g_tr.compare_exchange_strong(expect, e && *e && *e != '0' ? 1 : 0);
+    cur = g_tr.load(std::memory_order_acquire);
+  }
+  if (on >= 0) g_tr.store(on ? 1 : 0, std::memory_order_release);
+  return cur;
+}
+
+long ws_bytes(int B, int T, int H, int mode, int tr) { return layout(B, T, H, mode, tr).total; }
+
+int fwd_pack(const AttnP& p, void* ws_, long wsb, int tr, hipStream_t st) {
+  int rc = check_ws(p, ws_, wsb, 0, tr, "svl_attention_fwd_h2");
   if (rc) return rc;
-  const Layout l = layout(p.B, p.T, p.H, 0);
+  const Layout l = layout(p.B, p.T, p.H, 0, tr);
   char* ws = static_cast<char*>(ws_);
-  const H2W w = views(l, ws, 0);
+  const H2W w = views(l, ws, 0, tr);
   PackP q;
   memset(&q, 0, sizeof(q));
   for (int i = 0; i < 3; ++i) {
@@ -1068,6 +1250,7 @@
   }
   q.rm[0] = const_cast<char*>(w.q_rm);
   q.rm[1] = const_cast<char*>(w.k_rm);
+  q.rm[2] = const_cast<char*>(w.v_rm);
   q.tr[2] = const_cast<char*>(w.v_tr);
   q.exps = const_cast<int*>(w.exps);
   q.nrm = const_cast<float*>(w.nrm);
@@ -1077,30 +1260,42 @@
   return SVL_OK;
 }
 
-#define SVL_LAUNCH_V(KERN, LDS)                                       \
-    rc = set_lds(KERN<3>, mask, LDS);                                   \
+#define SVL_LAUNCH_V(KERN, VV, LDS)                                   \
+    rc = set_lds(KERN<VV>, mask, LDS);                                  \
     if (rc) return rc;                                                  \
-    hipLaunchKernelGGL(KERN<3>, grid, dim3(512), LDS, st, p, w);
-
-int fwd(const AttnP& p, int nb, void* ws_, long wsb, hipStream_t st) {
+    hipLaunchKernelGGL(KERN<VV>, grid, dim3(512), LDS, st, p, w);
+
+int fwd(const AttnP& p, int nb, void* ws_, long wsb, int tr, hipStream_t st) {
   (void)wsb;
   if (nb <= 0) return SVL_OK;
-  const Layout l = layout(p.B, p.T, p.H, 0);
-  const H2W w = views(l, static_cast<char*>(ws_), 0);
+  const Layout l = layout(p.B, p.T, p.H, 0, tr);
+  const H2W w = views(l, static_cast<char*>(ws_), 0, tr);
   int rc = SVL_OK;
-  static std::atomic<uint64_t> mask;
   const dim3 grid(nb * p.B * p.H);
-  SVL_LAUNCH_V(attn_fwd_h2_kernel, 3 * STG_F)
+  if (tr) {
+    static std::atomic<uint64_t> mask;
+    SVL_LAUNCH_V(attn_fwd_h2_kernel, 3, 3 * STG_F)
+  } else {
+    static std::atomic<uint64_t> mask;
+    SVL_LAUNCH_V(attn_fwd_h2_kernel, 7, 3 * STG_F)
+  }
   SVL_LAUNCH_CHECK("svl_attention_fwd_h2");
   return SVL_OK;
 }
 
-int bwd_prepare(const AttnP& p, const float* out, float* dsum_ws, void* ws_, long wsb, hipStream_t st) {
-  int rc = check_ws(p, ws_, wsb, 1, "svl_attention_bwd_h2");
+int bwd_prepare(const AttnP& p, const float* out, float* dsum_ws, void* ws_, long wsb, const void* sets, long setsb, int tr,
+                hipStream_t st) {
+  const int mode = sets ? 2 : 1;
+  int rc = check_ws(p, ws_, wsb, mode, tr, "svl_attention_bwd_h2");
   if (rc) return rc;
-  const Layout l = layout(p.B, p.T, p.H, 1);
+  if (sets) {
+    SVL_CHECK_ARG(!tr, "svl_attention_bwd_h2_sets: kept sets are row-major sets only (the tr switch is on)");
+    rc = check_ws(p, sets, setsb, 0, 0, "svl_attention_bwd_h2_sets (sets)");
+    if (rc) return rc;
+  }
+  const Layout l = layout(p.B, p.T, p.H, mode, tr);
   char* ws = static_cast<char*>(ws_);
-  const H2W w = views(l, ws, 1);
+  const H2W w = views(l, ws, mode, tr, static_cast<const char*>(sets));
   PackP q;
   memset(&q, 0, sizeof(q));
   for (int i = 0; i < 3; ++i) {
@@ -1109,18 +1304,25 @@
   }
   q.src[3] = p.dout;
   q.ld[3] = p.E;
-  for (int i = 0; i < 4; ++i) q.which[i] = i;
-  q.rm[0] = const_cast<char*>(w.q_rm);
-  q.rm[1] = const_cast<char*>(w.k_rm);
-  q.rm[2] = const_cast<char*>(w.v_rm);
   q.rm[3] = const_cast<char*>(w.do_rm);
-  q.tr[0] = const_cast<char*>(w.q_tr);
-  q.tr[1] = const_cast<char*>(w.k_tr);
   q.tr[3] = const_cast<char*>(w.do_tr);
+  if (sets) {
+    const Layout lf = layout(p.B, p.T, p.H, 0, 0);
+    q.which[0] = 3;
+    q.exps_in = reinterpret_cast<const int*>(static_cast<const char*>(sets) + lf.exps);
+    q.nrm_in = reinterpret_cast<const float*>(static_cast<const char*>(sets) + lf.nrm);
+  } else {
+    for (int i = 0; i < 4; ++i) q.which[i] = i;
+    q.rm[0] = const_cast<char*>(w.q_rm);
+    q.rm[1] = const_cast<char*>(w.k_rm);
+    q.rm[2] = const_cast<char*>(w.v_rm);
+    q.tr[0] = const_cast<char*>(w.q_tr);
+    q.tr[1] = const_cast<char*>(w.k_tr);
+  }
   q.exps = const_cast<int*>(w.exps);
   q.nrm = const_cast<float*>(w.nrm);
   q.B = p.B; q.T = p.T; q.H = p.H; q.Tp = l.Tp;
-  hipLaunchKernelGGL(attn_pack_kernel, dim3(p.B * p.H, 4), dim3(256), 0, st, q);
+  hipLaunchKernelGGL(attn_pack_kernel, dim3(p.B * p.H, sets ? 1 : 4), dim3(256), 0, st, q);
   SVL_LAUNCH_CHECK("svl_attention_bwd_h2/pack");
   const long groups = (long)p.B * p.H * l.Tp;
   hipLaunchKernelGGL(attn_ld_kernel, dim3((unsigned)((groups * 16 + 255) / 256)), dim3(256), 0, st, p.dout, out, p.lse, w.nrm,
@@ -1129,41 +1331,55 @@
   return SVL_OK;
 }
 
-int fwd_tail(const AttnP& p, int row0, void* ws_, hipStream_t aux) {
-  const Layout l = layout(p.B, p.T, p.H, 0);
-  const H2W w = views(l, static_cast<char*>(ws_), 0);
+int fwd_tail(const AttnP& p, int row0, void* ws_, int tr, hipStream_t aux) {
+  const Layout l = layout(p.B, p.T, p.H, 0, tr);
+  const H2W w = views(l, static_cast<char*>(ws_), 0, tr);
   const dim3 grid(p.B * p.H, (p.T - row0 + 31) / 32);
-  hipLaunchKernelGGL(attn_fwd_tail_h2_kernel<true>, grid, dim3(64 * TAILW), 0, aux, p, w, row0);
+  if (tr) hipLaunchKernelGGL((attn_fwd_tail_h2_kernel<true, false>), grid, dim3(64 * TAILW), 0, aux, p, w, row0);
+  else hipLaunchKernelGGL((attn_fwd_tail_h2_kernel<true, true>), grid, dim3(64 * TAILW), 0, aux, p, w, row0);
   SVL_LAUNCH_CHECK("svl_attention_fwd_h2/tail");
   return SVL_OK;
 }
 
-int bwd_tail(const AttnP& p, int row0, void* ws_, hipStream_t aux) {
-  const Layout l = layout(p.B, p.T, p.H, 1);
-  const H2W w = views(l, static_cast<char*>(ws_), 1);
+int bwd_tail(const AttnP& p, int row0, void* ws_, const void* sets, int tr, hipStream_t aux) {
+  const int mode = sets ? 2 : 1;
+  const Layout l = layout(p.B, p.T, p.H, mode, tr);
+  const H2W w = views(l, static_cast<char*>(ws_), mode, tr, static_cast<const char*>(sets));
   const dim3 grid(p.B * p.H, (p.T - row0 + 31) / 32);
-  hipLaunchKernelGGL(attn_dkv_tail_h2_kernel<true>, grid, dim3(64 * TAILW), 0, aux, p, w, row0);
-  hipLaunchKernelGGL(attn_dq_tail_h2_kernel<true>, grid, dim3(64 * TAILW), 0, aux, p, w, row0);
+  if (tr) {
+    hipLaunchKernelGGL((attn_dkv_tail_h2_kernel<true, false>), grid, dim3(64 * TAILW), 0, aux, p, w, row0);
+    hipLaunchKernelGGL((attn_dq_tail_h2_kernel<true, false>), grid, dim3(64 * TAILW), 0, aux, p, w, row0);
+  } else {
+    hipLaunchKernelGGL((attn_dkv_tail_h2_kernel<true, true>), grid, dim3(64 * TAILW), 0, aux, p, w, row0);
+    hipLaunchKernelGGL((attn_dq_tail_h2_kernel<true, true>), grid, dim3(64 * TAILW), 0, aux, p, w, row0);
+  }
   SVL_LAUNCH_CHECK("svl_attention_bwd_h2/tail");
   return SVL_OK;
 }
 
-int bwd_main(const AttnP& p, int nb, void* ws_, hipStream_t st) {
+int bwd_main(const AttnP& p, int nb, void* ws_, const void* sets, int tr, hipStream_t st) {
   if (nb <= 0) return SVL_OK;
-  const Layout l = layout(p.B, p.T, p.H, 1);
-  const H2W w = views(l, static_cast<char*>(ws_), 1);
+  const int mode = sets ? 2 : 1;
+  const Layout l = layout(p.B, p.T, p.H, mode, tr);
+  const H2W w = views(l, static_cast<char*>(ws_), mode, tr, static_cast<const char*>(sets));
   int rc = SVL_OK;
   const dim3 grid(nb * p.B * p.H);
-  {
+  if (tr) {
     static std::atomic<uint64_t> mask;
-    SVL_LAUNCH_V(attn_dkv_h2_kernel, 3 * STG_K)
-    SVL_LAUNCH_CHECK("svl_attention_bwd_h2/dkv");
-  }
-  {
+    SVL_LAUNCH_V(attn_dkv_h2_kernel, 3, 3 * STG_K)
+  } else {
     static std::atomic<uint64_t> mask;
-    SVL_LAUNCH_V(attn_dq_h2_kernel, 3 * STG_Q)
-    SVL_LAUNCH_CHECK("svl_attention_bwd_h2/dq");
-  }
+    SVL_LAUNCH_V(attn_dkv_h2_kernel, 7, 3 * STG_K_RM)
+  }
+  SVL_LAUNCH_CHECK("svl_attention_bwd_h2/dkv");
+  if (tr) {
+    static std::atomic<uint64_t> mask;
+    SVL_LAUNCH_V(attn_dq_h2_kernel, 3, 3 * STG_Q)
+  } else {
+    static std::atomic<uint64_t> mask;
+    SVL_LAUNCH_V(attn_dq_h2_kernel, 7, 3 * STG_Q_RM)
+  }
+  SVL_LAUNCH_CHECK("svl_attention_bwd_h2/dq");
   return SVL_OK;
 }
 
diff --git a/semivl_amd/lib.py b/semivl_amd/lib.py
--- a/semivl_amd/lib.py
+++ b/semivl_amd/lib.py
@@ -171,6 +171,8 @@
     "svl_attention_h2_ws_bytes": (_L, [_I, _I, _I, _I]),
     "svl_attention_fwd_h2": (_I, [_P, _I, _I, _I, _P, _P, _P, _L, _P, _L, _P]),
     "svl_attention_bwd_h2": (_I, [_P, _P, _P, _P, _I, _I, _I, _P, _P, _P, _L, _P, _L, _P]),
+    "svl_attention_h2_tr_sets": (_I, [_I]),
+    "svl_attention_bwd_h2_sets": (_I, [_P, _P, _P, _P, _I, _I, _I, _P, _P, _P, _L, _P, _L, _P]),
     "svl_conv_cout1_fwd": (_I, [_P, _L, _I, _I, _I, _I, _I, _I, _I, _I, _P, _P, _P, _P, _P]),
     "svl_conv_cout1_wgrad_blocks": (_I, [_I, _I, _I]),
     "svl_conv_cout1_wgrad": (_I, [_P, _P, _L, _I, _I, _I, _I, _I, _I, _P, _P, _P]),
diff --git a/semivl_amd/model/vit.py b/semivl_amd/model/vit.py
--- a/semivl_amd/model/vit.py
+++ b/semivl_amd/model/vit.py
@@ -101,15 +101,17 @@
     if not skip_x:
         o_p = None
         if D == 64 and pp and ops.attention_planes_ok():
-            o, P, o_p = ops.attention_fwd(qkv, Bn, T, heads, want_lse=save is not None, planes=True, want_out=save is not None)
+            o, P, o_p, *sets = ops.attention_fwd(qkv, Bn, T, heads, want_lse=save is not None, planes=True,
+                                                 want_out=save is not None, keep_sets=save is not None)
         elif D == 64:
-            o, P = ops.attention_fwd(qkv, Bn, T, heads, want_lse=save is not None)
+            o, P, *sets = ops.attention_fwd(qkv, Bn, T, heads, want_lse=save is not None, keep_sets=save is not None)
         else:
             o, P = ops.vit_attention_fwd(qkv, Bn, T, heads, D)
+            sets = []
         x2 = ops.linear(o_p if o_p is not None else (ops.split_planes(o) if pp else o), p["wout"], p["bout"], resid=x)
         xo, st2, h_pre = ffn(x2, save is not None)
         if save is not None:
-            save.update(o=o, P=P, x2=x2, st2=st2, h_pre=h_pre)
+            save.update(o=o, P=P, x2=x2, st2=st2, h_pre=h_pre, sets=sets[0] if sets else None)
     return xo, v
 
 
@@ -153,10 +155,10 @@
         do = ops.matmul_nn(dx2p if dx2p is not None else dx2, p["wout"])
         wout_parts.append((dx2, s["o"]))
         if D == 64 and pp and ops.attention_planes_ok() and not (s["want_v"] and dv is not None):
-            dqkv, dqkv_p = ops.attention_bwd(do, s["qkv"], s["o"], s["P"], Bn, T, heads, planes=True)
+            dqkv, dqkv_p = ops.attention_bwd(do, s["qkv"], s["o"], s["P"], Bn, T, heads, planes=True, sets=s.get("sets"))
             dqkv_amax = dqkv_p.amax
         elif D == 64:
-            dqkv = ops.attention_bwd(do, s["qkv"], s["o"], s["P"], Bn, T, heads)
+            dqkv = ops.attention_bwd(do, s["qkv"], s["o"], s["P"], Bn, T, heads, sets=s.get("sets"))
         else:
             dqkv = ops.vit_attention_bwd(do, s["qkv"], s["P"], Bn, T, heads, D)
         dx_res = dx2
diff --git a/semivl_amd/ops.py b/semivl_amd/ops.py
--- a/semivl_amd/ops.py
+++ b/semivl_amd/ops.py
@@ -837,42 +837,54 @@
 
 
 def _attn_ws(Bn, T, H, backward, dev):
-    n = L.load().svl_attention_h2_ws_bytes(Bn, T, H, 1 if backward else 0)
+    n = L.load().svl_attention_h2_ws_bytes(Bn, T, H, int(backward))
     return torch.empty(n + 1024, dtype=torch.uint8, device=dev), n
+
+
+def attention_tr_sets(on=None):
+    return bool(L.load().svl_attention_h2_tr_sets(-1 if on is None else int(bool(on))))
 
 
 def _ws_ptr(ws):
     return (ws.data_ptr() + 1023) // 1024 * 1024
 
 
-def attention_fwd(qkv, Bn, T, H, want_lse=True, planes=False, want_out=True):
+def attention_fwd(qkv, Bn, T, H, want_lse=True, planes=False, want_out=True, keep_sets=False):
     E = H * 64
     if planes and not attention_planes_ok():
         raise RuntimeError("attention_fwd: planes outputs need emulation mode 6 (attention_planes_ok())")
     out = empty(Bn * T, E, device=qkv.device)
     lse = empty(Bn * H * T, device=qkv.device) if want_lse else None
     e0 = _prof_begin()
+    sets = None
     if attention_h2():
-        ws, n = _attn_ws(Bn, T, H, False, qkv.device)
+        ws, n = _attn_ws(Bn, T, H, 0, qkv.device)
         L.check(L.load().svl_attention_fwd_h2(_p(qkv), Bn, T, H, _p(out), _p(lse), None, 0, _ws_ptr(ws), n, _st()),
                 "svl_attention_fwd_h2")
+        if keep_sets and not attention_tr_sets():
+            sets = ws
     else:
         L.check(L.load().svl_attention_fwd(_p(qkv), Bn, T, H, _p(out), _p(lse), None, 0, _st()), "svl_attention_fwd")
     _prof_end(_attn_family(), e0, 4.0 * Bn * H * T * T * 64, ("fwd_h2" if attention_h2() else "fwd", Bn, T, H))
     if not planes:
-        return out, lse
+        return (out, lse, sets) if keep_sets else (out, lse)
     op = split_planes(out)
-    return (out if want_out else None), lse, op
-
-
-def attention_bwd(dout, qkv, out, lse, Bn, T, H, planes=False):
+    return ((out if want_out else None), lse, op) + ((sets,) if keep_sets else ())
+
+
+def attention_bwd(dout, qkv, out, lse, Bn, T, H, planes=False, sets=None):
     if planes and not attention_planes_ok():
         raise RuntimeError("attention_bwd: planes outputs need emulation mode 6 (attention_planes_ok())")
     dqkv = torch.empty_like(qkv)
     ws = empty(Bn * H * T, device=qkv.device)
     e0 = _prof_begin()
-    if attention_h2():
-        wsb, n = _attn_ws(Bn, T, H, True, qkv.device)
+    if attention_h2() and sets is not None and not attention_tr_sets():
+        wsb, n = _attn_ws(Bn, T, H, 2, qkv.device)
+        L.check(L.load().svl_attention_bwd_h2_sets(_p(qkv), _p(out), _p(dout), _p(lse), Bn, T, H, _p(ws), _p(dqkv), _ws_ptr(sets),
+                                                   sets.numel() - (_ws_ptr(sets) - sets.data_ptr()), _ws_ptr(wsb), n, _st()),
+                "svl_attention_bwd_h2_sets")
+    elif attention_h2():
+        wsb, n = _attn_ws(Bn, T, H, 1, qkv.device)
         L.check(L.load().svl_attention_bwd_h2(_p(qkv), _p(out), _p(dout), _p(lse), Bn, T, H, _p(ws), _p(dqkv), None, 0,
                                               _ws_ptr(wsb), n, _st()), "svl_attention_bwd_h2")
     else:
```

Measured after the change: 106.8 images/s (median of 6 runs). +1.8%, better.
